# q8888620002/Group-Attribution-for-Diffusion-Models

Measured on AMD Instinct MI355X. Metric: shapley_coalitions_per_hour, higher is better.
Workload: dtype f32; 1 GPU; CIFAR-20 DDPM sFT coalition (BASELINE configs[1]): gd_steps=1000 @B=128 + 10240 samples x 100 DDIM steps @B=32 (32 batches fused/launch), UNet2DModel widths [128, 256, 256, 256] 35.75M params fp32; step = 1/1000 coalition = 1 train step + 1 sampler step @B=1024, enqueued on 3 HIP streams (the train step belongs to a later coalition: independent work); coalitions_in_flight=3

## Files before the change

group-attribution-for-diffusion-models_amd/csrc/gemm_dev.h:

```cpp
#pragma once
#include "gad_common.h"

namespace gadk {

constexpr int BK = 32;
constexpr int NTHREADS = 256;

static __device__ __attribute__((aligned(64))) float g_zero_block[16];

__device__ __forceinline__ int kc_off(int r, int q) { return r * BK + ((q ^ ((r >> 1) & 7)) << 2); }

__device__ __forceinline__ void glds16(const float* src, float* dst_wave_uniform) {
  __builtin_amdgcn_global_load_lds((const __attribute__((address_space(1))) void*)src,
                                   (__attribute__((address_space(3))) void*)dst_wave_uniform, 16, 0, 0);
}

__device__ __forceinline__ void barrier_after_dma() {
  __builtin_amdgcn_s_waitcnt(0x0F70);
  __syncthreads();
}

struct FastDiv {
  unsigned mul, shift;
  __device__ __forceinline__ int div(int n) const { return (int)((__umulhi((unsigned)n, mul) + (unsigned)n) >> shift); }
};

struct DevArgs {
  FastDiv fdC, fdKW, fdHoWo, fdWo, fdRpg, fdTaps;
  int kperm, taps;
  const float* A;
  const float* B;
  float* C;
  const unsigned short* Bh;
  const float* A2;
  int a_split, ldx2;
  const float* Ak2;
  const float* Bk2;
  int lda2, ldb2, k_split;
  int M, N, K;
  int lda, ldb, ldc;
  int batch_inner;
  long sA0, sA1, sB0, sB1, sC0, sC1;
  gad_conv_geom g;
  float alpha;
  const float* bias;
  const float* rowadd;
  int rows_per_group, ld_rowadd;
  const float* residual;
  int ldr;
  float* ws;
  int tiles_m, tiles_n, splitk, ktiles_per_split;
  int epi_vec;
};

__device__ __forceinline__ f32x4 ldg4(const float* p) { return *reinterpret_cast<const f32x4*>(p); }
__device__ __forceinline__ f32x4 zero4() { return f32x4{0.f, 0.f, 0.f, 0.f}; }
__device__ __forceinline__ f32x4 keep_if(f32x4 v, bool ok) { return ok ? v : zero4(); }

__device__ __forceinline__ int wave_id() { return __builtin_amdgcn_readfirstlane((int)(threadIdx.x >> 6)); }

template <int ROWS>
struct KCSlots {
  static constexpr int NS = ROWS / 32;
  __device__ static int row(int i) { return (threadIdx.x >> 3) + 32 * i; }
  __device__ static int kq4() { return ((threadIdx.x & 7) ^ ((threadIdx.x >> 4) & 7)) * 4; }
  __device__ static float* dma_dst(float* tile, int i) { return tile + (wave_id() * 8 + 32 * i) * BK; }
  __device__ static void store(float* lds, const f32x4* v, unsigned mask) {
#pragma unroll
    for (int i = 0; i < NS; ++i)
      *reinterpret_cast<f32x4*>(lds + row(i) * BK + (threadIdx.x & 7) * 4) = keep_if(v[i], (mask >> i) & 1u);
  }
};
template <int ROWS>
struct MCSlots {
  static constexpr int NS = ROWS / 32;
  static constexpr int F4 = ROWS / 4;
  static constexpr int KSTEP = NTHREADS / F4;
  __device__ static int krow(int i) { return threadIdx.x / F4 + KSTEP * i; }
  __device__ static int rq4() { return (threadIdx.x % F4) * 4; }
  __device__ static float* dma_dst(float* tile, int i) { return tile + (wave_id() * (KSTEP / 4) + KSTEP * i) * ROWS; }
  __device__ static void store(float* lds, const f32x4* v, unsigned mask) {
#pragma unroll
    for (int i = 0; i < NS; ++i)
      *reinterpret_cast<f32x4*>(lds + krow(i) * ROWS + rq4()) = keep_if(v[i], (mask >> i) & 1u);
  }
};

__device__ __forceinline__ const float* sel_src(const float* base, long off, bool ok) {
  const float* b = ok ? base : (const float*)g_zero_block;
  return b + (off & -(long)ok);
}


__device__ __forceinline__ int xcd_remap(int bid, int nwg) {
  int xcd = bid & 7, q = nwg >> 3, rr = nwg & 7;
  return (xcd < rr ? xcd * (q + 1) : rr * (q + 1) + (xcd - rr) * q) + (bid >> 3);
}

constexpr int EPI_LD = 40;
constexpr int EPI_WAVE = 32 * EPI_LD;

template <bool KC, int ROWS>
__device__ __forceinline__ f32x4 read_frag(const float* lds, int row, int g, int h) {
  if (KC) {
    return *reinterpret_cast<const f32x4*>(lds + kc_off(row, 2 * g + h));
  } else {
    const float* p = lds + (8 * g + 4 * h) * ROWS + row;
    return f32x4{p[0], p[ROWS], p[2 * ROWS], p[3 * ROWS]};
  }
}

template <int ROWS>
struct WinoKC : KCSlots<ROWS> {
  using S = KCSlots<ROWS>;
  const float* ptr[S::NS];
  long off;
  __device__ void init(const float* b, int ld, int row0, int nrows) {
#pragma unroll
    for (int i = 0; i < S::NS; ++i) {
      int r = row0 + S::row(i);
      r = r < nrows ? r : nrows - 1;
      ptr[i] = b + (long)r * ld + S::kq4();
    }
    off = 0;
  }
  __device__ __forceinline__ const float* src(int i) const { return ptr[i] + off; }
};

__device__ __forceinline__ void wino4_bt(const f32x4 (&d)[6], f32x4 (&t)[6]) {
  t[0] = 4.f * d[0] - 5.f * d[2] + d[4];
  t[1] = -4.f * (d[1] + d[2]) + d[3] + d[4];
  t[2] = 4.f * (d[1] - d[2]) - d[3] + d[4];
  t[3] = 2.f * (d[3] - d[1]) - d[2] + d[4];
  t[4] = 2.f * (d[1] - d[3]) - d[2] + d[4];
  t[5] = 4.f * d[1] - 5.f * d[3] + d[5];
// ... 4 lines not shown
```

group-attribution-for-diffusion-models_amd/csrc/gemm_f32.hip:

```cpp
#include "gad_common.h"
#include "gemm_dev.h"

using namespace gadk;

namespace gadk {
void launch_wino4_fused(const DevArgs& w, int bm, hipStream_t st);
}

namespace {

template <int ROWS, int VEC>
struct LoadKCDense : KCSlots<ROWS> {
  using S = KCSlots<ROWS>;
  const float* base;
  long roff[S::NS];
  unsigned rowmask;
  int kend, k;
  bool kok;
  __device__ void init(const float* b, int ld, int row0, int nrows, int kend_) {
    base = b;
    kend = kend_;
    rowmask = 0;
#pragma unroll
    for (int i = 0; i < S::NS; ++i) {
// ... 153 lines not shown
  __device__ void init(const float* b, int ld_, int row0, int nrows, int kend_) {
    kend = kend_;
    ld = ld_;
    int c0 = row0 + S::rq4();
    c0 = c0 < nrows ? c0 : nrows - 4;
#pragma unroll
    for (int i = 0; i < S::NS; ++i) ptr[i] = b + (long)S::krow(i) * ld + c0;
  }
  __device__ __forceinline__ void prep(int k0, unsigned& mask) { koff = (long)(k0 < kend ? k0 : kend - BK) * ld; mask = 0; }
  __device__ __forceinline__ const float* src(int i) const { return ptr[i] + koff; }
  __device__ __forceinline__ void slot(int, f32x4*, unsigned&) const {}
};
template <int ROWS>
struct LeanKC2 : KCSlots<ROWS> {
  using S = KCSlots<ROWS>;
  const float* ptr[S::NS];
  const float* ptr2[S::NS];
  int kend, ksplit, koff;
  bool second;
  __device__ void init(const float* b, int ld, const float* b2, int ld2, int ksplit_, int row0, int nrows, int kend_) {
    kend = kend_;
    ksplit = ksplit_;
#pragma unroll
    for (int i = 0; i < S::NS; ++i) {
      int r = row0 + S::row(i);
      r = r < nrows ? r : nrows - 1;
      ptr[i] = b + (long)r * ld + S::kq4();
      ptr2[i] = b2 + (long)r * ld2 + S::kq4();
    }
  }
  __device__ __forceinline__ void prep(int k0, unsigned& mask) {
    const int k = k0 < kend ? k0 : kend - BK;
    second = k >= ksplit;
    koff = second ? k - ksplit : k;
    mask = 0;
  }
  __device__ __forceinline__ const float* src(int i) const { return (second ? ptr2[i] : ptr[i]) + koff; }
  __device__ __forceinline__ void slot(int, f32x4*, unsigned&) const {}
};
template <int ROWS>
struct LeanMC2 : MCSlots<ROWS> {
  using S = MCSlots<ROWS>;
  const float* ptr[S::NS];
  const float* ptr2[S::NS];
  int kend, ksplit, ld, ld2;
  long koff;
  bool second;
  __device__ void init(const float* b, int ld_, const float* b2, int ld2_, int ksplit_, int row0, int nrows, int kend_) {
    kend = kend_;
    ksplit = ksplit_;
    ld = ld_;
    ld2 = ld2_;
    int c0 = row0 + S::rq4();
    c0 = c0 < nrows ? c0 : nrows - 4;
#pragma unroll
    for (int i = 0; i < S::NS; ++i) {
      ptr[i] = b + (long)S::krow(i) * ld + c0;
      ptr2[i] = b2 + (long)S::krow(i) * ld2 + c0;
    }
  }
  __device__ __forceinline__ void prep(int k0, unsigned& mask) {
    const int k = k0 < kend ? k0 : kend - BK;
    second = k >= ksplit;
    koff = second ? (long)(k - ksplit) * ld2 : (long)k * ld;
    mask = 0;
  }
  __device__ __forceinline__ const float* src(int i) const { return (second ? ptr2[i] : ptr[i]) + koff; }
  __device__ __forceinline__ void slot(int, f32x4*, unsigned&) const {}
};

template <int ROWS, bool TRANSPOSED, int VEC, bool TWO = false>
struct LoadConvRows : KCSlots<ROWS> {
  using S = KCSlots<ROWS>;
  const float* x;
  const float* x2;
  int csplit, ldx2;
  gad_conv_geom g;
  FastDiv fdC, fdKW;
  int bh[S::NS], bw[S::NS], boff[S::NS];
  unsigned rowmask;
  int kend, hlim, wlim;
  int k, c, r, s;
  bool kok;
  __device__ void init(const float* x_, const DevArgs& p, int row0, int nrows, int kend_) {
    x = x_;
    x2 = p.A2;
    csplit = p.a_split;
    ldx2 = p.ldx2;
    g = p.g;
    fdC = p.fdC;
    fdKW = p.fdKW;
    kend = kend_;
    hlim = g.upsample ? 2 * g.H : g.H;
    wlim = g.upsample ? 2 * g.W : g.W;
    rowmask = 0;
#pragma unroll
    for (int i = 0; i < S::NS; ++i) {
      int m = row0 + S::row(i);
      bool ok = m < nrows;
      int mm = ok ? m : 0;
      int img = p.fdHoWo.div(mm), rem = mm - img * (g.Ho * g.Wo);
      int oh = p.fdWo.div(rem), ow = rem - oh * g.Wo;
      boff[i] = img * g.H * g.W;
      rowmask |= (unsigned)ok << i;
      if (TRANSPOSED) {
        bh[i] = oh + g.pad_t;
        bw[i] = ow + g.pad_l;
      } else {
        bh[i] = oh * g.stride - g.pad_t;
        bw[i] = ow * g.stride - g.pad_l;
      }
    }
  }
  __device__ __forceinline__ long pix(int i, int rr, int ss, bool& ok) const { return (long)pixidx(i, rr, ss, ok) * g.ldx; }
  __device__ __forceinline__ int pixidx(int i, int rr, int ss, bool& ok) const {
    int ih, iw;
    if (TRANSPOSED) {
      int nh = bh[i] - rr, nw = bw[i] - ss;
      ok = (nh | nw) >= 0;
      if (g.stride == 2) {
        ok = ok && !((nh | nw) & 1);
        nh >>= 1;
        nw >>= 1;
      } else if (g.stride != 1) {
        ok = ok && (nh % g.stride == 0) && (nw % g.stride == 0);
        nh /= g.stride;
        nw /= g.stride;
      }
      ih = nh;
      iw = nw;
    } else {
      ih = bh[i] + rr;
      iw = bw[i] + ss;
      ok = (ih | iw) >= 0;
    }
    ok = ok && ih < hlim && iw < wlim;
    if (g.upsample) {
      ih >>= 1;
      iw >>= 1;
    }
    return boff[i] + ih * g.W + iw;
  }
  __device__ __forceinline__ void prep(int k0, unsigned& mask) {
    k = k0 + S::kq4();
    kok = k < kend;
    int kk = kok ? k : 0;
    int tap = fdC.div(kk);
    c = kk - tap * g.C;
    r = fdKW.div(tap);
    s = tap - r * g.KW;
    mask = rowmask;
  }
  __device__ __forceinline__ const float* src(int i) const {
    bool ok;
    if (TWO) {
      int pi = pixidx(i, r, s, ok);
      ok = ok && kok && ((rowmask >> i) & 1u);
      const bool second = c >= csplit;
      long off = second ? (long)pi * ldx2 + (c - csplit) : (long)pi * g.ldx + c;
      return sel_src(second ? x2 : x, off, ok);
    }
    long off = pix(i, r, s, ok) + c;
    ok = ok && kok && ((rowmask >> i) & 1u);
    return sel_src(x, off, ok);
  }
  __device__ __forceinline__ void slot(int i, f32x4* v, unsigned& mask) const {
    f32x4 t = zero4();
#pragma unroll
    for (int e = 0; e < 4; ++e) {
      int ke = k + e;
      bool ko = ke < kend;
      int kk = ko ? ke : 0;
      int tap = fdC.div(kk), cc = kk - tap * g.C;
      int rr = fdKW.div(tap), ss = tap - rr * g.KW;
      bool ok;
      long off = pix(i, rr, ss, ok) + cc;
      ok = ok && ko;
      float val = x[off & -(long)ok];
// ... 51 lines not shown
    fdHoWo = p.fdHoWo;
    fdWo = p.fdWo;
    kend = kend_;
    hlim = g.upsample ? 2 * g.H : g.H;
    wlim = g.upsample ? 2 * g.W : g.W;
    int n = col0 + S::rq4();
#pragma unroll
    for (int e = 0; e < NE; ++e) {
      int ne = n + e;
      nok[e] = ne < ncols;
      int nn = nok[e] ? ne : 0;
      int tap = p.fdC.div(nn);
      c[e] = nn - tap * g.C;
      r[e] = p.fdKW.div(tap);
      s[e] = tap - r[e] * g.KW;
    }
  }
  __device__ __forceinline__ void prep(int k0_, unsigned& mask) {
    k0 = k0_;
    mask = 0;
  }
  __device__ __forceinline__ long off_of(int i, int e, bool& ok) const {
    int m = k0 + S::krow(i);
    bool mok = m < kend;
    int mm = mok ? m : 0;
    int img = fdHoWo.div(mm), rem = mm - img * (g.Ho * g.Wo);
    int oh = fdWo.div(rem), ow = rem - oh * g.Wo;
    int ih = oh * g.stride - g.pad_t + r[e], iw = ow * g.stride - g.pad_l + s[e];
    ok = mok && nok[e] && (ih | iw) >= 0 && ih < hlim && iw < wlim;
    if (g.upsample) {
      ih >>= 1;
      iw >>= 1;
    }
    return (long)(img * g.H * g.W + ih * g.W + iw) * g.ldx + c[e];
  }
  __device__ __forceinline__ const float* src(int i) const {
    bool ok;
    long off = off_of(i, 0, ok);
    return sel_src(x, off, ok);
  }
  __device__ __forceinline__ void slot(int i, f32x4* v, unsigned& mask) const {
    f32x4 t = zero4();
#pragma unroll
    for (int e = 0; e < NE; ++e) {
      bool ok;
      long off = off_of(i, e, ok);
      float val = x[off & -(long)ok];
      t[e] = ok ? val : 0.f;
    }
    v[i] = t;
    mask |= 1u << i;
  }
};

template <int MODE, int ROWS, int VEC>
struct ALoader;
template <int ROWS, int VEC>
struct ALoader<GAD_A_KC, ROWS, VEC> : LoadKCDense<ROWS, VEC> {
  static constexpr bool KC = true;
  __device__ void setup(const DevArgs& p, const float* a, int row0, int kend) { this->init(a, p.lda, row0, p.M, kend); }
};
template <int ROWS, int VEC>
struct ALoader<GAD_A_MC, ROWS, VEC> : LoadMCDense<ROWS, VEC> {
  static constexpr bool KC = false;
  __device__ void setup(const DevArgs& p, const float* a, int row0, int kend) { this->init(a, p.lda, row0, p.M, kend); }
};
template <int ROWS, int VEC>
struct ALoader<GAD_A_CONV, ROWS, VEC> : LoadConvRows<ROWS, false, VEC> {
  static constexpr bool KC = true;
  __device__ void setup(const DevArgs& p, const float* a, int row0, int kend) { this->init(a, p, row0, p.M, kend); }
};
constexpr int A_CONV2 = 16;
template <int ROWS, int VEC>
struct ALoader<A_CONV2, ROWS, VEC> : LoadConvRows<ROWS, false, VEC, true> {
  static constexpr bool KC = true;
  __device__ void setup(const DevArgs& p, const float* a, int row0, int kend) { this->init(a, p, row0, p.M, kend); }
};
template <int ROWS, int VEC>
struct ALoader<GAD_A_CONVT, ROWS, VEC> : LoadConvRows<ROWS, true, VEC> {
  static constexpr bool KC = true;
  __device__ void setup(const DevArgs& p, const float* a, int row0, int kend) { this->init(a, p, row0, p.M, kend); }
};

constexpr int A_KC2 = 17;
template <int ROWS, int VEC>
struct ALoader<A_KC2, ROWS, VEC> : LoadKCDense2<ROWS> {
  static constexpr bool KC = true;
  __device__ void setup(const DevArgs& p, const float* a, int row0, int kend) {
    this->init(a, p.lda, p.Ak2, p.lda2, p.k_split, row0, p.M, kend);
  }
};

constexpr int A_KC_L = 20, A_MC_L = 21, B_KC_L = 22, B_MC_L = 23, A_KC2_L = 24, B_KC2_L = 25, B_MC2_L = 26;
template <int ROWS, int VEC>
struct ALoader<A_KC_L, ROWS, VEC> : LeanKC<ROWS> {
  static constexpr bool KC = true;
  __device__ void setup(const DevArgs& p, const float* a, int row0, int kend) { this->init(a, p.lda, row0, p.M, kend); }
};
template <int ROWS, int VEC>
struct ALoader<A_MC_L, ROWS, VEC> : LeanMC<ROWS> {
  static constexpr bool KC = false;
  __device__ void setup(const DevArgs& p, const float* a, int row0, int kend) { this->init(a, p.lda, row0, p.M, kend); }
};
template <int ROWS, int VEC>
struct ALoader<A_KC2_L, ROWS, VEC> : LeanKC2<ROWS> {
  static constexpr bool KC = true;
  __device__ void setup(const DevArgs& p, const float* a, int row0, int kend) {
    this->init(a, p.lda, p.Ak2, p.lda2, p.k_split, row0, p.M, kend);
  }
};

template <int MODE, int ROWS, int VEC>
struct BLoader;
constexpr int B_KC2 = 18, B_MC2 = 19;
template <int ROWS, int VEC>
struct BLoader<B_KC_L, ROWS, VEC> : LeanKC<ROWS> {
  static constexpr bool KC = true;
  __device__ void setup(const DevArgs& p, const float* b, int col0, int kend) { this->init(b, p.ldb, col0, p.N, kend); }
};
template <int ROWS, int VEC>
struct BLoader<B_MC_L, ROWS, VEC> : LeanMC<ROWS> {
  static constexpr bool KC = false;
  __device__ void setup(const DevArgs& p, const float* b, int col0, int kend) { this->init(b, p.ldb, col0, p.N, kend); }
};
template <int ROWS, int VEC>
struct BLoader<B_KC2_L, ROWS, VEC> : LeanKC2<ROWS> {
  static constexpr bool KC = true;
  __device__ void setup(const DevArgs& p, const float* b, int col0, int kend) {
    this->init(b, p.ldb, p.Bk2, p.ldb2, p.k_split, col0, p.N, kend);
  }
};
template <int ROWS, int VEC>
struct BLoader<B_MC2_L, ROWS, VEC> : LeanMC2<ROWS> {
  static constexpr bool KC = false;
  __device__ void setup(const DevArgs& p, const float* b, int col0, int kend) {
    this->init(b, p.ldb, p.Bk2, p.ldb2, p.k_split, col0, p.N, kend);
  }
};
template <int ROWS, int VEC>
struct BLoader<B_KC2, ROWS, VEC> : LoadKCDense2<ROWS> {
  static constexpr bool KC = true;
  __device__ void setup(const DevArgs& p, const float* b, int col0, int kend) {
    this->init(b, p.ldb, p.Bk2, p.ldb2, p.k_split, col0, p.N, kend);
  }
};
template <int ROWS, int VEC>
struct BLoader<B_MC2, ROWS, VEC> : LoadMCDense2<ROWS> {
  static constexpr bool KC = false;
  __device__ void setup(const DevArgs& p, const float* b, int col0, int kend) {
    this->init(b, p.ldb, p.Bk2, p.ldb2, p.k_split, col0, p.N, kend);
  }
};
template <int ROWS, int VEC>
struct BLoader<GAD_B_KC, ROWS, VEC> : LoadKCDense<ROWS, VEC> {
  static constexpr bool KC = true;
  __device__ void setup(const DevArgs& p, const float* b, int col0, int kend) { this->init(b, p.ldb, col0, p.N, kend); }
};
template <int ROWS, int VEC>
struct BLoader<GAD_B_MC, ROWS, VEC> : LoadMCDense<ROWS, VEC> {
  static constexpr bool KC = false;
  __device__ void setup(const DevArgs& p, const float* b, int col0, int kend) { this->init(b, p.ldb, col0, p.N, kend); }
};
template <int ROWS, int VEC>
struct BLoader<GAD_B_WDGRAD, ROWS, VEC> : LoadWDgrad<ROWS, VEC> {
  static constexpr bool KC = false;
  __device__ void setup(const DevArgs& p, const float* b, int col0, int kend) { this->init(b, p, col0, p.N, kend); }
};
template <int ROWS, int VEC>
struct BLoader<GAD_B_CONV, ROWS, VEC> : LoadConvCols<ROWS, VEC> {
  static constexpr bool KC = false;
  __device__ void setup(const DevArgs& p, const float* b, int col0, int kend) { this->init(b, p, col0, p.N, kend); }
};


template <int TM, int TN, int BM, int BN, int WM = 2, int WN = 2>
__device__ __forceinline__ void store_block(const DevArgs& p, const f32x16 (&acc)[TM][TN], int row0, int col0, int wm, int wn,
                                            int h, int l31, float* C, int ldc, const float* R, bool direct,
                                            float* scratch = nullptr) {
  if (scratch != nullptr && p.epi_vec) {
    const int lane = l31 + 32 * h;
    const int rr = lane >> 3, c4 = (lane & 7) * 4;
#pragma unroll
    for (int j = 0; j < TN; ++j) {
      const int n = col0 + wn * (BN / WN) + j * 32 + c4;
      const bool n_ok = n < p.N;
      float b0 = 0.f, b1 = 0.f, b2 = 0.f, b3 = 0.f;
      if (direct && p.bias && n_ok) {
        const f32x4 t = ldg4(p.bias + n);
        b0 = t[0]; b1 = t[1]; b2 = t[2]; b3 = t[3];
      }
#pragma unroll
      for (int i = 0; i < TM; ++i) {
#pragma unroll
        for (int e = 0; e < 16; ++e) scratch[((e & 3) + 8 * (e >> 2) + 4 * h) * EPI_LD + l31] = acc[i][j][e];
#pragma unroll
        for (int q = 0; q < 4; ++q) {
          const int r = rr + 8 * q;
          f32x4 v = *reinterpret_cast<const f32x4*>(scratch + r * EPI_LD + c4);
          const int m = row0 + wm * (BM / WM) + i * 32 + r;
          if (m >= p.M || !n_ok) continue;
          if (direct) {
            v = f32x4{__builtin_fmaf(v[0], p.alpha, b0), __builtin_fmaf(v[1], p.alpha, b1), __builtin_fmaf(v[2], p.alpha, b2),
                      __builtin_fmaf(v[3], p.alpha, b3)};
            if (p.rowadd) v += ldg4(p.rowadd + (long)p.fdRpg.div(m) * p.ld_rowadd + n);
            if (R) v += ldg4(R + (long)m * p.ldr + n);
          }
          *reinterpret_cast<f32x4*>(C + (long)m * ldc + n) = v;
        }
      }
    }
    return;
  }
#pragma unroll
  for (int j = 0; j < TN; ++j) {
    int n = col0 + wn * (BN / WN) + j * 32 + l31;
    if (n >= p.N) continue;
    float bias = (direct && p.bias) ? p.bias[n] : 0.f;
#pragma unroll
    for (int i = 0; i < TM; ++i) {
#pragma unroll
      for (int e = 0; e < 16; ++e) {
        int m = row0 + wm * (BM / WM) + i * 32 + (e & 3) + 8 * (e >> 2) + 4 * h;
        if (m >= p.M) continue;
        float v = acc[i][j][e];
        if (direct) {
          v = __builtin_fmaf(v, p.alpha, bias);
          if (p.rowadd) v += p.rowadd[(long)p.fdRpg.div(m) * p.ld_rowadd + n];
          if (R) v += R[(long)m * p.ldr + n];
        }
        C[(long)m * ldc + n] = v;
      }
    }
  }
}


template <int AM, int BMODE, int BM, int BN, int VEC, int TAG = 0>
__global__ __launch_bounds__(NTHREADS) void gemm_kernel(const DevArgs p) {
  constexpr int TM = BM / 64, TN = BN / 64;
  using AL = ALoader<AM, BM, VEC>;
  using BL = BLoader<BMODE, BN, VEC>;
  constexpr int A_TILE = BK * BM;
  constexpr int B_TILE = BK * BN;
  __shared__ __attribute__((aligned(16))) float lds[2 * (A_TILE + B_TILE)];

  const int t = xcd_remap(blockIdx.x, gridDim.x);
  int tiles = p.tiles_m * p.tiles_n;
  int zs = t / tiles, rem = t - zs * tiles;
  int tile_m = rem / p.tiles_n, tile_n = rem - tile_m * p.tiles_n;
  int z = zs / p.splitk, split = zs - z * p.splitk;
  int z0 = z / p.batch_inner, z1 = z - z0 * p.batch_inner;
  const float* A = p.A + z0 * p.sA0 + z1 * p.sA1;
  const float* B = p.B + z0 * p.sB0 + z1 * p.sB1;

  int row0 = tile_m * BM, col0 = tile_n * BN;
  int kbeg = split * p.ktiles_per_split * BK;
  int kend = min(p.K, kbeg + p.ktiles_per_split * BK);
  int nkt = (kend - kbeg + BK - 1) / BK;
  const int kt0 = split * p.ktiles_per_split;
  auto k0_of = [&](int kt) -> int {
    if (!p.kperm) return (kt0 + kt) * BK;
    int j = kt0 + kt;
    int chunk = p.fdTaps.div(j), tap = j - chunk * p.taps;
    return tap * p.g.C + chunk * BK;
  };
  if (p.kperm) kend = p.K;

  AL al;
  BL bl;
  al.setup(p, A, row0, kend);
  bl.setup(p, B, col0, kend);

  const int tid = threadIdx.x, wave = tid >> 6, lane = tid & 63;
  const int wm = wave >> 1, wn = wave & 1, h = lane >> 5, l31 = lane & 31;

  f32x16 acc[TM][TN];
#pragma unroll
  for (int i = 0; i < TM; ++i)
#pragma unroll
    for (int j = 0; j < TN; ++j)
#pragma unroll
      for (int e = 0; e < 16; ++e) acc[i][j][e] = 0.f;

  f32x4 ra[VEC == 4 ? 1 : AL::NS], rb[VEC == 4 ? 1 : BL::NS];
  unsigned ma = 0, mb = 0;
  auto stage_slot = [&](int piece, float* ta, float* tb) {
    constexpr int NSA = AL::NS, NSB = BL::NS;
    if (piece < NSA) {
      if (VEC == 4) glds16(al.src(piece), AL::dma_dst(ta, piece));
      else al.slot(piece, ra, ma);
    } else if (piece < NSA + NSB) {
      if (VEC == 4) glds16(bl.src(piece - NSA), BL::dma_dst(tb, piece - NSA));
      else bl.slot(piece - NSA, rb, mb);
    }
  };
  auto stage_commit = [&](float* ta, float* tb) {
    if (VEC != 4) {
      AL::store(ta, ra, ma);
      BL::store(tb, rb, mb);
    }
  };
  if (nkt > 0) {
    al.prep(k0_of(0), ma);
    bl.prep(k0_of(0), mb);
#pragma unroll
    for (int q = 0; q < AL::NS + BL::NS; ++q) stage_slot(q, lds, lds + A_TILE);
    stage_commit(lds, lds + A_TILE);
  }
  barrier_after_dma();

  for (int kt = 0; kt < nkt; ++kt) {
    float* cur = lds + (kt & 1) * (A_TILE + B_TILE);
    float* nxt = lds + ((kt + 1) & 1) * (A_TILE + B_TILE);
    const float* la = cur;
    const float* lb = cur + A_TILE;
    const int knext = (kt + 1 < nkt) ? k0_of(kt + 1) : p.K;
    al.prep(knext, ma);
    bl.prep(knext, mb);
    f32x4 fa[2][TM], fb[2][TN];
#pragma unroll
    for (int i = 0; i < TM; ++i) fa[0][i] = read_frag<AL::KC, BM>(la, wm * (BM / 2) + i * 32 + l31, 0, h);
#pragma unroll
    for (int j = 0; j < TN; ++j) fb[0][j] = read_frag<BL::KC, BN>(lb, wn * (BN / 2) + j * 32 + l31, 0, h);
#pragma unroll
    for (int g = 0; g < 4; ++g) {
#pragma unroll
      for (int s = 0; s < 4; ++s) {
#pragma unroll
        for (int i = 0; i < TM; ++i)
#pragma unroll
          for (int j = 0; j < TN; ++j)
            acc[i][j] = __builtin_amdgcn_mfma_f32_32x32x2f32(fa[g & 1][i][s], fb[g & 1][j][s], acc[i][j], 0, 0, 0);
        stage_slot(g * 4 + s, nxt, nxt + A_TILE);
        if (s == 1 && g < 3) {
#pragma unroll
          for (int i = 0; i < TM; ++i) fa[(g + 1) & 1][i] = read_frag<AL::KC, BM>(la, wm * (BM / 2) + i * 32 + l31, g + 1, h);
#pragma unroll
          for (int j = 0; j < TN; ++j) fb[(g + 1) & 1][j] = read_frag<BL::KC, BN>(lb, wn * (BN / 2) + j * 32 + l31, g + 1, h);
        }
#pragma unroll
        for (int q = 0; q < TM * TN; ++q) {
          __builtin_amdgcn_sched_group_barrier(0x008, 1, 0);
          __builtin_amdgcn_sched_group_barrier(0x002, 7, 0);
        }
        __builtin_amdgcn_sched_barrier(0);
      }
    }
    stage_commit(nxt, nxt + A_TILE);
    barrier_after_dma();
  }

  const bool direct = p.splitk == 1;
  float* C = direct ? p.C + z0 * p.sC0 + z1 * p.sC1 : p.ws + (long)zs * p.M * p.N;
  const float* R = (direct && p.residual) ? p.residual + z0 * p.sC0 + z1 * p.sC1 : nullptr;
  const int ldc = direct ? p.ldc : p.N;
  store_block<TM, TN, BM, BN>(p, acc, row0, col0, wm, wn, h, l31, C, ldc, R, direct, lds + (tid >> 6) * EPI_WAVE);
}

typedef __bf16 bf16x4_t __attribute__((ext_vector_type(4)));
typedef __bf16 bf16x8_t __attribute__((ext_vector_type(8)));
typedef short s16x4_t __attribute__((ext_vector_type(4)));
constexpr int LDK = BK + 8;
template <int ROWS> struct LdmOf { static constexpr int v = ROWS == 128 ? 160 : 96; };

__device__ __forceinline__ void store_bf16x4(unsigned short* dst, f32x4 v) {
  bf16x4_t h = {(__bf16)v[0], (__bf16)v[1], (__bf16)v[2], (__bf16)v[3]};
  *reinterpret_cast<bf16x4_t*>(dst) = h;
}

template <bool KC, int ROWS>
struct Bf16Tile;
template <int ROWS>
struct Bf16Tile<true, ROWS> {
  static constexpr int ELEMS = LDK * ROWS;
  __device__ static void put(unsigned short* tile, int i, f32x4 v) {
    store_bf16x4(tile + KCSlots<ROWS>::row(i) * LDK + KCSlots<ROWS>::kq4(), v);
  }
  __device__ static bf16x8_t frag(const unsigned short* tile, int r0, int ks, int lane) {
    return *reinterpret_cast<const bf16x8_t*>(tile + (r0 + (lane & 31)) * LDK + ks * 16 + 8 * (lane >> 5));
  }
};
template <int ROWS>
struct Bf16Tile<false, ROWS> {
  static constexpr int LDM = LdmOf<ROWS>::v;
  static constexpr int ELEMS = BK * LDM;
  __device__ static void put(unsigned short* tile, int i, f32x4 v) {
    store_bf16x4(tile + MCSlots<ROWS>::krow(i) * LDM + MCSlots<ROWS>::rq4(), v);
  }
  __device__ static bf16x8_t frag(const unsigned short* tile, int r0, int ks, int lane) {
    const int q = (lane & 15) >> 2, pp = lane & 3;
    const unsigned short* a0 = tile + (ks * 16 + 8 * (lane >> 5) + q) * LDM + r0 + 16 * ((lane >> 4) & 1) + 4 * pp;
    s16x4_t lo = __builtin_amdgcn_ds_read_tr16_b64_v4i16((__attribute__((address_space(3))) s16x4_t*)a0);
    s16x4_t hi = __builtin_amdgcn_ds_read_tr16_b64_v4i16((__attribute__((address_space(3))) s16x4_t*)(a0 + 4 * LDM));
    typedef short s16x8_t __attribute__((ext_vector_type(8)));
    s16x8_t both = {lo[0], lo[1], lo[2], lo[3], hi[0], hi[1], hi[2], hi[3]};
    return __builtin_bit_cast(bf16x8_t, both);
  }
};

template <int AM, int BMODE, int BM, int BN>
__global__ __launch_bounds__(NTHREADS) void gemm_bf16_kernel(const DevArgs p) {
  constexpr int TM = BM / 64, TN = BN / 64;
  using AL = ALoader<AM, BM, 4>;
  using BL = BLoader<BMODE, BN, 4>;
  using AT = Bf16Tile<AL::KC, BM>;
  using BT = Bf16Tile<BL::KC, BN>;
  constexpr int A_TILE = AT::ELEMS;
  constexpr int B_TILE = BT::ELEMS;
  __shared__ __attribute__((aligned(16))) unsigned short lds[2 * (A_TILE + B_TILE)];

  const int t = xcd_remap(blockIdx.x, gridDim.x);
  int tiles = p.tiles_m * p.tiles_n;
  int zs = t / tiles, rem = t - zs * tiles;
  int tile_m = rem / p.tiles_n, tile_n = rem - tile_m * p.tiles_n;
  int z = zs / p.splitk, split = zs - z * p.splitk;
  int z0 = z / p.batch_inner, z1 = z - z0 * p.batch_inner;
  const float* A = p.A + z0 * p.sA0 + z1 * p.sA1;
  const float* B = p.B + z0 * p.sB0 + z1 * p.sB1;

  int row0 = tile_m * BM, col0 = tile_n * BN;
  int kbeg = split * p.ktiles_per_split * BK;
  int kend = min(p.K, kbeg + p.ktiles_per_split * BK);
  int nkt = (kend - kbeg + BK - 1) / BK;
  const int kt0 = split * p.ktiles_per_split;
  auto k0_of = [&](int kt) -> int {
    if (!p.kperm) return (kt0 + kt) * BK;
    int j = kt0 + kt;
    int chunk = p.fdTaps.div(j), tap = j - chunk * p.taps;
    return tap * p.g.C + chunk * BK;
  };
  if (p.kperm) kend = p.K;

  AL al;
  BL bl;
  al.setup(p, A, row0, kend);
  bl.setup(p, B, col0, kend);

  const int tid = threadIdx.x, wave = tid >> 6, lane = tid & 63;
  const int wm = wave >> 1, wn = wave & 1, h = lane >> 5, l31 = lane & 31;
// ... 1079 lines not shown
#pragma unroll
      for (int i = 0; i < 6; ++i) gg[i][sx] = o[i];
    }
    float* u = dst + doff + (long)co * Cin + ci;
    const long ps = (long)Cout * Cin;
#pragma unroll
    for (int i = 0; i < 6; ++i) {
      float o[6];
      gmul(gg[i][0], gg[i][1], gg[i][2], o);
#pragma unroll
      for (int j = 0; j < 6; ++j) u[(long)(6 * i + j) * ps] = o[j];
    }
  }
}

struct WinoOut {
  const float* Mb;
  float* y;
  const float* bias;
  const float* rowadd;
  const float* residual;
  int N, ldc, ldr, ld_rowadd, Ho, Wo, TH, TW;
  long T;
  float alpha;
};

__device__ __forceinline__ void wino4_at(const f32x4 (&m)[6], f32x4 (&y)[4]) {
  const f32x4 s12 = m[1] + m[2], d12 = m[1] - m[2], s34 = m[3] + m[4], d34 = m[3] - m[4];
  y[0] = m[0] + s12 + s34;
  y[1] = d12 + 2.f * d34;
  y[2] = s12 + 4.f * s34;
  y[3] = d12 + 8.f * d34 + m[5];
}

template <bool HALF>
__global__ __launch_bounds__(256) void wino4_output_kernel(const WinoOut p) {
  const int N4 = p.N >> 2;
  const long idx = (long)blockIdx.x * 256 + threadIdx.x;
  if (idx >= p.T * N4) return;
  const long tile = idx / N4;
  const int n = (int)(idx - tile * N4) * 4;
  const int per = p.TH * p.TW;
  const int img = (int)(tile / per);
  const int r = (int)(tile - (long)img * per);
  const int ty = r / p.TW, tx = r - ty * p.TW;
  const long pos_stride = p.T * p.N;
  const float* src = p.Mb + tile * p.N + n;
  f32x4 t[4][HALF ? 4 : 6];
#pragma unroll
  for (int nu = 0; nu < (HALF ? 4 : 6); ++nu) {
    f32x4 m[6], col[4];
#pragma unroll
    for (int xi = 0; xi < 6; ++xi) m[xi] = ldg4(src + (long)((HALF ? 4 : 6) * xi + nu) * pos_stride);
    wino4_at(m, col);
#pragma unroll
    for (int i = 0; i < 4; ++i) t[i][nu] = col[i];
  }
  const f32x4 b = p.bias ? ldg4(p.bias + n) : zero4();
  const f32x4 ra = p.rowadd ? ldg4(p.rowadd + (long)img * p.ld_rowadd + n) : zero4();
#pragma unroll
  for (int i = 0; i < 4; ++i) {
    f32x4 y[4];
    if constexpr (HALF) {
#pragma unroll
      for (int j = 0; j < 4; ++j) y[j] = t[i][j];
    } else {
      f32x4 row6[6];
#pragma unroll
      for (int j = 0; j < 6; ++j) row6[j] = t[i][HALF ? 0 : j];
      wino4_at(row6, y);
    }
#pragma unroll
    for (int j = 0; j < 4; ++j) {
      const long pix = ((long)img * p.Ho + 4 * ty + i) * p.Wo + 4 * tx + j;
      f32x4 v = f32x4{__builtin_fmaf(y[j][0], p.alpha, b[0]), __builtin_fmaf(y[j][1], p.alpha, b[1]),
                      __builtin_fmaf(y[j][2], p.alpha, b[2]), __builtin_fmaf(y[j][3], p.alpha, b[3])};
      if (p.rowadd) v += ra;
      if (p.residual) v += ldg4(p.residual + pix * p.ldr + n);
      *reinterpret_cast<f32x4*>(p.y + pix * p.ldc + n) = v;
    }
  }
}

__global__ __launch_bounds__(256) void wino4_dy_kernel(const WinoIn p) {
  const int C4 = p.C >> 2;
  const long idx = (long)blockIdx.x * 256 + threadIdx.x;
  if (idx >= p.T * C4) return;
  const long tile = idx / C4;
  const int c = (int)(idx - tile * C4) * 4;
  const int per = p.TH * p.TW;
  const int n = (int)(tile / per);
  const int r = (int)(tile - (long)n * per);
  const int ty = r / p.TW, tx = r - ty * p.TW;
  const float* img = p.x + ((long)n * p.H * p.W + (long)(4 * ty) * p.W + 4 * tx) * p.ldx + c;
  auto amul = [](const f32x4 (&d)[4], f32x4 (&t)[6]) {
    const f32x4 s02 = d[0] + d[2], s13 = d[1] + d[3], a = d[0] + 4.f * d[2], b = 2.f * d[1] + 8.f * d[3];
    t[0] = d[0];
    t[1] = s02 + s13;
    t[2] = s02 - s13;
    t[3] = a + b;
    t[4] = a - b;
    t[5] = d[3];
  };
  f32x4 t[6][4];
#pragma unroll
  for (int dx = 0; dx < 4; ++dx) {
    f32x4 d[4], col[6];
#pragma unroll
    for (int dy = 0; dy < 4; ++dy) d[dy] = ldg4(img + ((long)dy * p.W + dx) * p.ldx);
    amul(d, col);
#pragma unroll
    for (int i = 0; i < 6; ++i) t[i][dx] = col[i];
  }
  const long pos_stride = p.T * p.C;
  float* out = p.V + tile * p.C + c;
#pragma unroll
  for (int i = 0; i < 6; ++i) {
    f32x4 v[6];
    amul(t[i], v);
#pragma unroll
    for (int j = 0; j < 6; ++j) *reinterpret_cast<f32x4*>(out + (long)(6 * i + j) * pos_stride) = v[j];
  }
}

__global__ __launch_bounds__(256) void wino4_dw_kernel(const float* dU, float* dW, int Cout, int Cin, int ldc) {
  const int C4 = Cin >> 2;
  const long idx = (long)blockIdx.x * 256 + threadIdx.x;
  if (idx >= (long)Cout * C4) return;
  const int co = (int)(idx / C4), ci = (int)(idx - (long)co * C4) * 4;
  const long ps = (long)Cout * Cin;
  const float* src = dU + (long)co * Cin + ci;
  auto gt = [](const f32x4 (&m)[6], f32x4 (&o)[3]) {
    const f32x4 s12 = m[1] + m[2], d21 = m[2] - m[1], s34 = m[3] + m[4], d34 = m[3] - m[4];
    o[0] = 0.25f * m[0] - (1.f / 6.f) * s12 + (1.f / 24.f) * s34;
    o[1] = (1.f / 6.f) * d21 + (1.f / 12.f) * d34;
    o[2] = (1.f / 6.f) * (s34 - s12) + m[5];
  };
  f32x4 t[3][6];
#pragma unroll
  for (int nu = 0; nu < 6; ++nu) {
    f32x4 m[6], col[3];
#pragma unroll
    for (int xi = 0; xi < 6; ++xi) m[xi] = ldg4(src + (long)(6 * xi + nu) * ps);
    gt(m, col);
#pragma unroll
    for (int r = 0; r < 3; ++r) t[r][nu] = col[r];
  }
  float* dst = dW + (long)co * ldc + ci;
#pragma unroll
  for (int r = 0; r < 3; ++r) {
    f32x4 o[3];
    gt(t[r], o);
#pragma unroll
    for (int sx = 0; sx < 3; ++sx) *reinterpret_cast<f32x4*>(dst + (long)(r * 3 + sx) * Cin) = o[sx];
  }
}

static FastDiv make_fastdiv(unsigned d) {
  FastDiv f;
  if (d == 0) d = 1;
  unsigned l = 0;
  while ((1ull << l) < d) ++l;
  f.shift = l;
  f.mul = (unsigned)((((1ull << l) - d) << 32) / d + 1);
  if (d == 1) f.mul = 0;
  return f;
}

static int pick_vec(const gad_gemm_args* a) {
  int vec = 4;
  const int am = a->a_mode, bmode = a->b_mode;
  if (am == GAD_A_KC && (a->K % 4 != 0 || a->lda % 4 != 0)) vec = 1;
  if (am == GAD_A_MC && (a->M % 4 != 0 || a->lda % 4 != 0)) vec = 1;
  if (bmode == GAD_B_KC && (a->K % 4 != 0 || a->ldb % 4 != 0)) vec = 1;
  if (bmode == GAD_B_MC && (a->N % 4 != 0 || a->ldb % 4 != 0)) vec = 1;
  if ((am == GAD_A_CONV || am == GAD_A_CONVT || bmode == GAD_B_CONV) && (a->g.C % 4 != 0 || a->g.ldx % 4 != 0)) vec = 1;
  return vec;
}

enum : int32_t {
  HINT_128 = 1,
  HINT_64 = 2,
  HINT_128x64 = 3,
  HINT_WGRAD_96 = 4, HINT_WGRAD_64 = 5, HINT_WGRAD_32 = 6,
  HINT_WINO2 = 7,
  HINT_WINO4 = 8,
  HINT_WINO4_FUSED32 = 9,
  HINT_WINO4_THREE = 10,
  HINT_WINO4_FUSED64 = 11,
  HINT_SPLIT_M = 1000,
};

struct Plan {
  int bm, bn, tiles_m, tiles_n, splitk, ktiles_per_split;
  long nblocks;
};

static bool dense_128x64_ok(const gad_gemm_args* a) {
  const bool dense = (a->a_mode == GAD_A_KC || a->a_mode == GAD_A_MC) && (a->b_mode == GAD_B_KC || a->b_mode == GAD_B_MC) &&
                     !(a->a_mode == GAD_A_MC && a->b_mode == GAD_B_KC);
  return dense && !a->A2 && pick_vec(a) == 4 && !(a->operand_precision == 1);
}
// ... 341 lines not shown
    const double t3 = t_gemm + (mb3 + y_bytes) / 4.9e12 + 12e-6;
    const bool full_ok = !(a->flags & GAD_GEMM_GENERAL_LOADERS) && a->tile_hint != HINT_WINO4_THREE;
    if (full_ok && (a->tile_hint == HINT_WINO4_FUSED32 || a->tile_hint == HINT_WINO4_FUSED64 || (t_full < 1.05 * t3 && blocks32 >= 320))) {
      p4.fused4 = 2;
      p4.bm = a->tile_hint == HINT_WINO4_FUSED64 ? 64 : narrow ? 65 : 32;
      p4.bn = p4.bm == 65 ? 32 : 64;
      p4.tiles_m = (int)gad_ceil_div(p4.T, p4.bm == 32 ? 32 : 64);
      p4.tiles_n = (int)gad_ceil_div(a->N, p4.bn);
    }
    const double mb = p4.fused4 == 2 ? 0.0 : mb3;
    p4.bytes = (int64_t)(vb + mb);
    t4 = (x_bytes + vb) / 4.9e12 + (p4.fused4 == 2 ? t_full : t3) + 6e-6;
  }
  if (a->tile_hint == HINT_WINO2 || force4) {
    if (a->tile_hint == HINT_WINO2 && f2_ok) { *wp = p2; return true; }
    if (force4 && f4_ok) { *wp = p4; return true; }
    return false;
  }
  double t_direct;
  PatchPlan pp;
  if (use_patch_conv_f32(a, &pp)) {
    t_direct = (double)gad_ceil_div(pp.blocks, 512) * pp.chunks_per_split * 9.0 * (128.0 * pp.bn * 64.0) / 0.264e12;
    if (pp.splitk > 1) t_direct += 4e-6 + (double)a->M * a->N * 4.0 * (pp.splitk + 1) / 3.0e12;
  } else {
    t_direct = 2.0 * a->M * (double)a->N * a->K / 110e12;
  }
  const double tw = t2 < t4 ? t2 : t4;
  if (!(tw < 0.9 * t_direct)) return false;
  *wp = t2 < t4 ? p2 : p4;
  return true;
}

struct WinoWgradPlan {
  long T;
  int64_t wy_bytes, v_bytes, du_bytes, bytes;
};
static bool use_wino_wgrad(const gad_gemm_args* a, WinoWgradPlan* wq) {
  const gad_conv_geom& g = a->g;
  if (!(a->flags & GAD_GEMM_WINO_WGRAD) || (a->flags & (GAD_GEMM_NO_WINO | GAD_GEMM_NO_PATCH | GAD_GEMM_INTERNAL_WINO4))) return false;
  if (a->operand_precision != 0 || a->a_mode != GAD_A_MC || a->b_mode != GAD_B_CONV || a->A2 || a->A_k2 || a->batch > 1) return false;
  if (!same_3x3(g) || (g.Ho & 3) || (g.Wo & 3)) return false;
  if (g.C % 4 != 0 || g.ldx % 4 != 0 || a->M % 4 != 0 || a->lda % 4 != 0 || a->N != 9 * g.C || a->ldc % 4 != 0) return false;
  if ((a->tile_hint != 0 && a->tile_hint != HINT_WINO4) || a->splitk_hint > 0 || a->K % (g.Ho * g.Wo) != 0) return false;
  if (a->alpha != 1.f || a->bias || a->rowadd || a->residual) return false;
  if (!(gad_aligned16(a->A) && gad_aligned16(a->B) && gad_aligned16(a->C))) return false;
  wq->T = (long)a->K / 16;
  wq->wy_bytes = (int64_t)36 * wq->T * a->M * 4;
  wq->v_bytes = (int64_t)36 * wq->T * g.C * 4;
  wq->du_bytes = (int64_t)36 * a->M * g.C * 4;
  wq->bytes = wq->wy_bytes + wq->v_bytes + wq->du_bytes;
  if (a->tile_hint == HINT_WINO4) return true;
  const double dy_bytes = 4.0 * a->K * a->M, x_bytes = 4.0 * (double)(a->K / (g.Ho * g.Wo)) * g.H * g.W * g.C;
  const double t_w = (dy_bytes + x_bytes + (double)wq->wy_bytes + (double)wq->v_bytes) / 4.9e12 + 36.0 * wq->T * a->M * (double)g.C * 2.0 / 100e12 +
                     3.0 * (double)wq->du_bytes / 3.0e12 + 30e-6;
  const double t_direct = 2.0 * a->K * (double)a->M * a->N / 115e12;
  return t_w < 0.9 * t_direct;
}


static gad_gemm_args products36(const gad_gemm_args* a, const float* A, const float* B, float* C, int am, int bm, int M, int N, int K) {
  gad_gemm_args sub = *a;
  sub.A = A; sub.B = B; sub.C = C;
  sub.a_mode = am; sub.b_mode = bm;
  sub.M = M; sub.N = N; sub.K = K;
  sub.lda = am == GAD_A_MC ? M : K; sub.ldb = bm == GAD_B_MC ? N : K; sub.ldc = N;
  sub.batch = 36; sub.batch_inner = 1;
  sub.strideA0 = (int64_t)M * K; sub.strideB0 = (int64_t)N * K; sub.strideC0 = (int64_t)M * N;
  sub.strideA1 = sub.strideB1 = sub.strideC1 = 0;
  sub.tile_hint = 0; sub.splitk_hint = 0;
  sub.flags = GAD_GEMM_INTERNAL_WINO4;
  sub.B_wino = nullptr; sub.B_wino4 = nullptr; sub.wino_ws = nullptr; sub.wino_ws_bytes = 0;
  sub.A2 = nullptr;
  return sub;
}
static gad_gemm_args wino_wgrad_products_args(const gad_gemm_args* a, const WinoWgradPlan& wq, float* Wy, float* V, float* dU) {
  return products36(a, Wy, V, dU, GAD_A_MC, GAD_B_MC, a->M, a->g.C, (int)wq.T);
}
static gad_gemm_args wino4_products_args(const gad_gemm_args* a, const WinoPlan& wp, float* V, float* Mb) {
  gad_gemm_args sub = products36(a, V, a->B_wino4, Mb, GAD_A_KC, GAD_B_KC, (int)wp.T, a->N, a->g.C);
  sub.alpha = 1.f; sub.bias = nullptr; sub.rowadd = nullptr; sub.residual = nullptr;
  return sub;
}

enum class RouteKind { ENGINE, PATCH_F32, PATCH_BF16, FEWOUT, WGRAD_PATCH, WINO, WINO_WGRAD, SPLIT_N, SPLIT_M };
struct Route {
  RouteKind kind;
  gad_gemm_args a;
  int vec;
  bool bf16;
  Plan plan;
  PatchPlan pp;
  WinoPlan wp;
  WinoWgradPlan wq;
  int wbm, wsplits;
  int split;
};

static Route route_of(const gad_gemm_args* args) {
  Route r{};
  r.a = canonical(args);
  const gad_gemm_args* a = &r.a;
  r.vec = pick_vec(a);
  r.bf16 = use_bf16(a);
  if (use_wino_wgrad(a, &r.wq)) r.kind = RouteKind::WINO_WGRAD;
  else if (use_wino(a, &r.wp)) r.kind = RouteKind::WINO;
  else if (patch_split_n(a, &r.split)) {
    r.kind = RouteKind::SPLIT_N;
    use_patch_conv_f32(a, &r.pp);
  } else if (wgrad_split_m(a, &r.split)) {
    r.kind = RouteKind::SPLIT_M;
    r.wsplits = wgrad_patch_splits(a, &r.wbm);
  } else if (use_fewout_conv(a)) r.kind = RouteKind::FEWOUT;
  else if ((r.wsplits = wgrad_patch_splits(a, &r.wbm))) r.kind = RouteKind::WGRAD_PATCH;
  else if (use_patch_conv(a)) r.kind = RouteKind::PATCH_BF16;
  else if (use_patch_conv_f32(a, &r.pp)) r.kind = RouteKind::PATCH_F32;
  else {
    r.kind = RouteKind::ENGINE;
    r.plan = make_plan(a);
  }
  return r;
}

struct Report { int kid, tile, splitk; };
static Report report(const Route& r) {
  switch (r.kind) {
    case RouteKind::ENGINE: return {r.bf16 ? 1 : 0, r.plan.bm, r.plan.splitk};
    case RouteKind::PATCH_F32: return {2, r.pp.bn, r.pp.splitk};
    case RouteKind::SPLIT_N: return {2, 224, r.pp.splitk};
    case RouteKind::SPLIT_M: return {2, 224, r.wsplits};
    case RouteKind::WGRAD_PATCH: return {2, r.wbm, r.wsplits};
    case RouteKind::PATCH_BF16: return {3, 128, 1};
    case RouteKind::FEWOUT: return {4, 256, 1};
    case RouteKind::WINO: return {r.wp.f == 2 ? 5 : 6, r.wp.f == 2 ? r.wp.bn : (r.wp.fused4 == 2 ? r.wp.bm : 128), 1};
    case RouteKind::WINO_WGRAD: return {7, 128, 1};
  }
  return {-1, 0, 0};
}

static void split_halves(const Route& r, gad_gemm_args* lo, gad_gemm_args* hi) {
  const gad_gemm_args* a = &r.a;
  const int s = r.split;
  *lo = *a;
  *hi = *a;
  if (r.kind == RouteKind::SPLIT_M) {
    if (a->tile_hint >= HINT_SPLIT_M) lo->tile_hint = hi->tile_hint = 0;
    lo->M = s;
    hi->M = a->M - s;
    hi->A = a->A + s;
    hi->C = a->C + (long)s * a->ldc;
    return;
  }
  lo->B_wino = lo->B_wino4 = hi->B_wino = hi->B_wino4 = nullptr;
  lo->wino_ws = hi->wino_ws = nullptr;
  lo->wino_ws_bytes = hi->wino_ws_bytes = 0;
  lo->N = s;
  hi->N = a->N - s;
  hi->B = a->B + (long)s * a->ldb;
  hi->C = a->C + s;
  if (a->bias) hi->bias = a->bias + s;
  if (a->rowadd) hi->rowadd = a->rowadd + s;
  if (a->residual) hi->residual = a->residual + s;
}

static int64_t workspace_bytes(const Route& r) {
  const gad_gemm_args* a = &r.a;
  switch (r.kind) {
    case RouteKind::ENGINE: case RouteKind::PATCH_F32: case RouteKind::WGRAD_PATCH: case RouteKind::PATCH_BF16: case RouteKind::FEWOUT: {
      const int splitk = report(r).splitk;
      return splitk > 1 ? (int64_t)(a->batch > 0 ? a->batch : 1) * splitk * a->M * a->N * (int64_t)sizeof(float) : 0;
    }
    case RouteKind::WINO: {
      if (r.wp.f == 2 || r.wp.fused4) return 0;
      const gad_gemm_args sub = wino4_products_args(a, r.wp, nullptr, nullptr);
      return gad_gemm_workspace_bytes(&sub);
    }
    case RouteKind::WINO_WGRAD: {
      const gad_gemm_args sub = wino_wgrad_products_args(a, r.wq, nullptr, nullptr, nullptr);
      return gad_gemm_workspace_bytes(&sub);
    }
    case RouteKind::SPLIT_N: case RouteKind::SPLIT_M: {
      gad_gemm_args lo, hi;
      split_halves(r, &lo, &hi);
      const int64_t wl = gad_gemm_workspace_bytes(&lo), wh = gad_gemm_workspace_bytes(&hi);
      return wl > wh ? wl : wh;
    }
  }
  return 0;
}

extern "C" int gad_gemm_uses_bf16(const gad_gemm_args* a) { return a && route_of(a).bf16 ? 1 : 0; }

extern "C" int gad_gemm_kernel_id(const gad_gemm_args* a) { return a ? report(route_of(a)).kid : -1; }

extern "C" int gad_gemm_plan(const gad_gemm_args* a, int32_t* tile, int32_t* splitk, int32_t* vec) {
  GAD_CHECK(a && tile && splitk && vec, "gad_gemm_plan: null pointer");
  const Route r = route_of(a);
  const Report rep = report(r);
  *tile = rep.tile;
  *splitk = rep.splitk;
  *vec = r.vec;
  return 0;
}

extern "C" int64_t gad_gemm_wino_bytes(const gad_gemm_args* a) {
  if (!a) return 0;
  const Route r = route_of(a);
  return r.kind == RouteKind::WINO ? r.wp.bytes : r.kind == RouteKind::WINO_WGRAD ? r.wq.bytes : 0;
}

extern "C" int64_t gad_gemm_workspace_bytes(const gad_gemm_args* a) { return a ? workspace_bytes(route_of(a)) : 0; }

extern "C" int gad_wino_weights(const float* src, float* dst, const int64_t* table, int64_t n_tiles, void* stream) {
  GAD_CHECK(src && dst && table && n_tiles > 0 && n_tiles < (1L << 31), "gad_wino_weights: bad arguments");
  static_assert(sizeof(long) == sizeof(int64_t), "table rows are 64-bit");
  hipLaunchKernelGGL(wino_weights_kernel, dim3((unsigned)n_tiles), dim3(256), 0, (hipStream_t)stream, src, dst, (const long*)table);
  GAD_LAUNCH_CHECK("gad_wino_weights");
  return 0;
}

extern "C" int gad_wino4_weights(const float* src, float* dst, const int64_t* table, int64_t n_tiles, void* stream) {
  GAD_CHECK(src && dst && table && n_tiles > 0 && n_tiles < (1L << 31), "gad_wino4_weights: bad arguments");
  hipLaunchKernelGGL(wino4_weights_kernel, dim3((unsigned)n_tiles), dim3(256), 0, (hipStream_t)stream, src, dst, (const long*)table);
  GAD_LAUNCH_CHECK("gad_wino4_weights");
  return 0;
}


static int check_args(const gad_gemm_args* a) {
  GAD_CHECK(a->M > 0 && a->N > 0 && a->K > 0, "gad_gemm: bad shape M=%d N=%d K=%d", a->M, a->N, a->K);
  const int am = a->a_mode, bmode = a->b_mode;
  GAD_CHECK(gad_aligned16(a->A) && gad_aligned16(a->B), "gad_gemm: A/B must be 16-byte aligned");
  const int k_first = a->A_k2 ? a->k_split : a->K;
  if (am == GAD_A_KC) GAD_CHECK(a->lda >= k_first, "gad_gemm: A_KC needs lda >= K (K=%d lda=%d)", k_first, a->lda);
  if (am == GAD_A_MC) GAD_CHECK(a->lda >= a->M, "gad_gemm: A_MC needs lda >= M (M=%d lda=%d)", a->M, a->lda);
  if (bmode == GAD_B_KC) GAD_CHECK(a->ldb >= k_first, "gad_gemm: B_KC needs ldb >= K (K=%d ldb=%d)", k_first, a->ldb);
  if (bmode == GAD_B_MC) GAD_CHECK(a->ldb >= a->N, "gad_gemm: B_MC needs ldb >= N (N=%d ldb=%d)", a->N, a->ldb);
  const bool convA = am == GAD_A_CONV || am == GAD_A_CONVT;
  if (convA || bmode == GAD_B_CONV || bmode == GAD_B_WDGRAD) {
    const gad_conv_geom& g = a->g;
    GAD_CHECK(g.H > 0 && g.W > 0 && g.C > 0 && g.Ho > 0 && g.Wo > 0 && g.KH > 0 && g.KW > 0 && g.stride > 0 &&
              g.ldx >= (a->A2 ? a->a_split : g.C), "gad_gemm: bad conv geometry");
    GAD_CHECK((long)g.H * g.W * g.ldx < (1L << 31), "gad_gemm: image too large for 32-bit pixel offsets");
    if (convA) {
      GAD_CHECK(a->K == g.KH * g.KW * g.C, "gad_gemm: conv K=%d != KH*KW*C=%d", a->K, g.KH * g.KW * g.C);
      GAD_CHECK(a->M % (g.Ho * g.Wo) == 0, "gad_gemm: conv M=%d not a multiple of Ho*Wo", a->M);
      GAD_CHECK((long)(a->M / (g.Ho * g.Wo)) * g.H * g.W < (1L << 31), "gad_gemm: too many pixels");
    }
    if (bmode == GAD_B_WDGRAD) {
      GAD_CHECK(am == GAD_A_CONVT, "gad_gemm: B_WDGRAD pairs with A_CONVT");
      GAD_CHECK(a->N % 4 == 0, "gad_gemm: B_WDGRAD needs N%%4==0 (N=%d)", a->N);
    }
    if (bmode == GAD_B_CONV) {
      GAD_CHECK(a->N == g.KH * g.KW * g.C, "gad_gemm: wgrad N=%d != KH*KW*C=%d", a->N, g.KH * g.KW * g.C);
      GAD_CHECK(a->K % (g.Ho * g.Wo) == 0, "gad_gemm: wgrad K=%d not a multiple of Ho*Wo", a->K);
      GAD_CHECK((long)(a->K / (g.Ho * g.Wo)) * g.H * g.W < (1L << 31), "gad_gemm: too many pixels");
    }
  }
  const int vec = pick_vec(a);
  if (a->A2) {
    GAD_CHECK(am == GAD_A_CONV && bmode == GAD_B_KC, "gad_gemm: A2 (two-source gather) is an A_CONV x B_KC feature");
    GAD_CHECK(a->a_split > 0 && a->a_split < a->g.C && a->a_split % 32 == 0 && a->g.C % 32 == 0,
              "gad_gemm: two-source gather needs a_split and C multiples of 32 (a_split=%d C=%d)", a->a_split, a->g.C);
    GAD_CHECK(a->ldx2 >= a->g.C - a->a_split && a->ldx2 % 4 == 0 && gad_aligned16(a->A2) && vec == 4,
              "gad_gemm: two-source gather: bad ldx2 / alignment");
  }
  if (a->A_k2) {
    GAD_CHECK(am == GAD_A_KC && (bmode == GAD_B_KC || bmode == GAD_B_MC) && a->B_k2 && !a->A2 && a->batch <= 1,
              "gad_gemm: the K-concatenated form (A_k2 / B_k2) is an A_KC x B_KC|B_MC feature");
    GAD_CHECK(a->k_split > 0 && a->k_split < a->K && a->k_split % 32 == 0, "gad_gemm: k_split must be a multiple of 32 inside (0, K) (k_split=%d K=%d)", a->k_split, a->K);
    const int k2 = a->K - a->k_split;
    GAD_CHECK(a->lda >= a->k_split && a->lda_k2 >= k2 && a->lda_k2 % 4 == 0 && k2 % 4 == 0 && gad_aligned16(a->A_k2) && gad_aligned16(a->B_k2),
              "gad_gemm: K-concatenated operands need 16-byte alignment and K2 %% 4 == 0 (K2=%d lda_k2=%d)", k2, a->lda_k2);
    if (bmode == GAD_B_KC) GAD_CHECK(a->ldb >= a->k_split && a->ldb_k2 >= k2 && a->ldb_k2 % 4 == 0, "gad_gemm: bad ldb_k2");
    else GAD_CHECK(a->ldb_k2 >= a->N && a->ldb_k2 % 4 == 0, "gad_gemm: bad ldb_k2");
    GAD_CHECK(vec == 4, "gad_gemm: the K-concatenated form needs the float4 path");
  }
  if (a->rowadd) GAD_CHECK(a->rows_per_group > 0 && a->ld_rowadd >= a->N, "gad_gemm: bad rowadd");
  if (a->residual) GAD_CHECK(a->ldr >= a->N, "gad_gemm: bad residual stride");
  GAD_CHECK(a->ldc >= a->N, "gad_gemm: ldc < N");
  GAD_CHECK(a->operand_precision == 0 || a->operand_precision == 1, "gad_gemm: operand_precision must be 0 (f32) or 1 (bf16 allowed)");
  return 0;
}

static int check_stage_flags(const Route& r) {
  const bool only_input = (r.a.flags & GAD_GEMM_WINO_ONLY_INPUT) != 0, skip_input = (r.a.flags & GAD_GEMM_WINO_SKIP_INPUT) != 0;
  GAD_CHECK(!(only_input && skip_input), "gad_gemm: GAD_GEMM_WINO_ONLY_INPUT and GAD_GEMM_WINO_SKIP_INPUT exclude each other");
  GAD_CHECK(!only_input || r.kind == RouteKind::WINO,
            "gad_gemm: GAD_GEMM_WINO_ONLY_INPUT on a launch that takes no Winograd forward route (kernel id %d)", report(r).kid);
  GAD_CHECK(!skip_input || r.kind == RouteKind::WINO || r.kind == RouteKind::WINO_WGRAD,
            "gad_gemm: GAD_GEMM_WINO_SKIP_INPUT on a launch that takes no Winograd route (kernel id %d)", report(r).kid);
  return 0;
}

static DevArgs dev_args(const gad_gemm_args* a) {
  DevArgs d;
  d.A = a->A; d.B = a->B; d.C = a->C;
  d.A2 = a->A2; d.a_split = a->a_split; d.ldx2 = a->ldx2;
  d.Ak2 = a->A_k2; d.Bk2 = a->B_k2; d.lda2 = a->lda_k2; d.ldb2 = a->ldb_k2; d.k_split = a->k_split;
  d.Bh = nullptr;
  d.M = a->M; d.N = a->N; d.K = a->K;
  d.lda = a->lda; d.ldb = a->ldb; d.ldc = a->ldc;
  d.batch_inner = a->batch_inner > 0 ? a->batch_inner : 1;
  d.sA0 = a->strideA0; d.sA1 = a->strideA1; d.sB0 = a->strideB0; d.sB1 = a->strideB1;
  d.sC0 = a->strideC0; d.sC1 = a->strideC1;
  d.g = a->g;
  d.fdC = make_fastdiv(a->g.C);
  d.fdKW = make_fastdiv(a->g.KW);
  d.fdHoWo = make_fastdiv((unsigned)a->g.Ho * a->g.Wo);
  d.fdWo = make_fastdiv(a->g.Wo);
  d.fdRpg = make_fastdiv(a->rows_per_group > 0 ? a->rows_per_group : 1);
  d.taps = a->g.KH * a->g.KW;
  d.fdTaps = make_fastdiv(d.taps > 0 ? d.taps : 1);
  const bool convA = a->a_mode == GAD_A_CONV || a->a_mode == GAD_A_CONVT;
  d.kperm = (convA && d.taps > 1 && a->g.C % BK == 0 && !(a->flags & GAD_GEMM_TAP_MAJOR_K)) ? 1 : 0;
  d.alpha = a->alpha;
  d.bias = a->bias; d.rowadd = a->rowadd; d.rows_per_group = a->rows_per_group > 0 ? a->rows_per_group : 1;
  d.ld_rowadd = a->ld_rowadd; d.residual = a->residual; d.ldr = a->ldr;
  d.ws = (float*)a->ws;
  d.tiles_m = d.tiles_n = d.splitk = d.ktiles_per_split = 1;
  d.epi_vec = (!(a->flags & GAD_GEMM_SCALAR_EPILOGUE) && gad_aligned16(a->C) && a->ldc % 4 == 0 && a->N % 4 == 0 &&
               a->strideC0 % 4 == 0 && a->strideC1 % 4 == 0 && (!a->bias || gad_aligned16(a->bias)) &&
               (!a->rowadd || (gad_aligned16(a->rowadd) && a->ld_rowadd % 4 == 0)) &&
               (!a->residual || (gad_aligned16(a->residual) && a->ldr % 4 == 0)) && (!a->ws || gad_aligned16(a->ws))) ? 1 : 0;
  return d;
}

static int launch_wino_wgrad(const Route& r, void* stream) {
  const gad_gemm_args* a = &r.a;
  const WinoWgradPlan& wq = r.wq;
  const gad_conv_geom& g = a->g;
  hipStream_t st = (hipStream_t)stream;
  GAD_CHECK(a->wino_ws && a->wino_ws_bytes >= wq.bytes && gad_aligned16(a->wino_ws),
            "gad_gemm: Winograd weight-gradient workspace too small or misaligned (%lld < %lld)", (long long)a->wino_ws_bytes, (long long)wq.bytes);
  float* Wy = (float*)a->wino_ws;
  float* V = Wy + wq.wy_bytes / 4;
  float* dU = V + wq.v_bytes / 4;
  const bool have_v = (a->flags & GAD_GEMM_WINO_SKIP_INPUT) && a->B_wino4 != nullptr;
  if (have_v) {
    GAD_CHECK(gad_aligned16(a->B_wino4), "gad_gemm: the kept Winograd input image (B_wino4 of a weight-gradient launch) must be 16-byte aligned");
    V = const_cast<float*>(a->B_wino4);
  }
  WinoIn wy;
  wy.x = a->A; wy.V = Wy;
  wy.H = g.Ho; wy.W = g.Wo; wy.C = a->M; wy.ldx = a->lda; wy.up = 0;
  wy.TH = g.Ho / 4; wy.TW = g.Wo / 4; wy.T = wq.T;
  WinoIn wi;
  wi.x = a->B; wi.V = V;
  wi.H = g.H; wi.W = g.W; wi.C = g.C; wi.ldx = g.ldx; wi.up = g.upsample ? 1 : 0;
  wi.TH = wy.TH; wi.TW = wy.TW; wi.T = wq.T;
  const long iy = wq.T * (a->M / 4), ix = wq.T * (g.C / 4);
  GAD_CHECK(gad_ceil_div(iy, 256) < (1L << 31) && gad_ceil_div(ix, 256) < (1L << 31), "gad_gemm: Winograd transform grid too large");
  hipLaunchKernelGGL(wino4_dy_kernel, dim3((unsigned)gad_ceil_div(iy, 256)), dim3(256), 0, st, wy);
  if (!have_v) hipLaunchKernelGGL(wino4_input_kernel, dim3((unsigned)gad_ceil_div(ix, 256)), dim3(256), 0, st, wi);
  GAD_LAUNCH_CHECK("gad_gemm(winograd wgrad transforms)");
  const gad_gemm_args sub = wino_wgrad_products_args(a, wq, Wy, V, dU);
  if (const int rc = gad_gemm(&sub, stream)) return rc;
  const long items = (long)a->M * (g.C / 4);
  hipLaunchKernelGGL(wino4_dw_kernel, dim3((unsigned)gad_ceil_div(items, 256)), dim3(256), 0, st, dU, a->C, a->M, g.C, a->ldc);
  GAD_LAUNCH_CHECK("gad_gemm(winograd wgrad output transform)");
  return 0;
}

static int launch_wino(const Route& r, const DevArgs& d, void* stream) {
  const gad_gemm_args* a = &r.a;
  const WinoPlan& wp = r.wp;
  const gad_conv_geom& g = a->g;
  hipStream_t st = (hipStream_t)stream;
  GAD_CHECK(a->wino_ws && a->wino_ws_bytes >= wp.bytes && gad_aligned16(a->wino_ws) && gad_aligned16(wp.f == 2 ? a->B_wino : a->B_wino4),
            "gad_gemm: Winograd workspace too small or misaligned (%lld < %lld)", (long long)a->wino_ws_bytes, (long long)wp.bytes);
  WinoIn wi;
  wi.x = a->A; wi.V = (float*)a->wino_ws;
  wi.H = g.H; wi.W = g.W; wi.C = g.C; wi.ldx = g.ldx; wi.up = g.upsample ? 1 : 0;
  wi.TH = g.Ho / wp.f; wi.TW = g.Wo / wp.f; wi.T = wp.T;
  const long items = wp.T * (g.C / 4);
  GAD_CHECK(gad_ceil_div(items, 256) < (1L << 31), "gad_gemm: Winograd input transform grid too large");
  const bool only_input = (a->flags & GAD_GEMM_WINO_ONLY_INPUT) != 0, skip_input = (a->flags & GAD_GEMM_WINO_SKIP_INPUT) != 0;
  auto products = [&](const float* U) {
    DevArgs w = d;
    w.A = wi.V; w.B = U;
    w.M = (int)wp.T; w.N = a->N; w.K = g.C;
    w.lda = g.C; w.ldb = g.C;
    w.sA0 = wp.T * (long)g.C; w.sB0 = (long)a->N * g.C;
    w.fdHoWo = make_fastdiv((unsigned)(wi.TH * wi.TW));
    w.fdWo = make_fastdiv((unsigned)wi.TW);
    w.tiles_m = wp.tiles_m; w.tiles_n = wp.tiles_n;
    return w;
  };
  if (wp.f == 4) {
    if (!skip_input) {
      hipLaunchKernelGGL(wino4_input_kernel, dim3((unsigned)gad_ceil_div(items, 256)), dim3(256), 0, st, wi);
      GAD_LAUNCH_CHECK("gad_gemm(winograd F4 input transform)");
    }
    if (only_input) return 0;
    if (wp.fused4 == 2) {
      GAD_CHECK((long)wp.tiles_m * wp.tiles_n < (1L << 31), "gad_gemm: Winograd grid too large");
      gadk::launch_wino4_fused(products(a->B_wino4), wp.bm, st);
      GAD_LAUNCH_CHECK("gad_gemm(winograd F4 fused products + output transform)");
      return 0;
    }
    float* Mb = wi.V + 36 * wp.T * (long)g.C;
    WinoOut wo;
    wo.Mb = Mb; wo.y = a->C; wo.bias = a->bias; wo.rowadd = a->rowadd; wo.residual = a->residual;
    wo.N = a->N; wo.ldc = a->ldc; wo.ldr = a->ldr; wo.ld_rowadd = a->ld_rowadd;
    wo.Ho = g.Ho; wo.Wo = g.Wo; wo.TH = wi.TH; wo.TW = wi.TW; wo.T = wp.T; wo.alpha = a->alpha;
    const long oitems = wp.T * (a->N / 4);
    if (wp.fused4 == 1) {
      DevArgs w = d;
      w.A = wi.V; w.B = a->B_wino4; w.C = Mb;
      w.M = (int)wp.T; w.N = a->N; w.K = g.C;
      w.lda = g.C; w.ldb = g.C; w.ldc = a->N;
      w.sA0 = wp.T * (long)g.C; w.sB0 = (long)a->N * g.C; w.sC0 = wp.T * (long)a->N;
      w.tiles_m = wp.tiles_m; w.tiles_n = wp.tiles_n;
      w.splitk = 1; w.bias = nullptr; w.rowadd = nullptr; w.residual = nullptr; w.alpha = 1.f;
      w.epi_vec = 1;
      dim3 grid((unsigned)((long)wp.tiles_m * wp.tiles_n * 6)), block(NTHREADS);
      if (wp.bm == 64) hipLaunchKernelGGL((wino4_gemm_kernel<64, 128>), grid, block, 0, st, w);
      else hipLaunchKernelGGL((wino4_gemm_kernel<128, 64>), grid, block, 0, st, w);
      GAD_LAUNCH_CHECK("gad_gemm(winograd F4 products)");
      hipLaunchKernelGGL(wino4_output_kernel<true>, dim3((unsigned)gad_ceil_div(oitems, 256)), dim3(256), 0, st, wo);
      GAD_LAUNCH_CHECK("gad_gemm(winograd F4 output transform)");
      return 0;
    }
    const gad_gemm_args sub = wino4_products_args(a, wp, wi.V, Mb);
    if (const int rc = gad_gemm(&sub, stream)) return rc;
    hipLaunchKernelGGL(wino4_output_kernel<false>, dim3((unsigned)gad_ceil_div(oitems, 256)), dim3(256), 0, st, wo);
    GAD_LAUNCH_CHECK("gad_gemm(winograd F4 output transform)");
    return 0;
  }
  if (!skip_input) {
    hipLaunchKernelGGL(wino_input_kernel, dim3((unsigned)gad_ceil_div(items, 256)), dim3(256), 0, st, wi);
    GAD_LAUNCH_CHECK("gad_gemm(winograd input transform)");
  }
  if (only_input) return 0;
  const DevArgs w = products(a->B_wino);
  dim3 grid((unsigned)((long)wp.tiles_m * wp.tiles_n)), block(NTHREADS);
// ... 41 lines not shown
  if (a->g.Wo == 64) GAD_WGRAD(64);
  else if (a->g.Wo == 32) GAD_WGRAD(32);
  else if (a->g.Wo == 16) GAD_WGRAD(16);
  else GAD_WGRAD(8);
#undef GAD_WGRAD
  GAD_LAUNCH_CHECK("gad_gemm(wgrad3x3 patch)");
  if (d.splitk > 1) {
    launch_splitk_reduce(d, 1, st);
    GAD_LAUNCH_CHECK("gad_gemm(wgrad splitk reduce)");
  }
  return 0;
}

static int launch_patch_bf16(const Route& r, DevArgs& d, hipStream_t st) {
  const gad_gemm_args* a = &r.a;
  d.tiles_m = (int)gad_ceil_div(a->M, 128);
  d.tiles_n = (int)gad_ceil_div(a->N, 128);
  d.splitk = 1;
  dim3 grid((unsigned)(d.tiles_m * d.tiles_n)), block(NTHREADS);
  const bool wb = a->B_bf16 != nullptr;
  if (wb) GAD_CHECK(gad_aligned16(a->B_bf16) && a->ldb % 8 == 0, "gad_gemm: B_bf16 must be 16-byte aligned with ldb %% 8 == 0");
  d.Bh = (const unsigned short*)a->B_bf16;
#define GAD_PATCH_BF16(W_, NI_)                                                                         \
  do {                                                                                                  \
    if (wb) hipLaunchKernelGGL((conv3x3_patch_bf16_kernel<W_, NI_, true>), grid, block, 0, st, d);      \
    else hipLaunchKernelGGL((conv3x3_patch_bf16_kernel<W_, NI_, false>), grid, block, 0, st, d);        \
  } while (0)
  if (a->g.Wo == 64) GAD_PATCH_BF16(64, 1);
  else if (a->g.Wo == 32) GAD_PATCH_BF16(32, 1);
  else if (a->g.Wo == 16) GAD_PATCH_BF16(16, 1);
  else if (a->g.Wo == 8) GAD_PATCH_BF16(8, 2);
  else GAD_PATCH_BF16(4, 8);
#undef GAD_PATCH_BF16
  GAD_LAUNCH_CHECK("gad_gemm(conv3x3 patch)");
  return 0;
}

static int launch_patch_f32(const Route& r, DevArgs& d, hipStream_t st) {
  const gad_gemm_args* a = &r.a;
  const PatchPlan& pp = r.pp;
  d.tiles_m = (int)gad_ceil_div(a->M, 128);
  d.tiles_n = (int)gad_ceil_div(a->N, pp.bn);
  d.splitk = pp.splitk;
  d.ktiles_per_split = pp.chunks_per_split;
  if (pp.splitk > 1) {
    int64_t need = (int64_t)pp.splitk * a->M * a->N * (int64_t)sizeof(float);
    GAD_CHECK(a->ws && a->ws_bytes >= need, "gad_gemm: patch-conv split-K workspace too small (%lld < %lld)", (long long)a->ws_bytes, (long long)need);
  }
  dim3 grid((unsigned)pp.blocks), block(NTHREADS);
  const bool dg = a->a_mode == GAD_A_CONVT;
#define GAD_PATCH(W_, NI_)                                                                                           \
  do {                                                                                                               \
    if (dg) hipLaunchKernelGGL((conv3x3_patch_f32_kernel<W_, NI_, true>), grid, block, 0, st, d);                    \
    else if (pp.bn == 96) hipLaunchKernelGGL((conv3x3_patch_f32_kernel<W_, NI_, false, 96>), grid, block, 0, st, d);   \
    else if (pp.bn == 160) hipLaunchKernelGGL((conv3x3_patch_f32_kernel<W_, NI_, false, 160>), grid, block, 0, st, d); \
    else hipLaunchKernelGGL((conv3x3_patch_f32_kernel<W_, NI_, false>), grid, block, 0, st, d);                      \
  } while (0)
  if (a->g.Wo == 64) GAD_PATCH(64, 1);
  else if (a->g.Wo == 32) GAD_PATCH(32, 1);
  else if (a->g.Wo == 16) GAD_PATCH(16, 1);
  else if (a->g.Wo == 8) GAD_PATCH(8, 2);
  else GAD_PATCH(4, 8);
#undef GAD_PATCH
  GAD_LAUNCH_CHECK("gad_gemm(conv3x3 patch f32)");
  if (pp.splitk > 1) {
    launch_splitk_reduce(d, 1, st);
    GAD_LAUNCH_CHECK("gad_gemm(patch splitk reduce)");
  }
  return 0;
}

static int launch_engine(const Route& r, DevArgs& d, hipStream_t st) {
  const gad_gemm_args* a = &r.a;
  const Plan& pl = r.plan;
  const int am = a->a_mode, bmode = a->b_mode, vec = r.vec;
  const bool bf16 = r.bf16;
  const long batch = a->batch > 0 ? a->batch : 1;
  GAD_CHECK(pl.nblocks > 0 && pl.nblocks < (1L << 31), "gad_gemm: grid too large");
  if (pl.splitk > 1) {
    int64_t need = (int64_t)batch * pl.splitk * a->M * a->N * (int64_t)sizeof(float);
    GAD_CHECK(a->ws && a->ws_bytes >= need, "gad_gemm: split-K workspace too small (%lld < %lld)", (long long)a->ws_bytes, (long long)need);
  }
  d.tiles_m = pl.tiles_m; d.tiles_n = pl.tiles_n; d.splitk = pl.splitk; d.ktiles_per_split = pl.ktiles_per_split;
  if (a->A2) {
    if (bf16) launch_bf16<A_CONV2, GAD_B_KC>(d, pl, st);
    else launch_mode<A_CONV2, GAD_B_KC, 4>(d, pl, st);
  } else if (a->A_k2) {
    const bool lean = vec == 4 && a->K % BK == 0 && a->k_split % BK == 0 && !(a->flags & GAD_GEMM_GENERAL_LOADERS);
    if (bmode == GAD_B_KC) {
      if (bf16 && lean) launch_bf16<A_KC2_L, B_KC2_L>(d, pl, st);
      else if (bf16) launch_bf16<A_KC2, B_KC2>(d, pl, st);
      else if (lean) launch_mode<A_KC2_L, B_KC2_L, 4>(d, pl, st);
      else launch_mode<A_KC2, B_KC2, 4>(d, pl, st);
    } else {
      if (bf16 && lean) launch_bf16<A_KC2_L, B_MC2_L>(d, pl, st);
      else if (bf16) launch_bf16<A_KC2, B_MC2>(d, pl, st);
      else if (lean) launch_mode<A_KC2_L, B_MC2_L, 4>(d, pl, st);
      else launch_mode<A_KC2, B_MC2, 4>(d, pl, st);
    }
  } else if (vec == 4 && a->K % BK == 0 && !(a->flags & GAD_GEMM_GENERAL_LOADERS) &&
             ((am == GAD_A_KC && (bmode == GAD_B_KC || bmode == GAD_B_MC)) || (am == GAD_A_MC && bmode == GAD_B_MC))) {
    if (bf16) {
      if (am == GAD_A_KC && bmode == GAD_B_KC) launch_bf16<A_KC_L, B_KC_L>(d, pl, st);
      else if (am == GAD_A_KC) launch_bf16<A_KC_L, B_MC_L>(d, pl, st);
      else launch_bf16<A_MC_L, B_MC_L>(d, pl, st);
    } else if (am == GAD_A_KC && bmode == GAD_B_KC) {
      if (a->flags & GAD_GEMM_INTERNAL_WINO4) launch_mode<A_KC_L, B_KC_L, 4, 1>(d, pl, st);
      else launch_mode<A_KC_L, B_KC_L, 4>(d, pl, st);
    }
    else if (am == GAD_A_KC) launch_mode<A_KC_L, B_MC_L, 4>(d, pl, st);
    else launch_mode<A_MC_L, B_MC_L, 4>(d, pl, st);
  } else
#define GAD_CASE(AMODE, BMODE_)                                                        \
  if (am == AMODE && bmode == BMODE_) {                                                \
    if (bf16) launch_bf16<AMODE, BMODE_>(d, pl, st);                                   \
    else if (vec == 4) launch_mode<AMODE, BMODE_, 4>(d, pl, st);                       \
    else launch_mode<AMODE, BMODE_, 1>(d, pl, st);                                     \
  } else
  GAD_CASE(GAD_A_KC, GAD_B_KC)
  GAD_CASE(GAD_A_KC, GAD_B_MC)
  GAD_CASE(GAD_A_MC, GAD_B_MC)
  GAD_CASE(GAD_A_CONV, GAD_B_KC)
  GAD_CASE(GAD_A_CONVT, GAD_B_WDGRAD)
  GAD_CASE(GAD_A_MC, GAD_B_CONV)
  {
    gad_set_error("gad_gemm: unsupported mode pair a_mode=%d b_mode=%d", am, bmode);
    return 1;
  }
#undef GAD_CASE
  GAD_LAUNCH_CHECK("gad_gemm");
  if (pl.splitk > 1) {
    launch_splitk_reduce(d, (int)batch, st);
    GAD_LAUNCH_CHECK("gad_gemm(splitk reduce)");
  }
  return 0;
}

extern "C" int gad_gemm(const gad_gemm_args* args, void* stream) {
  GAD_CHECK(args && args->A && args->B && args->C, "gad_gemm: null pointer");
  const gad_gemm_args canon = canonical(args);
  if (const int rc = check_args(&canon)) return rc;
  const Route r = route_of(&canon);
  if (const int rc = check_stage_flags(r)) return rc;
  hipStream_t st = (hipStream_t)stream;
  DevArgs d = dev_args(&r.a);
  switch (r.kind) {
    case RouteKind::SPLIT_N: case RouteKind::SPLIT_M: {
      gad_gemm_args lo, hi;
      split_halves(r, &lo, &hi);
      const int rc = gad_gemm(&lo, stream);
      return rc ? rc : gad_gemm(&hi, stream);
    }
    case RouteKind::WINO_WGRAD: return launch_wino_wgrad(r, stream);
    case RouteKind::WINO: return launch_wino(r, d, stream);
    case RouteKind::FEWOUT: return launch_fewout(r, d, st);
    case RouteKind::WGRAD_PATCH: return launch_wgrad_patch(r, d, st);
    case RouteKind::PATCH_BF16: return launch_patch_bf16(r, d, st);
    case RouteKind::PATCH_F32: return launch_patch_f32(r, d, st);
    case RouteKind::ENGINE: return launch_engine(r, d, st);
  }
  return 1;
}
```

group-attribution-for-diffusion-models_amd/gad/_capi.py:

```python
import ctypes as C
import os

_HERE = os.path.dirname(os.path.abspath(__file__))
LIB_PATH = os.path.join(_HERE, "libgad_hip.so")


class GadError(RuntimeError):
    pass


class ConvGeom(C.Structure):
    _fields_ = [("H", C.c_int32), ("W", C.c_int32), ("C", C.c_int32), ("ldx", C.c_int32),
                ("Ho", C.c_int32), ("Wo", C.c_int32), ("KH", C.c_int32), ("KW", C.c_int32),
                ("stride", C.c_int32), ("pad_t", C.c_int32), ("pad_l", C.c_int32), ("upsample", C.c_int32)]


class GemmArgs(C.Structure):
    _fields_ = [("A", C.c_void_p), ("B", C.c_void_p), ("C", C.c_void_p),
                ("a_mode", C.c_int32), ("b_mode", C.c_int32),
                ("M", C.c_int32), ("N", C.c_int32), ("K", C.c_int32),
                ("lda", C.c_int32), ("ldb", C.c_int32), ("ldc", C.c_int32),
                ("batch", C.c_int32), ("batch_inner", C.c_int32),
                ("strideA0", C.c_int64), ("strideA1", C.c_int64), ("strideB0", C.c_int64),
                ("strideB1", C.c_int64), ("strideC0", C.c_int64), ("strideC1", C.c_int64),
                ("g", ConvGeom),
                ("alpha", C.c_float), ("bias", C.c_void_p), ("rowadd", C.c_void_p),
                ("rows_per_group", C.c_int32), ("ld_rowadd", C.c_int32),
                ("residual", C.c_void_p), ("ldr", C.c_int32),
                ("ws", C.c_void_p), ("ws_bytes", C.c_int64),
                ("tile_hint", C.c_int32), ("splitk_hint", C.c_int32), ("operand_precision", C.c_int32),
                ("A2", C.c_void_p), ("a_split", C.c_int32), ("ldx2", C.c_int32), ("B_bf16", C.c_void_p),
                ("A_k2", C.c_void_p), ("B_k2", C.c_void_p), ("lda_k2", C.c_int32), ("ldb_k2", C.c_int32),
                ("k_split", C.c_int32), ("flags", C.c_int32),
                ("B_wino", C.c_void_p), ("wino_ws", C.c_void_p), ("wino_ws_bytes", C.c_int64), ("B_wino4", C.c_void_p)]


class GroupNormArgs(C.Structure):
    _fields_ = [("x", C.c_void_p), ("y", C.c_void_p), ("gamma", C.c_void_p), ("beta", C.c_void_p),
                ("mean", C.c_void_p), ("rstd", C.c_void_p), ("dy", C.c_void_p),
                ("dgamma", C.c_void_p), ("dbeta", C.c_void_p),
                ("B", C.c_int32), ("HW", C.c_int32), ("C", C.c_int32), ("G", C.c_int32),
                ("eps", C.c_float), ("silu", C.c_int32), ("ws", C.c_void_p), ("ws_bytes", C.c_int64),
                ("x2", C.c_void_p), ("C1", C.c_int32), ("flags", C.c_int32), ("dx_add", C.c_void_p)]


class AttentionArgs(C.Structure):
    _fields_ = [("q", C.c_void_p), ("k", C.c_void_p), ("v", C.c_void_p), ("o", C.c_void_p), ("lse", C.c_void_p),
                ("d_o", C.c_void_p), ("delta", C.c_void_p), ("dq", C.c_void_p), ("dk", C.c_void_p), ("dv", C.c_void_p),
                ("B", C.c_int32), ("heads", C.c_int32), ("Tq", C.c_int32), ("Tk", C.c_int32), ("d", C.c_int32),
                ("ldq", C.c_int32), ("ldk", C.c_int32), ("ldv", C.c_int32), ("ldo", C.c_int32),
                ("ld_do", C.c_int32), ("ld_dq", C.c_int32), ("ld_dk", C.c_int32), ("ld_dv", C.c_int32),
                ("stride_q", C.c_int64), ("stride_k", C.c_int64), ("stride_v", C.c_int64), ("stride_o", C.c_int64),
                ("stride_do", C.c_int64), ("stride_dq", C.c_int64), ("stride_dk", C.c_int64), ("stride_dv", C.c_int64),
                ("scale", C.c_float), ("operand_precision", C.c_int32),
                ("ws", C.c_void_p), ("ws_bytes", C.c_int64), ("flags", C.c_int32)]


ATTN_TWO_KERNEL_BWD, ATTN_NARROW_FWD = 1, 2


class HGemmArgs(C.Structure):
    _fields_ = [("A", C.c_void_p), ("A2", C.c_void_p), ("B", C.c_void_p), ("B2", C.c_void_p), ("C", C.c_void_p),
                ("M", C.c_int32), ("N", C.c_int32), ("K", C.c_int32),
                ("lda", C.c_int32), ("lda2", C.c_int32), ("ldb", C.c_int32), ("ldb2", C.c_int32), ("ldc", C.c_int32),
                ("k_split", C.c_int32), ("conv", C.c_int32),
                ("H", C.c_int32), ("W", C.c_int32), ("Cin", C.c_int32),
                ("Ho", C.c_int32), ("Wo", C.c_int32), ("KH", C.c_int32), ("KW", C.c_int32), ("stride", C.c_int32),
                ("pad_t", C.c_int32), ("pad_l", C.c_int32), ("upsample", C.c_int32),
                ("alpha", C.c_float), ("bias", C.c_void_p), ("rowadd", C.c_void_p),
                ("rows_per_group", C.c_int32), ("ld_rowadd", C.c_int32),
                ("residual", C.c_void_p), ("ldr", C.c_int32),
                ("out_f32", C.c_int32), ("accumulate", C.c_int32),
                ("ws", C.c_void_p), ("ws_bytes", C.c_int64),
                ("tile_hint", C.c_int32), ("splitk_hint", C.c_int32)]


class AdamArgs(C.Structure):
    _fields_ = [("p", C.c_void_p), ("g", C.c_void_p), ("m", C.c_void_p), ("v", C.c_void_p), ("ema", C.c_void_p),
                ("n", C.c_int64), ("sumsq", C.c_void_p), ("max_norm", C.c_float),
                ("lr", C.c_float), ("beta1", C.c_float), ("beta2", C.c_float), ("eps", C.c_float),
                ("weight_decay", C.c_float), ("adamw", C.c_int32), ("step", C.c_int32), ("ema_decay", C.c_float)]


class JLArgs(C.Structure):
    _fields_ = [("A", C.c_void_p), ("lda", C.c_int64), ("G", C.c_int32), ("P", C.c_int64), ("p0", C.c_int64),
                ("d", C.c_int32), ("seed", C.c_uint32), ("model_id", C.c_uint32), ("type", C.c_int32),
                ("accumulate", C.c_int32), ("out", C.c_void_p), ("workspace", C.c_void_p), ("workspace_bytes", C.c_int64)]


class HGemmSegArgs(C.Structure):
    _fields_ = [("A", C.c_void_p), ("B", C.c_void_p), ("C", C.c_void_p), ("ws", C.c_void_p), ("ws_bytes", C.c_int64),
                ("c_seg_stride", C.c_int64), ("M", C.c_int32), ("N", C.c_int32), ("L", C.c_int32), ("S", C.c_int32),
                ("lda", C.c_int32), ("ldb", C.c_int32), ("ldc", C.c_int32), ("alpha", C.c_float), ("accumulate", C.c_int32),
                ("splitk_hint", C.c_int32)]


JL_NORMAL, JL_RADEMACHER = 0, 1
POOL_MAX, POOL_AVG, POOL_AVG_VALID = 0, 1, 2
GELU_ERF, GELU_QUICK = 0, 1
SIM_X_F32, SIM_X_U8 = 0, 1

GEMM_NO_PATCH, GEMM_TAP_MAJOR_K, GEMM_SCALAR_EPILOGUE, GEMM_GENERAL_LOADERS, GN_TWO_PASS = 1, 2, 4, 8, 1
GEMM_NO_WINO = 16
GEMM_WINO_WGRAD = 32
GEMM_WINO_ONLY_INPUT, GEMM_WINO_SKIP_INPUT = 64, 128
A_KC, A_MC, A_CONV, A_CONVT = 0, 1, 2, 3
B_KC, B_MC, B_WDGRAD, B_CONV = 0, 1, 2, 3

_vp, _i32, _i64, _f32, _f64 = C.c_void_p, C.c_int32, C.c_int64, C.c_float, C.c_double

SIGNATURES = {
    "gad_version": (C.c_int, []),
    "gad_last_error": (C.c_char_p, []),
    "gad_gemm_workspace_bytes": (_i64, [C.POINTER(GemmArgs)]),
    "gad_gemm": (C.c_int, [C.POINTER(GemmArgs), _vp]),
    "gad_gemm_uses_bf16": (C.c_int, [C.POINTER(GemmArgs)]),
    "gad_gemm_kernel_id": (C.c_int, [C.POINTER(GemmArgs)]),
    "gad_gemm_wino_bytes": (_i64, [C.POINTER(GemmArgs)]),
    "gad_wino_weights": (C.c_int, [_vp, _vp, _vp, _i64, _vp]),
    "gad_wino4_weights": (C.c_int, [_vp, _vp, _vp, _i64, _vp]),
    "gad_groupnorm_one_pass": (C.c_int, [C.POINTER(GroupNormArgs)]),
    "gad_gemm_plan": (C.c_int, [C.POINTER(GemmArgs), C.POINTER(_i32), C.POINTER(_i32), C.POINTER(_i32)]),
    "gad_groupnorm_workspace_bytes": (_i64, [C.POINTER(GroupNormArgs)]),
    "gad_groupnorm_silu_fwd": (C.c_int, [C.POINTER(GroupNormArgs), _vp]),
    "gad_groupnorm_silu_bwd": (C.c_int, [C.POINTER(GroupNormArgs), _vp]),
    "gad_groupnorm_wino4_ok": (C.c_int, [C.POINTER(GroupNormArgs), C.c_int32]),
    "gad_groupnorm_silu_wino4": (C.c_int, [C.POINTER(GroupNormArgs), _vp, C.c_int32, _vp]),
    "gad_attention_supported": (C.c_int, [_i32]),
    "gad_attention_uses_bf16": (C.c_int, [C.POINTER(AttentionArgs), _i32]),
    "gad_attention_bwd_workspace_bytes": (_i64, [C.POINTER(AttentionArgs)]),
    "gad_attention_fwd": (C.c_int, [C.POINTER(AttentionArgs), _vp]),
    "gad_attention_bwd": (C.c_int, [C.POINTER(AttentionArgs), _vp]),
    "gad_softmax_fwd": (C.c_int, [_vp, _vp, _i64, _i32, _f32, _vp]),
    "gad_softmax_bwd": (C.c_int, [_vp, _vp, _vp, _i64, _i32, _f32, _vp]),
    "gad_layernorm_workspace_bytes": (_i64, [_i64, _i32]),
    "gad_layernorm_fwd": (C.c_int, [_vp, _vp, _vp, _vp, _vp, _vp, _i64, _i32, _f32, _vp]),
    "gad_layernorm_bwd": (C.c_int, [_vp, _vp, _vp, _vp, _vp, _vp, _vp, _vp, _i64, _i32, _vp, _i64, _vp]),
    "gad_geglu_fwd": (C.c_int, [_vp, _vp, _i64, _i32, _vp]),
    "gad_geglu_bwd": (C.c_int, [_vp, _vp, _vp, _i64, _i32, _vp]),
    "gad_timestep_embedding": (C.c_int, [_vp, _vp, _i32, _i32, _i32, _f32, _f32, _vp]),
    "gad_rotate_conv3x3": (C.c_int, [_vp, _vp, _vp, _i32, _vp]),
    "gad_silu_fwd": (C.c_int, [_vp, _vp, _i64, _vp]),
    "gad_silu_bwd": (C.c_int, [_vp, _vp, _vp, _i64, _vp]),
    "gad_concat_channels": (C.c_int, [_vp, _vp, _vp, _i64, _i32, _i32, _vp]),
    "gad_split_channels": (C.c_int, [_vp, _vp, _vp, _i64, _i32, _i32, _vp]),
    "gad_nchw_to_nhwc": (C.c_int, [_vp, _vp, _i32, _i32, _i32, _vp]),
    "gad_nhwc_to_nchw": (C.c_int, [_vp, _vp, _i32, _i32, _i32, _vp]),
    "gad_upsample2x_bwd": (C.c_int, [_vp, _vp, _i32, _i32, _i32, _i32, _vp]),
    "gad_colsum": (C.c_int, [_vp, _vp, _i32, _i64, _i32, _vp, _i64, _vp]),
    "gad_add_noise": (C.c_int, [_vp, _vp, _vp, _vp, _vp, _i32, _i64, _vp]),
    "gad_ddim_step": (C.c_int, [_vp, _vp, _vp, _i64, _f32, _f32, _f32, _vp]),
    "gad_cfg_ddim_step": (C.c_int, [_vp, _vp, _vp, _i64, _f32, _f32, _f32, _f32, _vp]),
    "gad_to_image01": (C.c_int, [_vp, _vp, _i64, _vp]),
    "gad_mse_fwd_bwd": (C.c_int, [_vp, _vp, _vp, _vp, _i64, _f32, _vp, _i64, _vp]),
    "gad_sumsq": (C.c_int, [_vp, _vp, _i64, _vp, _i64, _vp]),
    "gad_clip_adam_ema": (C.c_int, [C.POINTER(AdamArgs), _vp]),
    "gad_ema_update": (C.c_int, [_vp, _vp, _i64, _f32, _vp]),
    "gad_hgemm_workspace_bytes": (_i64, [C.POINTER(HGemmArgs)]),
    "gad_hgemm_plan": (C.c_int, [C.POINTER(HGemmArgs), C.POINTER(_i32), C.POINTER(_i32)]),
    "gad_hgemm": (C.c_int, [C.POINTER(HGemmArgs), _vp]),
    "gad_hgemm_tn_workspace_bytes": (_i64, [C.POINTER(HGemmArgs)]),
    "gad_hgemm_tn": (C.c_int, [C.POINTER(HGemmArgs), _vp]),
    "gad_hgemm_tn_seg_workspace_bytes": (_i64, [C.POINTER(HGemmSegArgs)]),
    "gad_hgemm_tn_seg": (C.c_int, [C.POINTER(HGemmSegArgs), _vp]),
    "gad_h_transpose": (C.c_int, [_vp, _vp, _i32, _i32, _i32, _i32, _i32, _vp]),
    "gad_h_cast": (C.c_int, [_vp, _vp, _i64, _i32, _vp]),
    "gad_h_shadow_pairs": (C.c_int, [_vp, _vp, _vp, _vp, _i32, _vp]),
    "gad_h_add": (C.c_int, [_vp, _vp, _vp, _i64, _vp]),
    "gad_h_groupnorm_workspace_bytes": (_i64, [C.POINTER(GroupNormArgs)]),
    "gad_h_groupnorm_silu_fwd": (C.c_int, [C.POINTER(GroupNormArgs), _vp]),
    "gad_h_groupnorm_silu_bwd": (C.c_int, [C.POINTER(GroupNormArgs), _vp]),
    "gad_h_layernorm_fwd": (C.c_int, [_vp, _vp, _vp, _vp, _vp, _vp, _i64, _i32, _f32, _vp]),
    "gad_h_layernorm_bwd": (C.c_int, [_vp, _vp, _vp, _vp, _vp, _vp, _vp, _i64, _i32, _vp]),
    "gad_h_geglu_fwd": (C.c_int, [_vp, _vp, _i64, _i32, _vp]),
    "gad_h_geglu_bwd": (C.c_int, [_vp, _vp, _vp, _i64, _i32, _vp]),
    "gad_h_upsample2x_bwd": (C.c_int, [_vp, _vp, _i32, _i32, _i32, _i32, _vp]),
    "gad_h_attention_fwd": (C.c_int, [C.POINTER(AttentionArgs), _vp]),
    "gad_h_attention_bwd": (C.c_int, [C.POINTER(AttentionArgs), _vp]),
    "gad_jl_project_workspace_bytes": (_i64, [C.POINTER(JLArgs)]),
    "gad_jl_project": (C.c_int, [C.POINTER(JLArgs), _vp]),
    "gad_image_metrics_workspace_bytes": (_i64, [_i32, _i32, _i32, _i32, _i32]),
    "gad_image_metrics": (C.c_int, [_vp, _vp, _vp, _i32, _i32, _i32, _i32, _i32, _f64, _f64, _f64, _vp, _i64, _vp]),
    "gad_add_noise_bcast": (C.c_int, [_vp, _vp, _vp, _vp, _vp, _i32, _i32, _i32, _i32, _i32, _i32, _vp]),
    "gad_mse_segments_workspace_bytes": (_i64, [_i32, _i32, _i32, _i32]),
    "gad_mse_segments": (C.c_int, [_vp, _vp, _vp, _i32, _i32, _i32, _i32, _vp, _i64, _vp]),
    "gad_wf_dots_workspace_bytes": (_i64, [_i64]),
    "gad_wf_dots": (C.c_int, [_vp, _vp, _vp, _i64, _vp, _vp, _i64, _vp]),
    "gad_wf_update": (C.c_int, [_vp, _vp, _vp, _f64, _i64, _vp]),
    "gad_pool2d": (C.c_int, [_vp, _vp, _i32, _i32, _i32, _i32, _i32, _i32, _i32, _i32, _i32, _i32, _i32, _i32, _i32, _vp]),
    "gad_resize_bilinear": (C.c_int, [_vp, _vp, _i32, _i32, _i32, _i32, _i32, _i32, _f32, _f32, _vp]),
    "gad_relu": (C.c_int, [_vp, _i64, _i32, _i32, _vp]),
    "gad_manifold_radii_workspace_bytes": (_i64, [_i32, _i32, _i32, _i32]),
    "gad_manifold_radii": (C.c_int, [_vp, _i32, _i32, _i32, _i32, _vp, _vp, _i64, _vp]),
    "gad_manifold_cover_workspace_bytes": (_i64, [_i32, _i32, _i32, _i32, _i32]),
    "gad_manifold_cover": (C.c_int, [_vp, _i32, _i32, _vp, _i32, _i32, _i32, _vp, _vp, _vp, _i64, _vp]),
    "gad_resize_bicubic_patches_workspace_bytes": (_i64, [_i32, _i32, _i32, _i32, _i32, _i32, _i32, _i32]),
    "gad_resize_bicubic_patches": (C.c_int, [_vp, _vp, _i32, _i32, _i32, _i32, _i32, _i32, _i32, _i32, _i32, _f32, _f32, _vp, _i64, _vp]),
    "gad_bicubic_max_taps": (_i32, [_i32, _i32]),
    "gad_bicubic_taps": (C.c_int, [_i32, _i32, _i32, _i32, _vp, _vp, _vp]),
    "gad_vit_tokens": (C.c_int, [_vp, _vp, _vp, _vp, _vp, _vp, _i32, _i32, _i32, _f32, _vp]),
    "gad_gelu": (C.c_int, [_vp, _i64, _i32, _i32, _i32, _vp]),
    "gad_l2_normalize_rows": (C.c_int, [_vp, _i64, _i32, _i32, _vp]),
    "gad_cosine_rows_workspace_bytes": (_i64, [_i64, _i64, _i64, _i32, _i32]),
# ... 24 lines not shown
```

group-attribution-for-diffusion-models_amd/gad/ops.py:

```python
from __future__ import annotations

import ctypes as C
import math
from typing import Optional

import torch

from . import _capi
from ._capi import (A_CONV, A_CONVT, A_KC, A_MC, B_CONV, B_KC, B_MC, B_WDGRAD, AdamArgs, ConvGeom, GemmArgs,
                    GroupNormArgs, check)

_WS = {}
WS_BYTES = 1 << 30


def _stream():
    return C.c_void_p(torch.cuda.current_stream().cuda_stream)


_raw_stream = getattr(torch._C, "_cuda_getCurrentRawStream", None)


WS_OVERRIDE = [None]


def workspace(device) -> torch.Tensor:
    if WS_OVERRIDE[0] is not None:
        return WS_OVERRIDE[0]
    stream = _raw_stream(device.index if device.index is not None else torch.cuda.current_device()) if _raw_stream is not None \
        else torch.cuda.current_stream(device).cuda_stream
    key = (device.type, device.index, stream)
    ws = _WS.get(key)
    if ws is None:
        ws = torch.empty(WS_BYTES, dtype=torch.uint8, device=device)
        _WS[key] = ws
    return ws


def _ptr(t: Optional[torch.Tensor]):
    return None if t is None else t.data_ptr()


def _req(t: torch.Tensor, name: str):
    if not (t.is_cuda and t.dtype == torch.float32 and t.is_contiguous()):
        raise _capi.GadError(f"{name}: expected a contiguous fp32 device tensor, got {t.dtype} {t.device} "
                             f"contiguous={t.is_contiguous()}")
    return t


def weight_krsc(w: torch.Tensor) -> torch.Tensor:
    v = w.permute(0, 2, 3, 1)
    if not v.is_contiguous():
        raise _capi.GadError("conv weight storage must be [Cout,KH,KW,Cin] (channels_last)")
    return v


_SINK_EPOCH = [0]
_SINK_ACTIVE = [False]


def begin_backward_step():
    _SINK_EPOCH[0] += 1
    _SINK_ACTIVE[0] = True


def end_backward_step():
    _SINK_ACTIVE[0] = False


_PER_SAMPLE = [None]


def _sink(param):
    if _PER_SAMPLE[0] is not None and param is not None and param.requires_grad:
        raise _capi.GadError("per-sample gradient sink: only the LoRA matrices of the half-precision activation path have "
                             "per-sample gradients (csrc/half.hip: gad_hgemm_tn_seg)")
    v = getattr(param, "_gad_sink", None) if (param is not None and _SINK_ACTIVE[0]) else None
    if v is None:
        return None, True
    first = getattr(param, "_gad_sink_epoch", -1) != _SINK_EPOCH[0]
    param._gad_sink_epoch = _SINK_EPOCH[0]
    return v, first


def _deliver(param, grad):
    v, first = _sink(param)
    if v is None:
        return grad
    if first:
        v.copy_(grad)
    else:
        v.add_(grad)
    return None


OPERAND_PRECISION = [0]


class operand_precision:

    def __init__(self, name):
        if name not in ("f32", "fp32", "no", "bf16", "bf16-operands", "bf16-activations"):
            raise ValueError(f"operand precision {name!r}: use 'f32', 'bf16' (= 'bf16-activations') or 'bf16-operands'")
        self.value = {"bf16": 2, "bf16-activations": 2, "bf16-operands": 1}.get(name, 0)

    def __enter__(self):
        self.prev = OPERAND_PRECISION[0]
        OPERAND_PRECISION[0] = self.value
        return self

    def __exit__(self, *exc):
        OPERAND_PRECISION[0] = self.prev
        return False


def set_operand_precision(name):
    OPERAND_PRECISION[0] = 0 if name in (None, "no", "f32", "fp32") else operand_precision("bf16" if name in ("fp16", "bf16") else name).value


def half_activations() -> bool:
    return OPERAND_PRECISION[0] == 2


KERNEL_FLAGS = {"gemm": 0, "gn": 0, "native_dgrad": False, "two_kernel_attn_bwd": False, "narrow_attn_fwd": False, "no_wino4": False,
                "no_gn_wino": False}


class kernel_flags:

    def __init__(self, no_patch=False, tap_major_k=False, gn_two_pass=False, scalar_epilogue=False, general_loaders=False,
                 native_dgrad=False, two_kernel_attn_bwd=False, narrow_attn_fwd=False, no_wino=False, no_wino4=False, no_gn_wino=False):
        self.native_dgrad, self.two_kernel_attn_bwd, self.narrow_attn_fwd, self.no_wino4 = native_dgrad, two_kernel_attn_bwd, narrow_attn_fwd, no_wino4
        self.no_gn_wino = no_gn_wino
        self.gemm = ((_capi.GEMM_NO_PATCH if no_patch else 0) | (_capi.GEMM_TAP_MAJOR_K if tap_major_k else 0)
                     | (_capi.GEMM_NO_WINO if no_wino else 0)
                     | (_capi.GEMM_SCALAR_EPILOGUE if scalar_epilogue else 0)
                     | (_capi.GEMM_GENERAL_LOADERS if general_loaders else 0))
        self.gn = _capi.GN_TWO_PASS if gn_two_pass else 0

    def __enter__(self):
        self.prev = dict(KERNEL_FLAGS)
        KERNEL_FLAGS["gemm"], KERNEL_FLAGS["gn"], KERNEL_FLAGS["native_dgrad"] = self.gemm, self.gn, self.native_dgrad
        KERNEL_FLAGS["two_kernel_attn_bwd"], KERNEL_FLAGS["narrow_attn_fwd"] = self.two_kernel_attn_bwd, self.narrow_attn_fwd
        KERNEL_FLAGS["no_wino4"] = self.no_wino4
        KERNEL_FLAGS["no_gn_wino"] = self.no_gn_wino
        return self

    def __exit__(self, *exc):
        KERNEL_FLAGS.update(self.prev)
        return False


SCRATCH_ALLOC = None
OUT_ALLOC = None
OUT_ALLOC_DT = None


ROUTE_STATS = None


def _scratch(kind, nbytes, device):
    if SCRATCH_ALLOC is not None:
        return SCRATCH_ALLOC(kind, nbytes, device)
    return torch.empty(nbytes, dtype=torch.uint8, device=device)


def _out(shape, device):
    if OUT_ALLOC is not None:
        return OUT_ALLOC(tuple(shape), device)
    return torch.empty(tuple(shape), device=device, dtype=torch.float32)


def gemm_raw(A, B, Cout, a_mode, b_mode, M, N, K, lda, ldb, ldc, *, geom: Optional[ConvGeom] = None, alpha=1.0,
             bias=None, rowadd=None, rows_per_group=1, residual=None, ldr=0, batch=1, batch_inner=1,
             sA=(0, 0), sB=(0, 0), sC=(0, 0), tile_hint=0, splitk_hint=0, A2=None, a_split=0, B_bf16=None,
             A_k2=None, B_k2=None, k_split=0, B_wino=None, B_wino4=None, wino_wgrad=False, wino_input=None, force_f32=False,
             keep_v=None, wino_v=None):
    lib = _capi.load()
    ws = workspace(A.device)
    a = GemmArgs()
    a.A, a.B, a.C = A.data_ptr(), B.data_ptr(), Cout.data_ptr()
    a.a_mode, a.b_mode = a_mode, b_mode
    a.M, a.N, a.K = M, N, K
    a.lda, a.ldb, a.ldc = lda, ldb, ldc
    a.batch, a.batch_inner = batch, batch_inner
    a.strideA0, a.strideA1 = sA
    a.strideB0, a.strideB1 = sB
    a.strideC0, a.strideC1 = sC
    if geom is not None:
        a.g = geom
    a.alpha = alpha
    a.bias, a.rowadd, a.residual = _ptr(bias), _ptr(rowadd), _ptr(residual)
    a.rows_per_group = rows_per_group
    a.ld_rowadd = (rowadd.stride(0) if rowadd.ndim == 2 else rowadd.shape[-1]) if rowadd is not None else 0
    a.ldr = ldr
    a.ws, a.ws_bytes = ws.data_ptr(), ws.numel()
    a.tile_hint, a.splitk_hint = tile_hint, splitk_hint
    a.operand_precision = 1 if (OPERAND_PRECISION[0] and not force_f32) else 0
    a.flags = KERNEL_FLAGS["gemm"]
    if A2 is not None:
        a.A2, a.a_split, a.ldx2 = A2.data_ptr(), a_split, A2.shape[-1]
    if B_bf16 is not None:
        a.B_bf16 = B_bf16.data_ptr()
    if A_k2 is not None:
        a.A_k2, a.B_k2, a.k_split = A_k2.data_ptr(), B_k2.data_ptr(), k_split
        a.lda_k2, a.ldb_k2 = A_k2.shape[-1], B_k2.shape[-1]
    if B_wino is not None or B_wino4 is not None:
        a.B_wino, a.B_wino4 = _ptr(B_wino), _ptr(B_wino4)
        need = lib.gad_gemm_wino_bytes(C.byref(a))
        if need:
            V = _scratch("wino", need, A.device)
            a.wino_ws, a.wino_ws_bytes = V.data_ptr(), need
            if keep_v is not None and a.B_wino4 and lib.gad_gemm_kernel_id(C.byref(a)) == 6:
                keep_v.append(V)
        else:
            a.B_wino = a.B_wino4 = None
    if wino_wgrad:
        a.flags |= _capi.GEMM_WINO_WGRAD
        need = lib.gad_gemm_wino_bytes(C.byref(a))
        if need:
            V = _scratch("wino", need, A.device)
            a.wino_ws, a.wino_ws_bytes = V.data_ptr(), need
            if wino_v is not None and wino_v.numel() >= 36 * (K // 16) * geom.C * 4:
                a.B_wino4 = wino_v.data_ptr()
                a.flags |= _capi.GEMM_WINO_SKIP_INPUT
        else:
            a.flags &= ~_capi.GEMM_WINO_WGRAD
    if wino_input is not None:
        if lib.gad_gemm_kernel_id(C.byref(a)) != 6 or not a.wino_ws:
            return False
        wino_input(V)
        a.flags |= _capi.GEMM_WINO_SKIP_INPUT
    if ROUTE_STATS is not None and (a.B_wino4 or a.flags & _capi.GEMM_WINO_WGRAD):
        key = (lib.gad_gemm_kernel_id(C.byref(a)), M, N, K, bool(a.flags & _capi.GEMM_WINO_SKIP_INPUT), torch.is_grad_enabled())
        ROUTE_STATS[key] = ROUTE_STATS.get(key, 0) + 1
    if SCRATCH_ALLOC is not None:
        need = lib.gad_gemm_workspace_bytes(C.byref(a))
        ws = _scratch("ws", need, A.device) if need else None
        a.ws, a.ws_bytes = (ws.data_ptr() if need else None), need
    if PROFILER is not None:
        PROFILER.gemm(lib, a, batch)
        return True
    check(lib.gad_gemm(C.byref(a), _stream()), "gad_gemm")
    return True


class GemmProfiler:
    NAMES = {(A_CONV, B_KC): "conv_fwd", (A_CONVT, B_WDGRAD): "conv_dgrad", (A_MC, B_CONV): "conv_wgrad",
             (A_KC, B_KC): "gemm_nt", (A_KC, B_MC): "gemm_nn", (A_MC, B_MC): "gemm_tn"}

    def __init__(self):
        self.records = []

    def gemm(self, lib, a, batch):
        tile, sk, vec = C.c_int32(), C.c_int32(), C.c_int32()
        check(lib.gad_gemm_plan(C.byref(a), C.byref(tile), C.byref(sk), C.byref(vec)), "gad_gemm_plan")
        kid = lib.gad_gemm_kernel_id(C.byref(a))
        s, e, mid = torch.cuda.Event(enable_timing=True), torch.cuda.Event(enable_timing=True), None
        s.record()
        if kid in (5, 6) and not (a.flags & _capi.GEMM_WINO_SKIP_INPUT):
            flags = a.flags
            mid = torch.cuda.Event(enable_timing=True)
            a.flags = flags | _capi.GEMM_WINO_ONLY_INPUT
            check(lib.gad_gemm(C.byref(a), _stream()), "gad_gemm")
            mid.record()
            a.flags = flags | _capi.GEMM_WINO_SKIP_INPUT
            check(lib.gad_gemm(C.byref(a), _stream()), "gad_gemm")
            a.flags = flags
        else:
            check(lib.gad_gemm(C.byref(a), _stream()), "gad_gemm")
        e.record()
        name = self.NAMES.get((a.a_mode, a.b_mode), "gemm") + ("", "_bf16", f"_patch_w{a.g.Wo}", f"_patch_bf16_w{a.g.Wo}", f"_fewout_valu_w{a.g.Wo}", "_wino", "_wino4", "_wino4")[kid]
        key = (name, tile.value, sk.value, vec.value)
        g = a.g
        if a.a_mode in (A_CONV, A_CONVT):
            a_elems = (a.M // max(1, g.Ho * g.Wo)) * g.H * g.W * g.C
        else:
            a_elems = a.M * a.K
        b_elems = (a.K // max(1, g.Ho * g.Wo)) * g.H * g.W * g.C if a.b_mode == B_CONV else a.N * a.K
        extra = a.M * a.N if a.residual else 0
        nbytes = 4.0 * max(1, batch) * (a_elems + b_elems + a.M * a.N + extra)
        flops = 2.0 * a.M * a.N * a.K * max(1, batch)
        executed = flops * ({5: 16.0 / 36.0, 6: 0.25, 7: 0.25}.get(kid, 1.0))
        stage = None
        if kid in (5, 6):
            npos, tpx = (16, 4) if kid == 5 else (36, 16)
            v_bytes = 4.0 * npos * (a.M // tpx) * g.C
            stage = (mid, 4.0 * a_elems + v_bytes if mid is not None else 0.0, v_bytes + 4.0 * (b_elems * npos / 9.0 + a.M * a.N + extra))
        self.records.append((key, flops, nbytes, s, e, executed, stage))

    def hgemm(self, lib, a, tn=False):
        s, e = torch.cuda.Event(enable_timing=True), torch.cuda.Event(enable_timing=True)
        if tn:
            s.record()
            check(lib.gad_hgemm_tn(C.byref(a), _stream()), "gad_hgemm_tn")
            e.record()
            nbytes = 2.0 * a.K * (a.M + a.N) + 4.0 * a.M * a.N
            flops = 2.0 * a.M * a.N * a.K
            self.records.append((("hgemm_tn_wgrad", 128, 0, 8), flops, nbytes, s, e, flops, None))
            return
        tile, sk = C.c_int32(), C.c_int32()
        check(lib.gad_hgemm_plan(C.byref(a), C.byref(tile), C.byref(sk)), "gad_hgemm_plan")
        s.record()
        check(lib.gad_hgemm(C.byref(a), _stream()), "gad_hgemm")
        e.record()
        if a.conv:
            name = f"hconv{a.KH}x{a.KW}" + ("_s2dgrad" if a.conv == 2 else "_s2" if a.stride == 2 else "_up" if a.upsample else "")
            a_elems = (a.M // max(1, a.Ho * a.Wo)) * a.H * a.W * a.Cin
        else:
            name = "hgemm_wgrad" if a.out_f32 else "hgemm_lora" if a.A2 else "hgemm"
            a_elems = a.M * a.K
        nbytes = 2.0 * (a_elems + a.N * a.K + (a.M * a.N if a.residual else 0)) + (4.0 if a.out_f32 else 2.0) * a.M * a.N
        flops = 2.0 * a.M * a.N * a.K
        self.records.append(((name, {1: 128, 2: 320, 5: 256320, 6: 256320, 7: 320, 8: 128, 9: 128}[tile.value], sk.value, 8), flops, nbytes, s, e, flops, None))

    def attention(self, fn, a, what, elem_bytes=4):
        s, e = torch.cuda.Event(enable_timing=True), torch.cuda.Event(enable_timing=True)
        s.record()
        check(fn(C.byref(a), _stream()), f"gad_attention_{what}")
        e.record()
        d_alg = getattr(a, "alg_d", a.d)
        unit = float(a.B) * a.heads * a.Tq * a.Tk * d_alg
        qb, kb = float(elem_bytes) * a.B * a.Tq * a.heads * d_alg, float(elem_bytes) * a.B * a.Tk * a.heads * d_alg
        flops, nbytes = (4.0 * unit, 2 * qb + 2 * kb) if what == "fwd" else (10.0 * unit, 4 * qb + 4 * kb)
        self.records.append(((f"attn_{what}_d{d_alg}", a.Tq, a.Tk, elem_bytes), flops, nbytes, s, e, flops, None))

    def summary(self):
        out = {}
        for key, fl, nb, s, e, ex, stage in self.records:
            d = out.setdefault(key, dict(launches=0, ms=0.0, flops=0.0, bytes=0.0, executed=0.0))
            d["launches"] += 1
            d["ms"] += s.elapsed_time(e)
            d["flops"] += fl
            d["bytes"] += nb
            d["executed"] += ex
            if stage is not None:
                d["bytes_rest"] = d.get("bytes_rest", 0.0) + stage[2]
                d.setdefault("ms_input", 0.0)
                d.setdefault("bytes_input", 0.0)
                d.setdefault("n_input", 0)
                if stage[0] is not None:
                    d["ms_input"] += s.elapsed_time(stage[0])
                    d["bytes_input"] += stage[1]
                    d["n_input"] += 1
        return out


PROFILER = None


def _conv_out_size(h, k, stride, pad_lo, pad_hi):
    return (h + pad_lo + pad_hi - k) // stride + 1


def conv2d_fwd_raw(x, w, bias, stride=1, pad=(1, 1, 1, 1), upsample=False, rowadd=None, residual=None,
                   tile_hint=0, splitk_hint=0, x2=None, wino_input=None, keep_v=None):
    _req(x, "conv x")
    Bn, H, W, C1 = x.shape
    Cin = C1
    if x2 is not None:
        _req(x2, "conv x2")
        if x2.shape[:3] != x.shape[:3]:
            raise _capi.GadError(f"conv x2 {tuple(x2.shape)} does not match x {tuple(x.shape)}")
        Cin = C1 + x2.shape[-1]
    wk = weight_krsc(w)
    Cout, KH, KW, wc = wk.shape
    if wc != Cin:
        raise _capi.GadError(f"conv weight expects {wc} input channels, got {Cin}")
    He, We = (2 * H, 2 * W) if upsample else (H, W)
    Ho = _conv_out_size(He, KH, stride, pad[0], pad[1])
    Wo = _conv_out_size(We, KW, stride, pad[2], pad[3])
    y = _out((Bn, Ho, Wo, Cout), x.device)
    g = ConvGeom(H, W, Cin, C1, Ho, Wo, KH, KW, stride, pad[0], pad[2], int(upsample))
    if residual is not None:
        _req(residual, "conv residual")
    wino_ok = (KH == 3 and KW == 3 and stride == 1 and x2 is None and tile_hint in (0, 7, 8, 9, 10, 11) and splitk_hint == 0
               and tuple(pad) == (1, 1, 1, 1))
    f4_maps = Ho % 4 == 0 and Wo % 4 == 0 and not KERNEL_FLAGS.get("no_wino4")
    launched = gemm_raw(x, wk, y, A_CONV, B_KC, Bn * Ho * Wo, Cout, KH * KW * Cin, 0, KH * KW * Cin, Cout, geom=g,
             bias=bias, rowadd=rowadd, rows_per_group=Ho * Wo, residual=residual, ldr=Cout,
             tile_hint=tile_hint, splitk_hint=splitk_hint, A2=x2, a_split=C1, wino_input=wino_input, keep_v=keep_v,
             B_wino=wino_weight(w, 2) if (wino_ok and (tile_hint == 7 or (tile_hint == 0 and not f4_maps))) else None,
             B_wino4=wino_weight(w, 4) if (wino_ok and tile_hint != 7 and f4_maps) else None,
             B_bf16=bf16_weight(w) if (OPERAND_PRECISION[0] >= 1 and KH == 3 and Cin % 32 == 0 and x2 is None
                                       and not torch.cuda.is_current_stream_capturing()) else None)
    return y if launched is not False else None


def gn_silu_conv3x3_raw(x, x2, gamma, beta, G, eps, w, bias, rowadd=None, residual=None, tile_hint=0):
    _req(x, "groupnorm x")
    Bn, H, W, C1 = x.shape
    Cin = C1 + (x2.shape[-1] if x2 is not None else 0)
    lib = _capi.load()

    def plain():
        h = group_norm_cat_raw(x, x2, gamma, beta, G, eps, True) if x2 is not None else group_norm(x, gamma, beta, G, eps, True)
        return conv2d_fwd_raw(h, w, bias, 1, (1, 1, 1, 1), False, rowadd=rowadd, residual=residual, tile_hint=tile_hint)
    if (torch.is_grad_enabled() or tuple(w.shape[2:]) != (3, 3) or w.shape[1] != Cin or OPERAND_PRECISION[0] != 0 or KERNEL_FLAGS["gn"]
            or KERNEL_FLAGS.get("no_gn_wino") or H % 4 or W % 4):
        return plain()
    mean = torch.empty((Bn, G), device=x.device, dtype=torch.float32)
    rstd = torch.empty_like(mean)
    a = GroupNormArgs()
    a.x, a.gamma, a.beta, a.mean, a.rstd = x.data_ptr(), gamma.data_ptr(), beta.data_ptr(), mean.data_ptr(), rstd.data_ptr()
    a.B, a.HW, a.C, a.G, a.eps, a.silu = Bn, H * W, Cin, G, eps, 1
    if x2 is not None:
        _req(x2, "groupnorm x2")
        a.x2, a.C1 = x2.data_ptr(), C1
    if not lib.gad_groupnorm_wino4_ok(C.byref(a), W):
        return plain()

    def fill(V):
        check(lib.gad_groupnorm_silu_wino4(C.byref(a), V.data_ptr(), W, _stream()), "gad_groupnorm_silu_wino4")
    y = conv2d_fwd_raw(_ShapeOnly(x, (Bn, H, W, Cin)), w, bias, 1, (1, 1, 1, 1), False, rowadd=rowadd, residual=residual,
                       tile_hint=tile_hint, wino_input=fill)
    return y if y is not None else plain()


class _ShapeOnly:

    def __init__(self, t, shape):
        self._t, self.shape, self.device, self.dtype = t, tuple(shape), t.device, t.dtype
        self.is_cuda = t.is_cuda

    def data_ptr(self):
        return self._t.data_ptr()

    def is_contiguous(self):
        return True


def bf16_weight(w):
    home = getattr(w, "_gad_flat", None)
    if home is not None and w.data_ptr() == home[0].data_ptr() + 4 * home[1]:
        flat, off, n = home
        key = (flat._version, WEIGHT_EPOCH[0], getattr(flat, "_gad_epoch", 0))
        cached = getattr(flat, "_gad_bf16", None)
        if cached is None or cached[0] != key:
            shadow = cached[1] if cached is not None else torch.empty(flat.numel(), device=flat.device, dtype=torch.bfloat16)
            shadow.copy_(flat.detach())
            cached = (key, shadow, {o_: p_._version for p_, o_, _ in getattr(flat, "_gad_params", ())})
            flat._gad_bf16 = cached
        if cached[2].get(off, w._version) != w._version:
            cached[1][off:off + n].copy_(flat.detach()[off:off + n])
            cached[2][off] = w._version
        o, i, kh, kw = w.shape
        return cached[1][off:off + n].view(o, kh, kw, i)
    key = weight_key(w)
    cached = getattr(w, "_gad_bf16", None)
    if cached is None or cached[0] != key:
        cached = (key, weight_krsc(w).detach().to(torch.bfloat16).contiguous())
        w._gad_bf16 = cached
    return cached[1]


def _in_flat_buffer(w) -> bool:
    home = getattr(w, "_gad_flat", None)
    return home is not None and w.data_ptr() == home[0].data_ptr() + 4 * home[1]


def dgrad_as_forward(w, stride, pad) -> bool:
    return (tuple(w.shape[2:]) == (3, 3) and stride == 1 and tuple(pad) == (1, 1, 1, 1) and w.shape[0] % 32 == 0
            and w.shape[1] >= 64 and (not w.requires_grad or _in_flat_buffer(w)) and not KERNEL_FLAGS.get("native_dgrad"))


def _rot_table(flat):
    cached = getattr(flat, "_gad_rot_table", None)
    if cached is None:
# ... 49 lines not shown

def _wino_ok(co, ci):
    return ci % 32 == 0 and co % 4 == 0 and co >= 64


def _wino_transform(src, items, npos):
    rows, where, doff = [], {}, 0
    for off, co, ci in items:
        where[off] = (doff, npos * co * ci)
        rows += [(off, doff, co, ci, a, b) for a in range(0, co, 32) for b in range(0, ci, 32)]
        doff += npos * co * ci
    U = torch.empty(max(doff, 1), device=src.device, dtype=torch.float32)
    table = torch.tensor(rows, dtype=torch.int64, device=src.device)
    return U, where, table, len(rows)


def wino_weight(w, f=2):
    co, ci = w.shape[0], w.shape[1]
    if (tuple(w.shape[2:]) != (3, 3) or not _wino_ok(co, ci) or OPERAND_PRECISION[0] >= 1
            or KERNEL_FLAGS["gemm"] & (_capi.GEMM_NO_WINO | _capi.GEMM_NO_PATCH | _capi.GEMM_SCALAR_EPILOGUE | _capi.GEMM_TAP_MAJOR_K)
            or (f == 4 and KERNEL_FLAGS.get("no_wino4"))):
        return None
    lib = _capi.load()
    launch, npos, attr = (lib.gad_wino_weights, 16, "_gad_wino") if f == 2 else (lib.gad_wino4_weights, 36, "_gad_wino4")
    if _in_flat_buffer(w):
        flat, off, n = w._gad_flat
        key = (flat._version, WEIGHT_EPOCH[0], getattr(flat, "_gad_epoch", 0))
        cached = getattr(flat, attr, None)
        if cached is None:
            items = [(o_, a, b) for o_, a, b in _conv3x3_residents(flat) if _wino_ok(a, b)]
            cached = [None, *_wino_transform(flat, items, npos), {}]
            setattr(flat, attr, cached)
        _, U, where, table, tiles, versions = cached
        if off not in where:
            return None
        stale = cached[0] != key or versions.get(off, w._version) != w._version
        if stale:
            check(launch(flat.data_ptr(), U.data_ptr(), table.data_ptr(), tiles, _stream()), "gad_wino_weights")
            cached[0] = key
            cached[5] = {o_: p_._version for p_, o_, _ in getattr(flat, "_gad_params", ())}
        d0, dn = where[off]
        return U[d0:d0 + dn]
    key = weight_key(w)
    cached = getattr(w, attr, None)
    if cached is None or cached[0] != key:
        src = weight_krsc(w).detach()
        if cached is None:
            U, _, table, tiles = _wino_transform(src, [(0, co, ci)], npos)
        else:
            U, table, tiles = cached[1], cached[2], cached[3]
        check(launch(src.data_ptr(), U.data_ptr(), table.data_ptr(), tiles, _stream()), "gad_wino_weights")
        cached = (key, U, table, tiles)
        setattr(w, attr, cached)
    return cached[1]


def refresh_wino(module):
    for p in module.parameters():
        if p.ndim == 4 and tuple(p.shape[2:]) == (3, 3):
            home = p._gad_flat[0] if _in_flat_buffer(p) else p
            for f, attr in ((2, "_gad_wino"), (4, "_gad_wino4")):
                if getattr(home, attr, None) is not None:
                    wino_weight(p, f)


def two_source_ok(c1: int, c2: int) -> bool:
    return c1 % 32 == 0 and c2 % 32 == 0


def conv2d_dgrad_raw(dy, w, x_shape, stride=1, pad=(1, 1, 1, 1), upsample=False, tile_hint=0, splitk_hint=0):
    _req(dy, "conv dy")
    Bn, H, W, Cin = x_shape
    wk = weight_krsc(w)
    Cout, KH, KW, _ = wk.shape
    _, Ho, Wo, _ = dy.shape
    He, We = (2 * H, 2 * W) if upsample else (H, W)
    dxe = _out((Bn, He, We, Cin), dy.device)
    if (KH == 1 and KW == 1 and stride == 1 and tuple(pad) == (0, 0, 0, 0) and not upsample and Cin % 4 == 0 and Cout % 4 == 0
            and not KERNEL_FLAGS["gemm"] & _capi.GEMM_GENERAL_LOADERS):
        gemm_raw(dy, wk, dxe, A_KC, B_MC, Bn * H * W, Cin, Cout, Cout, Cin, Cin, tile_hint=tile_hint, splitk_hint=splitk_hint)
        return dxe
    g = ConvGeom(Ho, Wo, Cout, Cout, He, We, KH, KW, stride, pad[0], pad[2], 0)
    gemm_raw(dy, wk, dxe, A_CONVT, B_WDGRAD, Bn * He * We, Cin, KH * KW * Cout, 0, 0, Cin, geom=g,
             tile_hint=tile_hint, splitk_hint=splitk_hint)
    return _upsample2x_bwd(dxe, x_shape) if upsample else dxe


def _upsample2x_bwd(dxe, x_shape):
    Bn, H, W, Cin = x_shape
    dx = torch.empty((Bn, H, W, Cin), device=dxe.device, dtype=torch.float32)
    check(_capi.load().gad_upsample2x_bwd(dxe.data_ptr(), dx.data_ptr(), Bn, H, W, Cin, _stream()), "gad_upsample2x_bwd")
    return dx


def conv2d_wgrad_raw(dy, x, w_like, stride=1, pad=(1, 1, 1, 1), upsample=False, tile_hint=0, splitk_hint=0, out=None, wino_v=None):
    _req(dy, "conv dy")
    _req(x, "conv x")
    Bn, H, W, Cin = x.shape
    Cout, _, KH, KW = w_like.shape
    _, Ho, Wo, _ = dy.shape
    dwk = _out((Cout, KH, KW, Cin), dy.device) if out is None else weight_krsc(out)
    if (KH == 1 and KW == 1 and stride == 1 and tuple(pad) == (0, 0, 0, 0) and not upsample and Cin % 4 == 0 and Cout % 4 == 0
            and not KERNEL_FLAGS["gemm"] & _capi.GEMM_GENERAL_LOADERS):
        gemm_raw(dy, x, dwk, A_MC, B_MC, Cout, Cin, Bn * H * W, Cout, Cin, Cin, tile_hint=tile_hint, splitk_hint=splitk_hint)
        return dwk.permute(0, 3, 1, 2)
    g = ConvGeom(H, W, Cin, Cin, Ho, Wo, KH, KW, stride, pad[0], pad[2], int(upsample))
    wino = (KH == 3 and KW == 3 and stride == 1 and tuple(pad) == (1, 1, 1, 1) and tile_hint in (0, 8) and splitk_hint == 0
            and Ho % 4 == 0 and Wo % 4 == 0 and OPERAND_PRECISION[0] == 0 and not KERNEL_FLAGS.get("no_wino4")
            and not KERNEL_FLAGS["gemm"] & (_capi.GEMM_NO_WINO | _capi.GEMM_NO_PATCH | _capi.GEMM_SCALAR_EPILOGUE | _capi.GEMM_TAP_MAJOR_K
                                            | _capi.GEMM_GENERAL_LOADERS))
    gemm_raw(dy, x, dwk, A_MC, B_CONV, Cout, KH * KW * Cin, Bn * Ho * Wo, Cout, 0, KH * KW * Cin, geom=g,
             tile_hint=tile_hint, splitk_hint=splitk_hint, wino_wgrad=wino, wino_v=wino_v)
    return dwk.permute(0, 3, 1, 2)


def colsum_raw(dy2d: torch.Tensor, segments=1, out=None):
    lib = _capi.load()
    ws = workspace(dy2d.device)
    rows, N = dy2d.shape
    if out is None:
        out = torch.empty((segments, N), device=dy2d.device, dtype=torch.float32)
    check(lib.gad_colsum(dy2d.data_ptr(), out.data_ptr(), segments, rows // segments, N, ws.data_ptr(), ws.numel(),
                         _stream()), "gad_colsum")
    return out


def linear_fwd_raw(x2d, w, bias=None, residual=None, alpha=1.0, force_f32=False):
    M, K = x2d.shape
    N = w.shape[0]
    y = _out((M, N), x2d.device)
    gemm_raw(x2d, w, y, A_KC, B_KC, M, N, K, K, K, N, bias=bias, residual=residual, ldr=N, alpha=alpha, force_f32=force_f32)
    return y


def conv_krsc_raw(x, w_krsc, bias, kh, kw, stride, pad_h, pad_w, out=None, c0=0):
    Bn, H, W, ci = x.shape
    co = w_krsc.shape[0]
    Ho, Wo = (H + 2 * pad_h - kh) // stride + 1, (W + 2 * pad_w - kw) // stride + 1
    if out is None:
        out = torch.empty((Bn, Ho, Wo, co), device=x.device, dtype=torch.float32)
    gemm_raw(x, w_krsc, out[..., c0:c0 + co], A_CONV, B_KC, Bn * Ho * Wo, co, kh * kw * ci, 0, kh * kw * ci, out.shape[-1],
             geom=ConvGeom(H, W, ci, ci, Ho, Wo, kh, kw, stride, pad_h, pad_w, 0), bias=bias, force_f32=True)
    return out


def relu_raw(t):
    Cn = t.shape[-1]
    check(_capi.load().gad_relu(t.data_ptr(), t.numel() // Cn, Cn, Cn, _stream()), "gad_relu")
    return t


def pool2d_raw(x, out, c0, k, stride, pad, mode, relu_in=False):
    Bn, H, W, Cn = x.shape
    check(_capi.load().gad_pool2d(x.data_ptr(), out[..., c0:].data_ptr(), Bn, H, W, Cn, Cn, out.shape[-1], out.shape[1],
                                  out.shape[2], k, stride, pad, mode, int(relu_in), _stream()), "gad_pool2d")
    return out


def resize_bilinear_raw(x_nchw, R, a, b):
    Bn, Cn, H, W = x_nchw.shape
    y = torch.empty((Bn, R, R, Cn), device=x_nchw.device, dtype=torch.float32)
    check(_capi.load().gad_resize_bilinear(x_nchw.data_ptr(), y.data_ptr(), Bn, Cn, H, W, R, R, a, b, _stream()),
          "gad_resize_bilinear")
    return y


def gelu_raw(h, kind):
    check(_capi.load().gad_gelu(h.data_ptr(), h.shape[0], h.shape[1], h.shape[1], kind, _stream()), "gad_gelu")
    return h


def l2_normalize_rows_raw(x2d):
    _req(x2d, "l2_normalize input")
    check(_capi.load().gad_l2_normalize_rows(x2d.data_ptr(), x2d.shape[0], x2d.shape[1], x2d.shape[1], _stream()),
          "gad_l2_normalize_rows")
    return x2d


def layernorm_fwd_raw(x, gamma, beta, eps):
    C_ = x.shape[-1]
    rows = x.numel() // C_
    y = torch.empty_like(x)
    stats = torch.empty((2, rows), device=x.device, dtype=torch.float32)
    check(_capi.load().gad_layernorm_fwd(x.data_ptr(), y.data_ptr(), gamma.data_ptr(), beta.data_ptr(), stats[0].data_ptr(),
                                         stats[1].data_ptr(), rows, C_, eps, _stream()), "gad_layernorm_fwd")
    return y, stats[0], stats[1]


def linear_dgrad_raw(dy2d, w):
    M, N = dy2d.shape
    K = w.shape[1]
    dx = _out((M, K), dy2d.device)
    gemm_raw(dy2d, w, dx, A_KC, B_MC, M, K, N, N, K, K)
    return dx


def linear_wgrad_raw(dy2d, x2d, out=None):
    M, N = dy2d.shape
    K = x2d.shape[1]
    dw = _out((N, K), dy2d.device) if out is None else out
    gemm_raw(dy2d, x2d, dw, A_MC, B_MC, N, K, M, N, K, K)
    return dw


def _param_grad(param, compute):
    v, first = _sink(param)
    if v is None:
        return compute(None)
    if first:
        compute(v)
    else:
        v.add_(compute(None))
    return None


def _conv_backward(ctx, dy, x, x_shape, w, stride, pad, upsample, has, need):
    dy = dy.contiguous()
    dx = None
    if need[0]:
        if dgrad_as_forward(w, stride, pad):
            dx = conv2d_fwd_raw(dy, rotated_weight(w), None)
            if upsample:
                dx = _upsample2x_bwd(dx, x_shape)
        else:
            dx = conv2d_dgrad_raw(dy, w, x_shape, stride, pad, upsample)
    V, ctx.wino_v = ctx.wino_v, None
    dw = _param_grad(w, lambda o: conv2d_wgrad_raw(dy, x, w, stride, pad, upsample, out=o, wino_v=V)) if need[1] else None
    db, dr = _conv_epilogue_grads(dy, ctx.bias_ref, has[0] and need[2], has[1] and need[3])
    dres = dy if (has[2] and need[4]) else None
    return dx, dw, db, dr, dres


class Conv2dFn(torch.autograd.Function):

    @staticmethod
    def forward(ctx, x, w, bias, rowadd, residual, stride, pad, upsample):
        ctx.save_for_backward(x, w)
        ctx.bias_ref = bias
        ctx.cfg = (stride, pad, upsample, (bias is not None, rowadd is not None, residual is not None))
        keep = [] if ctx.needs_input_grad[1] else None
        y = conv2d_fwd_raw(x, w, bias, stride, pad, upsample, rowadd, residual, keep_v=keep)
        ctx.wino_v = keep[0] if keep else None
        return y

    @staticmethod
    def backward(ctx, dy):
        x, w = ctx.saved_tensors
        stride, pad, upsample, has = ctx.cfg
        return (*_conv_backward(ctx, dy, x, x.shape, w, stride, pad, upsample, has, ctx.needs_input_grad[:5]), None, None, None)


def _conv_epilogue_grads(dy, bias, need_bias, need_rowadd):
    Bn, Ho, Wo, Cout = dy.shape
    db = dr = None
    if need_rowadd:
        dr = colsum_raw(dy.view(Bn * Ho * Wo, Cout), segments=Bn)
        if need_bias:
            db = _param_grad(bias, lambda o: colsum_raw(dr, 1, out=o).view(Cout))
    elif need_bias:
        db = _param_grad(bias, lambda o: colsum_raw(dy.view(Bn * Ho * Wo, Cout), 1, out=o).view(Cout))
    return db, dr


class GnSiluConv3x3Fn(torch.autograd.Function):

    @staticmethod
    def forward(ctx, x, gamma, beta, w, bias, rowadd, residual, G, eps, bypass):
        _req(x, "groupnorm x")
        Bn = x.shape[0]
        mean = torch.empty((Bn, G), device=x.device, dtype=torch.float32)
        rstd = torch.empty_like(mean)
        keep = [] if ctx.needs_input_grad[3] else None
        h = torch.empty_like(x)
        check(_capi.load().gad_groupnorm_silu_fwd(C.byref(_gn_args(x, h, gamma, beta, mean, rstd, G, eps, True)), _stream()),
              "gad_groupnorm_silu_fwd")
        y = conv2d_fwd_raw(h, w, bias, 1, (1, 1, 1, 1), False, rowadd=rowadd, residual=residual, keep_v=keep)
        ctx.save_for_backward(x, gamma, beta, mean, rstd, w, h if keep is not None else None)
        ctx.wino_v = keep[0] if keep else None
        ctx.bias_ref = bias
        ctx.cfg = (G, eps, (bias is not None, rowadd is not None, residual is not None))
        return (y, x.view_as(x)) if bypass else y

    @staticmethod
    def backward(ctx, dy, dbypass=None):
        x, gamma, beta, mean, rstd, w, h = ctx.saved_tensors
        G, eps, has = ctx.cfg
        need = ctx.needs_input_grad
        if dy is None:
            return (dbypass, *([None] * 9))
        dh, dw, db, dr, dres = _conv_backward(ctx, dy, h, x.shape, w, 1, (1, 1, 1, 1), False, has,
                                              (need[0] or need[1] or need[2], *need[3:7]))
        dx = dgamma = dbeta = None
        if dh is not None:
            dx, dgamma, dbeta = _gn_backward(x, gamma, beta, mean, rstd, G, eps, True, dh, dbypass, need[1] or need[2])
        elif dbypass is not None:
            dx = dbypass
        return dx, dgamma, dbeta, dw, db, dr, dres, None, None, None


def gn_silu_conv3x3(x, gamma, beta, G, eps, w, bias, rowadd=None, residual=None, bypass=False):
    if x.dtype == torch.bfloat16 or tuple(w.shape[2:]) != (3, 3) or w.shape[1] != x.shape[-1] or x.ndim != 4:
        if bypass:
            h, x = group_norm_bypass(x, gamma, beta, G, eps, True)
        else:
            h = group_norm(x, gamma, beta, G, eps, True)
        y = conv2d(h, w, bias, rowadd, residual)
        return (y, x) if bypass else y
    if bypass and not (torch.is_grad_enabled() and x.requires_grad):
        return GnSiluConv3x3Fn.apply(x, gamma, beta, w, bias, rowadd, residual, G, eps, False), x
    return GnSiluConv3x3Fn.apply(x, gamma, beta, w, bias, rowadd, residual, G, eps, bypass)


def _half():
    from . import half
    return half


def conv2d(x, w, bias=None, rowadd=None, residual=None, stride=1, pad=(1, 1, 1, 1), upsample=False):
    if x.dtype == torch.bfloat16:
        return _half().conv2d(x, w, bias, rowadd, residual, stride, pad, upsample)
    return Conv2dFn.apply(x, w, bias, rowadd, residual, stride, pad, upsample)


class LinearFn(torch.autograd.Function):
    @staticmethod
    def forward(ctx, x, w, bias, residual):
        shp = x.shape
        x2 = _req(x, "linear x").view(-1, shp[-1])
        ctx.save_for_backward(x2, w)
        ctx.shp = shp
        ctx.bias_ref = bias
        ctx.flags = (bias is not None, residual is not None)
        r2 = residual.view(-1, w.shape[0]) if residual is not None else None
        return linear_fwd_raw(x2, w, bias, r2).view(*shp[:-1], w.shape[0])

    @staticmethod
    def backward(ctx, dy):
        x2, w = ctx.saved_tensors
        dy2 = dy.contiguous().view(-1, w.shape[0])
        dx = linear_dgrad_raw(dy2, w).view(ctx.shp) if ctx.needs_input_grad[0] else None
        dw = _param_grad(w, lambda o: linear_wgrad_raw(dy2, x2, out=o)) if ctx.needs_input_grad[1] else None
        db = _param_grad(ctx.bias_ref, lambda o: colsum_raw(dy2, 1, out=o).view(-1)) \
            if (ctx.flags[0] and ctx.needs_input_grad[2]) else None
# ... 718 lines not shown
```

include/gad.h:

```cpp
#ifndef GAD_H
#define GAD_H
#include <stdint.h>
#ifdef __cplusplus
extern "C" {
#endif

int gad_version(void);
const char* gad_last_error(void);

enum gad_a_mode {
  GAD_A_KC = 0,
  GAD_A_MC = 1,
  GAD_A_CONV = 2,
  GAD_A_CONVT = 3
};
enum gad_b_mode {
  GAD_B_KC = 0,
  GAD_B_MC = 1,
  GAD_B_WDGRAD = 2,
  GAD_B_CONV = 3
};

typedef struct gad_conv_geom {
  int32_t H, W, C;
  int32_t ldx;
  int32_t Ho, Wo;
  int32_t KH, KW;
  int32_t stride;
  int32_t pad_t, pad_l;
  int32_t upsample;
} gad_conv_geom;

typedef struct gad_gemm_args {
  const float* A;
  const float* B;
  float* C;
  int32_t a_mode, b_mode;
  int32_t M, N, K;
  int32_t lda, ldb, ldc;
  int32_t batch, batch_inner;
  int64_t strideA0, strideA1, strideB0, strideB1, strideC0, strideC1;
  gad_conv_geom g;
  float alpha;
  const float* bias;
  const float* rowadd;
  int32_t rows_per_group, ld_rowadd;
  const float* residual;
  int32_t ldr;
  void* ws;
  int64_t ws_bytes;
  int32_t tile_hint;
  int32_t splitk_hint;
  int32_t operand_precision;
  const float* A2;
  int32_t a_split, ldx2;
  const void* B_bf16;
  const float* A_k2;
  const float* B_k2;
  int32_t lda_k2, ldb_k2, k_split;
  int32_t flags;
  const float* B_wino;
  void* wino_ws;
  int64_t wino_ws_bytes;
  const float* B_wino4;
} gad_gemm_args;
enum gad_gemm_flags {
  GAD_GEMM_NO_WINO = 16,
  GAD_GEMM_WINO_WGRAD = 32,
  GAD_GEMM_NO_PATCH = 1,
  GAD_GEMM_TAP_MAJOR_K = 2,
  GAD_GEMM_SCALAR_EPILOGUE = 4,
  GAD_GEMM_GENERAL_LOADERS = 8,
  GAD_GEMM_WINO_ONLY_INPUT = 64,
  GAD_GEMM_WINO_SKIP_INPUT = 128
};

int64_t gad_gemm_workspace_bytes(const gad_gemm_args* a);
int gad_gemm_plan(const gad_gemm_args* a, int32_t* tile, int32_t* splitk, int32_t* vec);
int gad_gemm(const gad_gemm_args* a, void* stream);
int gad_gemm_uses_bf16(const gad_gemm_args* a);
int gad_gemm_kernel_id(const gad_gemm_args* a);
int64_t gad_gemm_wino_bytes(const gad_gemm_args* a);
int gad_wino_weights(const float* src, float* dst, const int64_t* table, int64_t n_tiles, void* stream);
int gad_wino4_weights(const float* src, float* dst, const int64_t* table, int64_t n_tiles, void* stream);

typedef struct gad_groupnorm_args {
  const float* x;
  float* y;
  const float* gamma;
  const float* beta;
  float* mean;
  float* rstd;
  const float* dy;
  float* dgamma;
  float* dbeta;
  int32_t B, HW, C, G;
  float eps;
  int32_t silu;
  void* ws;
  int64_t ws_bytes;
  const float* x2;
  int32_t C1;
  int32_t flags;
  const float* dx_add;
} gad_groupnorm_args;
enum gad_groupnorm_flags { GAD_GN_TWO_PASS = 1 };

int64_t gad_groupnorm_workspace_bytes(const gad_groupnorm_args* a);
int gad_groupnorm_one_pass(const gad_groupnorm_args* a);
int gad_groupnorm_silu_fwd(const gad_groupnorm_args* a, void* stream);
int gad_groupnorm_silu_bwd(const gad_groupnorm_args* a, void* stream);
int gad_groupnorm_wino4_ok(const gad_groupnorm_args* a, int32_t W);
int gad_groupnorm_silu_wino4(const gad_groupnorm_args* a, float* V, int32_t W, void* stream);

typedef struct gad_attention_args {
  const float* q; const float* k; const float* v;
  float* o;
  float* lse;
  const float* d_o;
  float* delta;
  float* dq; float* dk; float* dv;
  int32_t B, heads, Tq, Tk, d;
  int32_t ldq, ldk, ldv, ldo, ld_do, ld_dq, ld_dk, ld_dv;
  int64_t stride_q, stride_k, stride_v, stride_o, stride_do, stride_dq, stride_dk, stride_dv;
  float scale;
  int32_t operand_precision;
  void* ws;
  int64_t ws_bytes;
  int32_t flags;
} gad_attention_args;
#define GAD_ATTN_TWO_KERNEL_BWD 1
#define GAD_ATTN_NARROW_FWD 2
int64_t gad_attention_bwd_workspace_bytes(const gad_attention_args* a);
int gad_attention_supported(int32_t d);
int gad_attention_uses_bf16(const gad_attention_args* a, int32_t backward);
int gad_attention_fwd(const gad_attention_args* a, void* stream);
int gad_attention_bwd(const gad_attention_args* a, void* stream);

int gad_softmax_fwd(const float* s, float* p, int64_t rows, int32_t n, float scale, void* stream);
int gad_softmax_bwd(const float* p, const float* dp, float* ds, int64_t rows, int32_t n, float scale,
                    void* stream);

int64_t gad_layernorm_workspace_bytes(int64_t rows, int32_t C);
int gad_layernorm_fwd(const float* x, float* y, const float* gamma, const float* beta, float* mean, float* rstd,
                      int64_t rows, int32_t C, float eps, void* stream);
int gad_layernorm_bwd(const float* x, const float* dy, float* dx, const float* dx_add, const float* gamma, const float* mean,
                      const float* rstd, float* dgamma_dbeta, int64_t rows, int32_t C, void* ws, int64_t ws_bytes,
                      void* stream);
int gad_geglu_fwd(const float* h, float* out, int64_t M, int32_t F, void* stream);
int gad_geglu_bwd(const float* h, const float* dout, float* dh, int64_t M, int32_t F, void* stream);

int gad_timestep_embedding(const int64_t* t, float* out, int32_t B, int32_t dim, int32_t flip_sin_to_cos,
                           float freq_shift, float max_period, void* stream);
int gad_silu_fwd(const float* x, float* y, int64_t n, void* stream);
int gad_silu_bwd(const float* x, const float* dy, float* dx, int64_t n, void* stream);
int gad_rotate_conv3x3(const float* src, float* dst, const int64_t* table, int32_t n_tiles, void* stream);
int gad_concat_channels(const float* a, const float* b, float* out, int64_t pixels, int32_t C1, int32_t C2,
                        void* stream);
int gad_split_channels(const float* d, float* da, float* db, int64_t pixels, int32_t C1, int32_t C2,
                       void* stream);
int gad_nchw_to_nhwc(const float* x, float* y, int32_t B, int32_t C, int32_t HW, void* stream);
int gad_nhwc_to_nchw(const float* x, float* y, int32_t B, int32_t C, int32_t HW, void* stream);
int gad_upsample2x_bwd(const float* dy, float* dx, int32_t B, int32_t H, int32_t W, int32_t C, void* stream);
int gad_colsum(const float* dy, float* out, int32_t S, int64_t M, int32_t N, void* ws, int64_t ws_bytes,
               void* stream);

int gad_add_noise(const float* x0, const float* eps, const int64_t* t, const float* alphas_cumprod,
// ... 154 lines not shown
```

Measured before the change: 45.86 coalitions/hour.

## Add stride-2 parity-class dgrad and shared Winograd dy transforms in conv backward

Stride-2 transposed-conv dgrad GEMMs are split into four output parity classes. Each class only iterates over the kernel taps that actually contribute, which removes the structurally zero taps from the K loop. Conv backward also gains a fused kernel that reads dy once and writes both the Winograd input transform for dgrad and the transform for wgrad, plus per-tile sums used for the bias and rowadd gradients. This removes a redundant pass over dy and the separate colsum reads, at the cost of more kernel variants, extra scratch buffers and probe calls on the host.

New measurement: 46.30 coalitions/hour (median of 6 runs). Within noise of the previous version (+1.0%).

```diff
diff --git a/group-attribution-for-diffusion-models_amd/csrc/gemm_dev.h b/group-attribution-for-diffusion-models_amd/csrc/gemm_dev.h
--- a/group-attribution-for-diffusion-models_amd/csrc/gemm_dev.h
+++ b/group-attribution-for-diffusion-models_amd/csrc/gemm_dev.h
@@ -51,6 +51,11 @@
   float* ws;
   int tiles_m, tiles_n, splitk, ktiles_per_split;
   int epi_vec;
+  int s2_tile0[5];
+  int s2_rows[4];
+  int s2_n[2][2];
+  int s2_o0[2][2];
+  FastDiv s2_fd_hw[4], s2_fd_w[2];
 };
 
 __device__ __forceinline__ f32x4 ldg4(const float* p) { return *reinterpret_cast<const f32x4*>(p); }
diff --git a/group-attribution-for-diffusion-models_amd/csrc/gemm_f32.hip b/group-attribution-for-diffusion-models_amd/csrc/gemm_f32.hip
--- a/group-attribution-for-diffusion-models_amd/csrc/gemm_f32.hip
+++ b/group-attribution-for-diffusion-models_amd/csrc/gemm_f32.hip
@@ -259,7 +259,7 @@
   int kend, hlim, wlim;
   int k, c, r, s;
   bool kok;
-  __device__ void init(const float* x_, const DevArgs& p, int row0, int nrows, int kend_) {
+  __device__ __forceinline__ void init_source(const float* x_, const DevArgs& p, int kend_) {
     x = x_;
     x2 = p.A2;
     csplit = p.a_split;
@@ -271,6 +271,9 @@
     hlim = g.upsample ? 2 * g.H : g.H;
     wlim = g.upsample ? 2 * g.W : g.W;
     rowmask = 0;
+  }
+  __device__ void init(const float* x_, const DevArgs& p, int row0, int nrows, int kend_) {
+    init_source(x_, p, kend_);
 #pragma unroll
     for (int i = 0; i < S::NS; ++i) {
       int m = row0 + S::row(i);
@@ -488,6 +491,61 @@
   __device__ void setup(const DevArgs& p, const float* a, int row0, int kend) { this->init(a, p, row0, p.M, kend); }
 };
 
+struct RowsAsIs {
+  __device__ __forceinline__ bool ok(const DevArgs& p, int m) const { return m < p.M; }
+  __device__ __forceinline__ int operator()(int m) const { return m; }
+};
+__host__ __device__ __forceinline__ int s2_first(int parity, int pad) { return (parity + pad) & 1; }
+__host__ __device__ __forceinline__ int s2_count(int n, int first) { return n > first ? (n - first + 1) / 2 : 0; }
+struct RowsS2P {
+  int rows, hw, nw, oh0, ow0, HoWo, Wo;
+  FastDiv fd_hw, fd_w;
+  __device__ __forceinline__ RowsS2P(const DevArgs& p, int cls) {
+    const int ph = cls >> 1, pw = cls & 1;
+    rows = p.s2_rows[cls];
+    nw = p.s2_n[1][pw];
+    hw = p.s2_n[0][ph] * nw;
+    oh0 = p.s2_o0[0][ph];
+    ow0 = p.s2_o0[1][pw];
+    HoWo = p.g.Ho * p.g.Wo;
+    Wo = p.g.Wo;
+    fd_hw = p.s2_fd_hw[cls];
+    fd_w = p.s2_fd_w[pw];
+  }
+  __device__ __forceinline__ bool ok(const DevArgs&, int m) const { return m < rows; }
+  __device__ __forceinline__ void pixel(int m, int& img, int& oh, int& ow) const {
+    img = fd_hw.div(m);
+    const int rem = m - img * hw, i = fd_w.div(rem);
+    oh = oh0 + 2 * i;
+    ow = ow0 + 2 * (rem - i * nw);
+  }
+  __device__ __forceinline__ int operator()(int m) const {
+    int img, oh, ow;
+    pixel(m, img, oh, ow);
+    return img * HoWo + oh * Wo + ow;
+  }
+};
+constexpr int A_CONVT_S2P = 27;
+template <int ROWS, int VEC>
+struct ALoader<A_CONVT_S2P, ROWS, VEC> : LoadConvRows<ROWS, true, VEC> {
+  static constexpr bool KC = true;
+  using S = KCSlots<ROWS>;
+  __device__ void setup(const DevArgs& p, const float* a, const RowsS2P& rm, int row0, int kend) {
+    this->init_source(a, p, kend);
+#pragma unroll
+    for (int i = 0; i < S::NS; ++i) {
+      const int m = row0 + S::row(i);
+      const bool ok = m < rm.rows;
+      int img, oh, ow;
+      rm.pixel(ok ? m : 0, img, oh, ow);
+      this->boff[i] = img * this->g.H * this->g.W;
+      this->rowmask |= (unsigned)ok << i;
+      this->bh[i] = oh + this->g.pad_t;
+      this->bw[i] = ow + this->g.pad_l;
+    }
+  }
+};
+
 constexpr int A_KC2 = 17;
 template <int ROWS, int VEC>
 struct ALoader<A_KC2, ROWS, VEC> : LoadKCDense2<ROWS> {
@@ -579,10 +637,10 @@
 };
 
 
-template <int TM, int TN, int BM, int BN, int WM = 2, int WN = 2>
+template <int TM, int TN, int BM, int BN, int WM = 2, int WN = 2, class RM = RowsAsIs>
 __device__ __forceinline__ void store_block(const DevArgs& p, const f32x16 (&acc)[TM][TN], int row0, int col0, int wm, int wn,
                                             int h, int l31, float* C, int ldc, const float* R, bool direct,
-                                            float* scratch = nullptr) {
+                                            float* scratch = nullptr, const RM rm = RM()) {
   if (scratch != nullptr && p.epi_vec) {
     const int lane = l31 + 32 * h;
     const int rr = lane >> 3, c4 = (lane & 7) * 4;
@@ -603,8 +661,9 @@
         for (int q = 0; q < 4; ++q) {
           const int r = rr + 8 * q;
           f32x4 v = *reinterpret_cast<const f32x4*>(scratch + r * EPI_LD + c4);
-          const int m = row0 + wm * (BM / WM) + i * 32 + r;
-          if (m >= p.M || !n_ok) continue;
+          const int mt = row0 + wm * (BM / WM) + i * 32 + r;
+          if (!rm.ok(p, mt) || !n_ok) continue;
+          const int m = rm(mt);
           if (direct) {
             v = f32x4{__builtin_fmaf(v[0], p.alpha, b0), __builtin_fmaf(v[1], p.alpha, b1), __builtin_fmaf(v[2], p.alpha, b2),
                       __builtin_fmaf(v[3], p.alpha, b3)};
@@ -626,8 +685,9 @@
     for (int i = 0; i < TM; ++i) {
 #pragma unroll
       for (int e = 0; e < 16; ++e) {
-        int m = row0 + wm * (BM / WM) + i * 32 + (e & 3) + 8 * (e >> 2) + 4 * h;
-        if (m >= p.M) continue;
+        const int mt = row0 + wm * (BM / WM) + i * 32 + (e & 3) + 8 * (e >> 2) + 4 * h;
+        if (!rm.ok(p, mt)) continue;
+        const int m = rm(mt);
         float v = acc[i][j][e];
         if (direct) {
           v = __builtin_fmaf(v, p.alpha, bias);
@@ -663,8 +723,23 @@
   int kbeg = split * p.ktiles_per_split * BK;
   int kend = min(p.K, kbeg + p.ktiles_per_split * BK);
   int nkt = (kend - kbeg + BK - 1) / BK;
+  constexpr bool S2P = AM == A_CONVT_S2P;
+  const int cls = S2P ? (tile_m >= p.s2_tile0[1]) + (tile_m >= p.s2_tile0[2]) + (tile_m >= p.s2_tile0[3]) : 0;
+  const int tap_bits = S2P ? 2 - (cls >> 1) - (cls & 1) : 0;
+  const int chunks = p.g.C / BK;
+  if (S2P) {
+    row0 = (tile_m - p.s2_tile0[cls]) * BM;
+    nkt = chunks << tap_bits;
+  }
   const int kt0 = split * p.ktiles_per_split;
   auto k0_of = [&](int kt) -> int {
+    if (S2P) {
+      const int ti = p.kperm ? kt & ((1 << tap_bits) - 1) : kt / chunks;
+      const int chunk = p.kperm ? kt >> tap_bits : kt - ti * chunks;
+      const int ph = cls >> 1, pw = cls & 1;
+      const int r = ph ? 1 : 2 * (pw ? ti : ti >> 1), s = pw ? 1 : 2 * (ti & 1);
+      return (r * p.g.KW + s) * p.g.C + chunk * BK;
+    }
     if (!p.kperm) return (kt0 + kt) * BK;
     int j = kt0 + kt;
     int chunk = p.fdTaps.div(j), tap = j - chunk * p.taps;
@@ -674,7 +749,8 @@
 
   AL al;
   BL bl;
-  al.setup(p, A, row0, kend);
+  if constexpr (S2P) al.setup(p, A, RowsS2P(p, cls), row0, kend);
+  else al.setup(p, A, row0, kend);
   bl.setup(p, B, col0, kend);
 
   const int tid = threadIdx.x, wave = tid >> 6, lane = tid & 63;
@@ -760,7 +836,10 @@
   float* C = direct ? p.C + z0 * p.sC0 + z1 * p.sC1 : p.ws + (long)zs * p.M * p.N;
   const float* R = (direct && p.residual) ? p.residual + z0 * p.sC0 + z1 * p.sC1 : nullptr;
   const int ldc = direct ? p.ldc : p.N;
-  store_block<TM, TN, BM, BN>(p, acc, row0, col0, wm, wn, h, l31, C, ldc, R, direct, lds + (tid >> 6) * EPI_WAVE);
+  if constexpr (S2P)
+    store_block<TM, TN, BM, BN, 2, 2, RowsS2P>(p, acc, row0, col0, wm, wn, h, l31, C, ldc, R, direct, lds + (tid >> 6) * EPI_WAVE, RowsS2P(p, cls));
+  else
+    store_block<TM, TN, BM, BN>(p, acc, row0, col0, wm, wn, h, l31, C, ldc, R, direct, lds + (tid >> 6) * EPI_WAVE);
 }
 
 typedef __bf16 bf16x4_t __attribute__((ext_vector_type(4)));
@@ -2006,6 +2085,16 @@
   }
 }
 
+__device__ __forceinline__ void wino4_amul(const f32x4 (&d)[4], f32x4 (&t)[6]) {
+  const f32x4 s02 = d[0] + d[2], s13 = d[1] + d[3], a = d[0] + 4.f * d[2], b = 2.f * d[1] + 8.f * d[3];
+  t[0] = d[0];
+  t[1] = s02 + s13;
+  t[2] = s02 - s13;
+  t[3] = a + b;
+  t[4] = a - b;
+  t[5] = d[3];
+}
+
 __global__ __launch_bounds__(256) void wino4_dy_kernel(const WinoIn p) {
   const int C4 = p.C >> 2;
   const long idx = (long)blockIdx.x * 256 + threadIdx.x;
@@ -2017,22 +2106,13 @@
   const int r = (int)(tile - (long)n * per);
   const int ty = r / p.TW, tx = r - ty * p.TW;
   const float* img = p.x + ((long)n * p.H * p.W + (long)(4 * ty) * p.W + 4 * tx) * p.ldx + c;
-  auto amul = [](const f32x4 (&d)[4], f32x4 (&t)[6]) {
-    const f32x4 s02 = d[0] + d[2], s13 = d[1] + d[3], a = d[0] + 4.f * d[2], b = 2.f * d[1] + 8.f * d[3];
-    t[0] = d[0];
-    t[1] = s02 + s13;
-    t[2] = s02 - s13;
-    t[3] = a + b;
-    t[4] = a - b;
-    t[5] = d[3];
-  };
   f32x4 t[6][4];
 #pragma unroll
   for (int dx = 0; dx < 4; ++dx) {
     f32x4 d[4], col[6];
 #pragma unroll
     for (int dy = 0; dy < 4; ++dy) d[dy] = ldg4(img + ((long)dy * p.W + dx) * p.ldx);
-    amul(d, col);
+    wino4_amul(d, col);
 #pragma unroll
     for (int i = 0; i < 6; ++i) t[i][dx] = col[i];
   }
@@ -2041,7 +2121,86 @@
 #pragma unroll
   for (int i = 0; i < 6; ++i) {
     f32x4 v[6];
-    amul(t[i], v);
+    wino4_amul(t[i], v);
+#pragma unroll
+    for (int j = 0; j < 6; ++j) *reinterpret_cast<f32x4*>(out + (long)(6 * i + j) * pos_stride) = v[j];
+  }
+}
+
+struct WinoDy2 {
+  const float* dy;
+  float* V;
+  float* Wy;
+  float* tilesum;
+  int H, W, C, ldx;
+  int TH, TW;
+  long T;
+};
+
+__global__ __launch_bounds__(256) void wino4_dy2_kernel(const WinoDy2 p) {
+  const int C4 = p.C >> 2;
+  const long idx = (long)blockIdx.x * 256 + threadIdx.x;
+  if (idx >= p.T * C4) return;
+  const long tile = idx / C4;
+  const int c = (int)(idx - tile * C4) * 4;
+  const int per = p.TH * p.TW;
+  const int n = (int)(tile / per);
+  const int r = (int)(tile - (long)n * per);
+  const int ty = r / p.TW, tx = r - ty * p.TW;
+  const float* img = p.dy + (long)n * p.H * p.W * p.ldx + c;
+  f32x4 t[6][6];
+#pragma unroll
+  for (int dx = 0; dx < 6; ++dx) {
+    const int xx = 4 * tx - 1 + dx;
+    const bool xok = xx >= 0 && xx < p.W;
+    f32x4 d[6], col[6];
+#pragma unroll
+    for (int dy = 0; dy < 6; ++dy) {
+      const int yy = 4 * ty - 1 + dy;
+      const bool ok = xok && yy >= 0 && yy < p.H;
+      d[dy] = ok ? ldg4(img + ((long)yy * p.W + xx) * p.ldx) : zero4();
+    }
+    wino4_bt(d, col);
+#pragma unroll
+    for (int i = 0; i < 6; ++i) t[i][dx] = col[i];
+  }
+  const long pos_stride = p.T * p.C;
+  {
+    float* out = p.V + tile * p.C + c;
+#pragma unroll
+    for (int i = 0; i < 6; ++i) {
+      f32x4 v[6];
+      wino4_bt(t[i], v);
+#pragma unroll
+      for (int j = 0; j < 6; ++j) *reinterpret_cast<f32x4*>(out + (long)(6 * i + j) * pos_stride) = v[j];
+    }
+  }
+  const float* inner = img + ((long)(4 * ty) * p.W + 4 * tx) * p.ldx;
+  asm volatile("" : "+v"(inner));
+  f32x4 in[4][4];
+#pragma unroll
+  for (int dx = 0; dx < 4; ++dx)
+#pragma unroll
+    for (int dy = 0; dy < 4; ++dy) in[dx][dy] = ldg4(inner + ((long)dy * p.W + dx) * p.ldx);
+  if (p.tilesum) {
+    f32x4 s[4];
+#pragma unroll
+    for (int dx = 0; dx < 4; ++dx) s[dx] = (in[dx][0] + in[dx][1]) + (in[dx][2] + in[dx][3]);
+    *reinterpret_cast<f32x4*>(p.tilesum + tile * p.C + c) = (s[0] + s[1]) + (s[2] + s[3]);
+  }
+  f32x4 u[6][4];
+#pragma unroll
+  for (int dx = 0; dx < 4; ++dx) {
+    f32x4 col[6];
+    wino4_amul(in[dx], col);
+#pragma unroll
+    for (int i = 0; i < 6; ++i) u[i][dx] = col[i];
+  }
+  float* out = p.Wy + tile * p.C + c;
+#pragma unroll
+  for (int i = 0; i < 6; ++i) {
+    f32x4 v[6];
+    wino4_amul(u[i], v);
 #pragma unroll
     for (int j = 0; j < 6; ++j) *reinterpret_cast<f32x4*>(out + (long)(6 * i + j) * pos_stride) = v[j];
   }
@@ -2549,6 +2708,32 @@
   return sub;
 }
 
+struct S2Classes {
+  int tile0[5];
+  long rows[4];
+  int n[2][2], o0[2][2];
+};
+static S2Classes s2_classes(const gad_conv_geom& g, long images, int bm) {
+  S2Classes c{};
+  for (int par = 0; par < 2; ++par) {
+    c.o0[0][par] = s2_first(par, g.pad_t);
+    c.o0[1][par] = s2_first(par, g.pad_l);
+    c.n[0][par] = s2_count(g.Ho, c.o0[0][par]);
+    c.n[1][par] = s2_count(g.Wo, c.o0[1][par]);
+  }
+  for (int q = 0; q < 4; ++q) {
+    c.rows[q] = images * c.n[0][q >> 1] * c.n[1][q & 1];
+    c.tile0[q + 1] = c.tile0[q] + (int)gad_ceil_div(c.rows[q], bm);
+  }
+  return c;
+}
+static bool use_s2_parity(const gad_gemm_args* a) {
+  const gad_conv_geom& g = a->g;
+  return (a->flags & GAD_GEMM_S2_PARITY) && a->a_mode == GAD_A_CONVT && a->b_mode == GAD_B_WDGRAD && a->operand_precision == 0 &&
+         g.KH == 3 && g.KW == 3 && g.stride == 2 && !g.upsample && g.C % BK == 0 && pick_vec(a) == 4 && a->batch <= 1 &&
+         a->tile_hint == 0 && a->splitk_hint <= 0 && a->M % (g.Ho * g.Wo) == 0;
+}
+
 enum class RouteKind { ENGINE, PATCH_F32, PATCH_BF16, FEWOUT, WGRAD_PATCH, WINO, WINO_WGRAD, SPLIT_N, SPLIT_M };
 struct Route {
   RouteKind kind;
@@ -2561,6 +2746,8 @@
   WinoWgradPlan wq;
   int wbm, wsplits;
   int split;
+  bool s2p;
+  S2Classes s2;
 };
 
 static Route route_of(const gad_gemm_args* args) {
@@ -2584,6 +2771,15 @@
   else {
     r.kind = RouteKind::ENGINE;
     r.plan = make_plan(a);
+    if ((r.s2p = use_s2_parity(a))) {
+      r.s2 = s2_classes(a->g, a->M / (a->g.Ho * a->g.Wo), r.plan.bm);
+      r.plan.bn = r.plan.bm;
+      r.plan.tiles_m = r.s2.tile0[4];
+      r.plan.tiles_n = (int)gad_ceil_div(a->N, r.plan.bn);
+      r.plan.splitk = 1;
+      r.plan.ktiles_per_split = (int)gad_ceil_div(a->K, BK);
+      r.plan.nblocks = (long)r.plan.tiles_m * r.plan.tiles_n;
+    }
   }
   return r;
 }
@@ -2657,6 +2853,26 @@
 
 extern "C" int gad_gemm_uses_bf16(const gad_gemm_args* a) { return a && route_of(a).bf16 ? 1 : 0; }
 
+extern "C" int gad_gemm_s2_parity(const gad_gemm_args* a) {
+  if (!a) return 0;
+  const Route r = route_of(a);
+  return r.kind == RouteKind::ENGINE && r.s2p ? 1 : 0;
+}
+
+extern "C" int64_t gad_s2_parity_rows(const gad_conv_geom* g, int32_t images, int32_t q) {
+  if (!g || images <= 0 || q < 0 || q > 3 || g->Ho <= 0 || g->Wo <= 0) return -1;
+  return s2_classes(*g, images, 128).rows[q];
+}
+
+extern "C" int64_t gad_s2_parity_pixel(const gad_conv_geom* g, int32_t images, int32_t q, int64_t i) {
+  if (!g || images <= 0 || q < 0 || q > 3 || g->Ho <= 0 || g->Wo <= 0) return -1;
+  const S2Classes c = s2_classes(*g, images, 128);
+  if (i < 0 || i >= c.rows[q]) return -1;
+  const long nw = c.n[1][q & 1], hw = c.n[0][q >> 1] * nw;
+  const long img = i / hw, rem = i - img * hw, ih = rem / nw;
+  return img * g->Ho * g->Wo + (c.o0[0][q >> 1] + 2 * ih) * g->Wo + c.o0[1][q & 1] + 2 * (rem - ih * nw);
+}
+
 extern "C" int gad_gemm_kernel_id(const gad_gemm_args* a) { return a ? report(route_of(a)).kid : -1; }
 
 extern "C" int gad_gemm_plan(const gad_gemm_args* a, int32_t* tile, int32_t* splitk, int32_t* vec) {
@@ -2689,6 +2905,24 @@
   GAD_CHECK(src && dst && table && n_tiles > 0 && n_tiles < (1L << 31), "gad_wino4_weights: bad arguments");
   hipLaunchKernelGGL(wino4_weights_kernel, dim3((unsigned)n_tiles), dim3(256), 0, (hipStream_t)stream, src, dst, (const long*)table);
   GAD_LAUNCH_CHECK("gad_wino4_weights");
+  return 0;
+}
+
+extern "C" int gad_wino4_dy_transforms(const gad_wino4_dy_args* a, void* stream) {
+  GAD_CHECK(a && a->dy && a->V && a->Wy, "gad_wino4_dy_transforms: null pointer");
+  GAD_CHECK(a->B > 0 && a->H > 0 && a->W > 0 && a->C > 0 && a->H % 4 == 0 && a->W % 4 == 0 && a->C % 4 == 0 && a->ldx % 4 == 0 && a->ldx >= a->C,
+            "gad_wino4_dy_transforms: bad shape B=%d H=%d W=%d C=%d ldx=%d (maps and channels in multiples of 4)", a->B, a->H, a->W, a->C, a->ldx);
+  GAD_CHECK(gad_aligned16(a->dy) && gad_aligned16(a->V) && gad_aligned16(a->Wy) && (!a->tilesum || gad_aligned16(a->tilesum)),
+            "gad_wino4_dy_transforms: dy, V, Wy and tilesum must be 16-byte aligned");
+  GAD_CHECK((long)a->H * a->W * a->ldx < (1L << 31) && (long)a->B * a->H * a->W < (1L << 31), "gad_wino4_dy_transforms: image too large");
+  WinoDy2 p;
+  p.dy = a->dy; p.V = a->V; p.Wy = a->Wy; p.tilesum = a->tilesum;
+  p.H = a->H; p.W = a->W; p.C = a->C; p.ldx = a->ldx;
+  p.TH = a->H / 4; p.TW = a->W / 4; p.T = (long)a->B * p.TH * p.TW;
+  const long items = p.T * (a->C / 4);
+  GAD_CHECK(gad_ceil_div(items, 256) < (1L << 31), "gad_wino4_dy_transforms: grid too large");
+  hipLaunchKernelGGL(wino4_dy2_kernel, dim3((unsigned)gad_ceil_div(items, 256)), dim3(256), 0, (hipStream_t)stream, p);
+  GAD_LAUNCH_CHECK("gad_wino4_dy_transforms");
   return 0;
 }
 
@@ -2756,11 +2990,13 @@
             "gad_gemm: GAD_GEMM_WINO_ONLY_INPUT on a launch that takes no Winograd forward route (kernel id %d)", report(r).kid);
   GAD_CHECK(!skip_input || r.kind == RouteKind::WINO || r.kind == RouteKind::WINO_WGRAD,
             "gad_gemm: GAD_GEMM_WINO_SKIP_INPUT on a launch that takes no Winograd route (kernel id %d)", report(r).kid);
+  GAD_CHECK(!(r.a.flags & GAD_GEMM_WINO_SKIP_DY) || r.kind == RouteKind::WINO_WGRAD,
+            "gad_gemm: GAD_GEMM_WINO_SKIP_DY on a launch that takes no Winograd weight-gradient route (kernel id %d)", report(r).kid);
   return 0;
 }
 
 static DevArgs dev_args(const gad_gemm_args* a) {
-  DevArgs d;
+  DevArgs d{};
   d.A = a->A; d.B = a->B; d.C = a->C;
   d.A2 = a->A2; d.a_split = a->a_split; d.ldx2 = a->ldx2;
   d.Ak2 = a->A_k2; d.Bk2 = a->B_k2; d.lda2 = a->lda_k2; d.ldb2 = a->ldb_k2; d.k_split = a->k_split;
@@ -2817,7 +3053,7 @@
   wi.TH = wy.TH; wi.TW = wy.TW; wi.T = wq.T;
   const long iy = wq.T * (a->M / 4), ix = wq.T * (g.C / 4);
   GAD_CHECK(gad_ceil_div(iy, 256) < (1L << 31) && gad_ceil_div(ix, 256) < (1L << 31), "gad_gemm: Winograd transform grid too large");
-  hipLaunchKernelGGL(wino4_dy_kernel, dim3((unsigned)gad_ceil_div(iy, 256)), dim3(256), 0, st, wy);
+  if (!(a->flags & GAD_GEMM_WINO_SKIP_DY)) hipLaunchKernelGGL(wino4_dy_kernel, dim3((unsigned)gad_ceil_div(iy, 256)), dim3(256), 0, st, wy);
   if (!have_v) hipLaunchKernelGGL(wino4_input_kernel, dim3((unsigned)gad_ceil_div(ix, 256)), dim3(256), 0, st, wi);
   GAD_LAUNCH_CHECK("gad_gemm(winograd wgrad transforms)");
   const gad_gemm_args sub = wino_wgrad_products_args(a, wq, Wy, V, dU);
@@ -3025,7 +3261,21 @@
     GAD_CHECK(a->ws && a->ws_bytes >= need, "gad_gemm: split-K workspace too small (%lld < %lld)", (long long)a->ws_bytes, (long long)need);
   }
   d.tiles_m = pl.tiles_m; d.tiles_n = pl.tiles_n; d.splitk = pl.splitk; d.ktiles_per_split = pl.ktiles_per_split;
-  if (a->A2) {
+  if (r.s2p) {
+    const S2Classes& c = r.s2;
+    for (int q = 0; q < 4; ++q) {
+      GAD_CHECK(c.rows[q] < (1L << 31), "gad_gemm: too many rows in a parity class");
+      d.s2_tile0[q] = c.tile0[q];
+      d.s2_rows[q] = (int)c.rows[q];
+      d.s2_fd_hw[q] = make_fastdiv((unsigned)(c.n[0][q >> 1] * c.n[1][q & 1]));
+    }
+    d.s2_tile0[4] = c.tile0[4];
+    for (int ax = 0; ax < 2; ++ax)
+      for (int par = 0; par < 2; ++par) { d.s2_n[ax][par] = c.n[ax][par]; d.s2_o0[ax][par] = c.o0[ax][par]; }
+    d.s2_fd_w[0] = make_fastdiv((unsigned)c.n[1][0]);
+    d.s2_fd_w[1] = make_fastdiv((unsigned)c.n[1][1]);
+    launch_mode<A_CONVT_S2P, GAD_B_WDGRAD, 4>(d, pl, st);
+  } else if (a->A2) {
     if (bf16) launch_bf16<A_CONV2, GAD_B_KC>(d, pl, st);
     else launch_mode<A_CONV2, GAD_B_KC, 4>(d, pl, st);
   } else if (a->A_k2) {
diff --git a/group-attribution-for-diffusion-models_amd/gad/_capi.py b/group-attribution-for-diffusion-models_amd/gad/_capi.py
--- a/group-attribution-for-diffusion-models_amd/gad/_capi.py
+++ b/group-attribution-for-diffusion-models_amd/gad/_capi.py
@@ -35,6 +35,11 @@
                 ("B_wino", C.c_void_p), ("wino_ws", C.c_void_p), ("wino_ws_bytes", C.c_int64), ("B_wino4", C.c_void_p)]
 
 
+class Wino4DyArgs(C.Structure):
+    _fields_ = [("dy", C.c_void_p), ("V", C.c_void_p), ("Wy", C.c_void_p), ("tilesum", C.c_void_p),
+                ("B", C.c_int32), ("H", C.c_int32), ("W", C.c_int32), ("C", C.c_int32), ("ldx", C.c_int32)]
+
+
 class GroupNormArgs(C.Structure):
     _fields_ = [("x", C.c_void_p), ("y", C.c_void_p), ("gamma", C.c_void_p), ("beta", C.c_void_p),
                 ("mean", C.c_void_p), ("rstd", C.c_void_p), ("dy", C.c_void_p),
@@ -104,6 +109,8 @@
 GEMM_NO_WINO = 16
 GEMM_WINO_WGRAD = 32
 GEMM_WINO_ONLY_INPUT, GEMM_WINO_SKIP_INPUT = 64, 128
+GEMM_WINO_SKIP_DY = 256
+GEMM_S2_PARITY = 512
 A_KC, A_MC, A_CONV, A_CONVT = 0, 1, 2, 3
 B_KC, B_MC, B_WDGRAD, B_CONV = 0, 1, 2, 3
 
@@ -116,9 +123,13 @@
     "gad_gemm": (C.c_int, [C.POINTER(GemmArgs), _vp]),
     "gad_gemm_uses_bf16": (C.c_int, [C.POINTER(GemmArgs)]),
     "gad_gemm_kernel_id": (C.c_int, [C.POINTER(GemmArgs)]),
+    "gad_gemm_s2_parity": (C.c_int, [C.POINTER(GemmArgs)]),
+    "gad_s2_parity_rows": (_i64, [C.POINTER(ConvGeom), _i32, _i32]),
+    "gad_s2_parity_pixel": (_i64, [C.POINTER(ConvGeom), _i32, _i32, _i64]),
     "gad_gemm_wino_bytes": (_i64, [C.POINTER(GemmArgs)]),
     "gad_wino_weights": (C.c_int, [_vp, _vp, _vp, _i64, _vp]),
     "gad_wino4_weights": (C.c_int, [_vp, _vp, _vp, _i64, _vp]),
+    "gad_wino4_dy_transforms": (C.c_int, [C.POINTER(Wino4DyArgs), _vp]),
     "gad_groupnorm_one_pass": (C.c_int, [C.POINTER(GroupNormArgs)]),
     "gad_gemm_plan": (C.c_int, [C.POINTER(GemmArgs), C.POINTER(_i32), C.POINTER(_i32), C.POINTER(_i32)]),
     "gad_groupnorm_workspace_bytes": (_i64, [C.POINTER(GroupNormArgs)]),
diff --git a/group-attribution-for-diffusion-models_amd/gad/ops.py b/group-attribution-for-diffusion-models_amd/gad/ops.py
--- a/group-attribution-for-diffusion-models_amd/gad/ops.py
+++ b/group-attribution-for-diffusion-models_amd/gad/ops.py
@@ -83,6 +83,11 @@
     return v, first
 
 
+def _sink_peek(param):
+    v = getattr(param, "_gad_sink", None) if (param is not None and _SINK_ACTIVE[0]) else None
+    return v if (v is not None and getattr(param, "_gad_sink_epoch", -1) != _SINK_EPOCH[0]) else None
+
+
 def _deliver(param, grad):
     v, first = _sink(param)
     if v is None:
@@ -123,15 +128,16 @@
 
 
 KERNEL_FLAGS = {"gemm": 0, "gn": 0, "native_dgrad": False, "two_kernel_attn_bwd": False, "narrow_attn_fwd": False, "no_wino4": False,
-                "no_gn_wino": False}
+                "no_gn_wino": False, "no_dy_once": False, "no_s2_parity": False}
 
 
 class kernel_flags:
 
     def __init__(self, no_patch=False, tap_major_k=False, gn_two_pass=False, scalar_epilogue=False, general_loaders=False,
-                 native_dgrad=False, two_kernel_attn_bwd=False, narrow_attn_fwd=False, no_wino=False, no_wino4=False, no_gn_wino=False):
+                 native_dgrad=False, two_kernel_attn_bwd=False, narrow_attn_fwd=False, no_wino=False, no_wino4=False, no_gn_wino=False,
+                 no_dy_once=False, no_s2_parity=False):
         self.native_dgrad, self.two_kernel_attn_bwd, self.narrow_attn_fwd, self.no_wino4 = native_dgrad, two_kernel_attn_bwd, narrow_attn_fwd, no_wino4
-        self.no_gn_wino = no_gn_wino
+        self.no_gn_wino, self.no_dy_once, self.no_s2_parity = no_gn_wino, no_dy_once, no_s2_parity
         self.gemm = ((_capi.GEMM_NO_PATCH if no_patch else 0) | (_capi.GEMM_TAP_MAJOR_K if tap_major_k else 0)
                      | (_capi.GEMM_NO_WINO if no_wino else 0)
                      | (_capi.GEMM_SCALAR_EPILOGUE if scalar_epilogue else 0)
@@ -143,7 +149,8 @@
         KERNEL_FLAGS["gemm"], KERNEL_FLAGS["gn"], KERNEL_FLAGS["native_dgrad"] = self.gemm, self.gn, self.native_dgrad
         KERNEL_FLAGS["two_kernel_attn_bwd"], KERNEL_FLAGS["narrow_attn_fwd"] = self.two_kernel_attn_bwd, self.narrow_attn_fwd
         KERNEL_FLAGS["no_wino4"] = self.no_wino4
-        KERNEL_FLAGS["no_gn_wino"] = self.no_gn_wino
+        KERNEL_FLAGS["no_gn_wino"], KERNEL_FLAGS["no_dy_once"] = self.no_gn_wino, self.no_dy_once
+        KERNEL_FLAGS["no_s2_parity"] = self.no_s2_parity
         return self
 
     def __exit__(self, *exc):
@@ -175,7 +182,7 @@
              bias=None, rowadd=None, rows_per_group=1, residual=None, ldr=0, batch=1, batch_inner=1,
              sA=(0, 0), sB=(0, 0), sC=(0, 0), tile_hint=0, splitk_hint=0, A2=None, a_split=0, B_bf16=None,
              A_k2=None, B_k2=None, k_split=0, B_wino=None, B_wino4=None, wino_wgrad=False, wino_input=None, force_f32=False,
-             keep_v=None, wino_v=None):
+             keep_v=None, wino_v=None, probe=False, wino_ws=None, s2_parity=False):
     lib = _capi.load()
     ws = workspace(A.device)
     a = GemmArgs()
@@ -197,7 +204,8 @@
     a.ws, a.ws_bytes = ws.data_ptr(), ws.numel()
     a.tile_hint, a.splitk_hint = tile_hint, splitk_hint
     a.operand_precision = 1 if (OPERAND_PRECISION[0] and not force_f32) else 0
-    a.flags = KERNEL_FLAGS["gemm"]
+    a.flags = KERNEL_FLAGS["gemm"] | (_capi.GEMM_S2_PARITY if s2_parity else 0)
+    need = 0
     if A2 is not None:
         a.A2, a.a_split, a.ldx2 = A2.data_ptr(), a_split, A2.shape[-1]
     if B_bf16 is not None:
@@ -208,24 +216,30 @@
     if B_wino is not None or B_wino4 is not None:
         a.B_wino, a.B_wino4 = _ptr(B_wino), _ptr(B_wino4)
         need = lib.gad_gemm_wino_bytes(C.byref(a))
-        if need:
-            V = _scratch("wino", need, A.device)
-            a.wino_ws, a.wino_ws_bytes = V.data_ptr(), need
+        if need and not probe:
+            V = wino_ws if wino_ws is not None else _scratch("wino", need, A.device)
+            a.wino_ws, a.wino_ws_bytes = V.data_ptr(), V.numel()
             if keep_v is not None and a.B_wino4 and lib.gad_gemm_kernel_id(C.byref(a)) == 6:
                 keep_v.append(V)
-        else:
+        elif not need:
             a.B_wino = a.B_wino4 = None
     if wino_wgrad:
         a.flags |= _capi.GEMM_WINO_WGRAD
         need = lib.gad_gemm_wino_bytes(C.byref(a))
-        if need:
-            V = _scratch("wino", need, A.device)
-            a.wino_ws, a.wino_ws_bytes = V.data_ptr(), need
+        if need and not probe:
+            V = wino_ws if wino_ws is not None else _scratch("wino", need, A.device)
+            a.wino_ws, a.wino_ws_bytes = V.data_ptr(), V.numel()
+            if wino_ws is not None:
+                a.flags |= _capi.GEMM_WINO_SKIP_DY
             if wino_v is not None and wino_v.numel() >= 36 * (K // 16) * geom.C * 4:
                 a.B_wino4 = wino_v.data_ptr()
                 a.flags |= _capi.GEMM_WINO_SKIP_INPUT
-        else:
+        elif not need:
             a.flags &= ~_capi.GEMM_WINO_WGRAD
+    if probe:
+        return lib.gad_gemm_kernel_id(C.byref(a)), need
+    if wino_ws is not None and not wino_wgrad:
+        a.flags |= _capi.GEMM_WINO_SKIP_INPUT
     if wino_input is not None:
         if lib.gad_gemm_kernel_id(C.byref(a)) != 6 or not a.wino_ws:
             return False
@@ -271,6 +285,9 @@
             check(lib.gad_gemm(C.byref(a), _stream()), "gad_gemm")
         e.record()
         name = self.NAMES.get((a.a_mode, a.b_mode), "gemm") + ("", "_bf16", f"_patch_w{a.g.Wo}", f"_patch_bf16_w{a.g.Wo}", f"_fewout_valu_w{a.g.Wo}", "_wino", "_wino4", "_wino4")[kid]
+        s2p = bool(a.flags & _capi.GEMM_S2_PARITY) and lib.gad_gemm_s2_parity(C.byref(a)) == 1
+        if s2p:
+            name += "_s2parity"
         key = (name, tile.value, sk.value, vec.value)
         g = a.g
         if a.a_mode in (A_CONV, A_CONVT):
@@ -281,7 +298,7 @@
         extra = a.M * a.N if a.residual else 0
         nbytes = 4.0 * max(1, batch) * (a_elems + b_elems + a.M * a.N + extra)
         flops = 2.0 * a.M * a.N * a.K * max(1, batch)
-        executed = flops * ({5: 16.0 / 36.0, 6: 0.25, 7: 0.25}.get(kid, 1.0))
+        executed = flops * (0.25 if s2p else {5: 16.0 / 36.0, 6: 0.25, 7: 0.25}.get(kid, 1.0))
         stage = None
         if kid in (5, 6):
             npos, tpx = (16, 4) if kid == 5 else (36, 16)
@@ -354,7 +371,7 @@
 
 
 def conv2d_fwd_raw(x, w, bias, stride=1, pad=(1, 1, 1, 1), upsample=False, rowadd=None, residual=None,
-                   tile_hint=0, splitk_hint=0, x2=None, wino_input=None, keep_v=None):
+                   tile_hint=0, splitk_hint=0, x2=None, wino_input=None, keep_v=None, probe=False, wino_ws=None):
     _req(x, "conv x")
     Bn, H, W, C1 = x.shape
     Cin = C1
@@ -370,7 +387,7 @@
     He, We = (2 * H, 2 * W) if upsample else (H, W)
     Ho = _conv_out_size(He, KH, stride, pad[0], pad[1])
     Wo = _conv_out_size(We, KW, stride, pad[2], pad[3])
-    y = _out((Bn, Ho, Wo, Cout), x.device)
+    y = x if probe else _out((Bn, Ho, Wo, Cout), x.device)
     g = ConvGeom(H, W, Cin, C1, Ho, Wo, KH, KW, stride, pad[0], pad[2], int(upsample))
     if residual is not None:
         _req(residual, "conv residual")
@@ -380,10 +397,13 @@
     launched = gemm_raw(x, wk, y, A_CONV, B_KC, Bn * Ho * Wo, Cout, KH * KW * Cin, 0, KH * KW * Cin, Cout, geom=g,
              bias=bias, rowadd=rowadd, rows_per_group=Ho * Wo, residual=residual, ldr=Cout,
              tile_hint=tile_hint, splitk_hint=splitk_hint, A2=x2, a_split=C1, wino_input=wino_input, keep_v=keep_v,
+             probe=probe, wino_ws=wino_ws,
              B_wino=wino_weight(w, 2) if (wino_ok and (tile_hint == 7 or (tile_hint == 0 and not f4_maps))) else None,
              B_wino4=wino_weight(w, 4) if (wino_ok and tile_hint != 7 and f4_maps) else None,
              B_bf16=bf16_weight(w) if (OPERAND_PRECISION[0] >= 1 and KH == 3 and Cin % 32 == 0 and x2 is None
                                        and not torch.cuda.is_current_stream_capturing()) else None)
+    if probe:
+        return launched
     return y if launched is not False else None
 
 
@@ -599,7 +619,7 @@
         return dxe
     g = ConvGeom(Ho, Wo, Cout, Cout, He, We, KH, KW, stride, pad[0], pad[2], 0)
     gemm_raw(dy, wk, dxe, A_CONVT, B_WDGRAD, Bn * He * We, Cin, KH * KW * Cout, 0, 0, Cin, geom=g,
-             tile_hint=tile_hint, splitk_hint=splitk_hint)
+             tile_hint=tile_hint, splitk_hint=splitk_hint, s2_parity=stride == 2 and not KERNEL_FLAGS.get("no_s2_parity"))
     return _upsample2x_bwd(dxe, x_shape) if upsample else dxe
 
 
@@ -610,25 +630,40 @@
     return dx
 
 
-def conv2d_wgrad_raw(dy, x, w_like, stride=1, pad=(1, 1, 1, 1), upsample=False, tile_hint=0, splitk_hint=0, out=None, wino_v=None):
+def conv2d_wgrad_raw(dy, x, w_like, stride=1, pad=(1, 1, 1, 1), upsample=False, tile_hint=0, splitk_hint=0, out=None, wino_v=None,
+                     probe=False, wino_ws=None):
     _req(dy, "conv dy")
     _req(x, "conv x")
     Bn, H, W, Cin = x.shape
     Cout, _, KH, KW = w_like.shape
     _, Ho, Wo, _ = dy.shape
-    dwk = _out((Cout, KH, KW, Cin), dy.device) if out is None else weight_krsc(out)
+    dwk = (x if probe else _out((Cout, KH, KW, Cin), dy.device)) if out is None else weight_krsc(out)
     if (KH == 1 and KW == 1 and stride == 1 and tuple(pad) == (0, 0, 0, 0) and not upsample and Cin % 4 == 0 and Cout % 4 == 0
             and not KERNEL_FLAGS["gemm"] & _capi.GEMM_GENERAL_LOADERS):
-        gemm_raw(dy, x, dwk, A_MC, B_MC, Cout, Cin, Bn * H * W, Cout, Cin, Cin, tile_hint=tile_hint, splitk_hint=splitk_hint)
-        return dwk.permute(0, 3, 1, 2)
+        r = gemm_raw(dy, x, dwk, A_MC, B_MC, Cout, Cin, Bn * H * W, Cout, Cin, Cin, tile_hint=tile_hint, splitk_hint=splitk_hint,
+                     probe=probe)
+        return r if probe else dwk.permute(0, 3, 1, 2)
     g = ConvGeom(H, W, Cin, Cin, Ho, Wo, KH, KW, stride, pad[0], pad[2], int(upsample))
     wino = (KH == 3 and KW == 3 and stride == 1 and tuple(pad) == (1, 1, 1, 1) and tile_hint in (0, 8) and splitk_hint == 0
             and Ho % 4 == 0 and Wo % 4 == 0 and OPERAND_PRECISION[0] == 0 and not KERNEL_FLAGS.get("no_wino4")
             and not KERNEL_FLAGS["gemm"] & (_capi.GEMM_NO_WINO | _capi.GEMM_NO_PATCH | _capi.GEMM_SCALAR_EPILOGUE | _capi.GEMM_TAP_MAJOR_K
                                             | _capi.GEMM_GENERAL_LOADERS))
-    gemm_raw(dy, x, dwk, A_MC, B_CONV, Cout, KH * KW * Cin, Bn * Ho * Wo, Cout, 0, KH * KW * Cin, geom=g,
-             tile_hint=tile_hint, splitk_hint=splitk_hint, wino_wgrad=wino, wino_v=wino_v)
-    return dwk.permute(0, 3, 1, 2)
+    r = gemm_raw(dy, x, dwk, A_MC, B_CONV, Cout, KH * KW * Cin, Bn * Ho * Wo, Cout, 0, KH * KW * Cin, geom=g,
+                 tile_hint=tile_hint, splitk_hint=splitk_hint, wino_wgrad=wino, wino_v=wino_v, probe=probe, wino_ws=wino_ws)
+    return r if probe else dwk.permute(0, 3, 1, 2)
+
+
+def wino4_dy_transforms_raw(dy, V, Wy, tilesum=None):
+    _req(dy, "conv dy")
+    a = _capi.Wino4DyArgs()
+    a.dy, a.V, a.Wy, a.tilesum = dy.data_ptr(), V.data_ptr(), Wy.data_ptr(), _ptr(tilesum)
+    a.B, a.H, a.W, a.C = dy.shape
+    a.ldx = dy.shape[-1]
+    nbytes = 36 * (dy.numel() // 16) * 4
+    if V.numel() * V.element_size() < nbytes or Wy.numel() * Wy.element_size() < nbytes or (
+            tilesum is not None and tilesum.numel() * tilesum.element_size() < nbytes // 36):
+        raise _capi.GadError("wino4_dy_transforms: V / Wy / tilesum smaller than the images written into them")
+    check(_capi.load().gad_wino4_dy_transforms(C.byref(a), _stream()), "gad_wino4_dy_transforms")
 
 
 def colsum_raw(dy2d: torch.Tensor, segments=1, out=None):
@@ -734,6 +769,24 @@
 def _conv_backward(ctx, dy, x, x_shape, w, stride, pad, upsample, has, need):
     dy = dy.contiguous()
     dx = None
+    V, ctx.wino_v = ctx.wino_v, None
+    need_bias, need_rowadd = has[0] and need[2], has[1] and need[3]
+    if need[0] and need[1] and dgrad_as_forward(w, stride, pad) and not KERNEL_FLAGS.get("no_dy_once"):
+        wr = rotated_weight(w)
+        kid_d, bytes_d = conv2d_fwd_raw(dy, wr, None, probe=True)
+        kid_w, bytes_w = conv2d_wgrad_raw(dy, x, w, stride, pad, upsample, out=_sink_peek(w), wino_v=V, probe=True)
+        if kid_d == 6 and kid_w == 7:
+            Bn, Ho, Wo, Cout = dy.shape
+            ws_d, ws_w = _scratch("wino", bytes_d, dy.device), _scratch("wino", bytes_w, dy.device)
+            tilesum = _scratch("tilesum", Bn * Ho * Wo // 16 * Cout * 4, dy.device).view(torch.float32) if (need_bias or need_rowadd) else None
+            wino4_dy_transforms_raw(dy, ws_d, ws_w, tilesum)
+            dx = conv2d_fwd_raw(dy, wr, None, wino_ws=ws_d)
+            if upsample:
+                dx = _upsample2x_bwd(dx, x_shape)
+            dw = _param_grad(w, lambda o: conv2d_wgrad_raw(dy, x, w, stride, pad, upsample, out=o, wino_v=V, wino_ws=ws_w))
+            db, dr = _conv_epilogue_grads(tilesum.view(Bn, Ho * Wo // 16, Cout) if tilesum is not None else None, ctx.bias_ref,
+                                          need_bias, need_rowadd)
+            return dx, dw, db, dr, (dy if (has[2] and need[4]) else None)
     if need[0]:
         if dgrad_as_forward(w, stride, pad):
             dx = conv2d_fwd_raw(dy, rotated_weight(w), None)
@@ -741,9 +794,8 @@
                 dx = _upsample2x_bwd(dx, x_shape)
         else:
             dx = conv2d_dgrad_raw(dy, w, x_shape, stride, pad, upsample)
-    V, ctx.wino_v = ctx.wino_v, None
     dw = _param_grad(w, lambda o: conv2d_wgrad_raw(dy, x, w, stride, pad, upsample, out=o, wino_v=V)) if need[1] else None
-    db, dr = _conv_epilogue_grads(dy, ctx.bias_ref, has[0] and need[2], has[1] and need[3])
+    db, dr = _conv_epilogue_grads(dy, ctx.bias_ref, need_bias, need_rowadd)
     dres = dy if (has[2] and need[4]) else None
     return dx, dw, db, dr, dres
 
@@ -768,14 +820,17 @@
 
 
 def _conv_epilogue_grads(dy, bias, need_bias, need_rowadd):
-    Bn, Ho, Wo, Cout = dy.shape
     db = dr = None
+    if not (need_rowadd or need_bias):
+        return db, dr
+    Bn, Cout = dy.shape[0], dy.shape[-1]
+    rows = dy.reshape(-1, Cout)
     if need_rowadd:
-        dr = colsum_raw(dy.view(Bn * Ho * Wo, Cout), segments=Bn)
+        dr = colsum_raw(rows, segments=Bn)
         if need_bias:
             db = _param_grad(bias, lambda o: colsum_raw(dr, 1, out=o).view(Cout))
     elif need_bias:
-        db = _param_grad(bias, lambda o: colsum_raw(dy.view(Bn * Ho * Wo, Cout), 1, out=o).view(Cout))
+        db = _param_grad(bias, lambda o: colsum_raw(rows, 1, out=o).view(Cout))
     return db, dr
 
 
diff --git a/include/gad.h b/include/gad.h
--- a/include/gad.h
+++ b/include/gad.h
@@ -72,17 +72,31 @@
   GAD_GEMM_SCALAR_EPILOGUE = 4,
   GAD_GEMM_GENERAL_LOADERS = 8,
   GAD_GEMM_WINO_ONLY_INPUT = 64,
-  GAD_GEMM_WINO_SKIP_INPUT = 128
+  GAD_GEMM_WINO_SKIP_INPUT = 128,
+  GAD_GEMM_WINO_SKIP_DY = 256,
+  GAD_GEMM_S2_PARITY = 512
 };
 
 int64_t gad_gemm_workspace_bytes(const gad_gemm_args* a);
 int gad_gemm_plan(const gad_gemm_args* a, int32_t* tile, int32_t* splitk, int32_t* vec);
 int gad_gemm(const gad_gemm_args* a, void* stream);
 int gad_gemm_uses_bf16(const gad_gemm_args* a);
+int gad_gemm_s2_parity(const gad_gemm_args* a);
+int64_t gad_s2_parity_rows(const gad_conv_geom* g, int32_t images, int32_t q);
+int64_t gad_s2_parity_pixel(const gad_conv_geom* g, int32_t images, int32_t q, int64_t i);
 int gad_gemm_kernel_id(const gad_gemm_args* a);
 int64_t gad_gemm_wino_bytes(const gad_gemm_args* a);
 int gad_wino_weights(const float* src, float* dst, const int64_t* table, int64_t n_tiles, void* stream);
 int gad_wino4_weights(const float* src, float* dst, const int64_t* table, int64_t n_tiles, void* stream);
+
+typedef struct gad_wino4_dy_args {
+  const float* dy;
+  float* V;
+  float* Wy;
+  float* tilesum;
+  int32_t B, H, W, C, ldx;
+} gad_wino4_dy_args;
+int gad_wino4_dy_transforms(const gad_wino4_dy_args* a, void* stream);
 
 typedef struct gad_groupnorm_args {
   const float* x;
```
